# Genie-Kim/PintheMemory

Measured on AMD Instinct MI355X. Metric: train imgs/sec 768x768 bs=8 R50-DeepLabV3+ +mem, higher is better.
Workload: dtype f32

## Files before the change

include/pinmem_hip.h:

```cpp
#ifndef PINMEM_HIP_H
#define PINMEM_HIP_H
#include <stddef.h>
#include <stdint.h>

#ifdef __cplusplus
extern "C" {
#endif

typedef enum pm_status { PM_OK = 0, PM_EINVAL = -1, PM_EWORKSPACE = -2, PM_ELAUNCH = -3, PM_EUNSUPPORTED = -4 } pm_status;

typedef enum pm_dtype { PM_F32 = 0, PM_BF16 = 1 } pm_dtype;
#define PM_TF_ZERO_PAD64 1

typedef struct pm_tensor {
  void* ptr;
  int32_t n, h, w, c;
  int64_t pitch;
  int32_t dtype;
  int32_t flags;
} pm_tensor;

#define PM_ABI_VERSION 400

typedef struct pm_conv_params {
  int32_t struct_size;
  int32_t kh, kw, stride, pad, dil;
  int32_t prec;
  void* wino_v;
  int64_t wino_v_bytes;
  void* wxf;
  int64_t wxf_bytes;
  int32_t wxf_valid;
} pm_conv_params;

typedef struct pm_conv_epilogue {
  int64_t struct_size;
  const float* bias;
  const float* scale;
  const float* shift;
  const float* residual;
  int64_t residual_pitch;
  int32_t relu;
  float* bn_partials;
  int64_t bn_partials_bytes;
} pm_conv_epilogue;

const char* pm_last_error(void);
int pm_version(void);

size_t pm_conv_workspace(const pm_tensor* x, const pm_tensor* y, const pm_conv_params* p, int which );
size_t pm_conv_winograd_v_bytes(const pm_tensor* x, const pm_tensor* y, const pm_conv_params* p);
size_t pm_conv_wxf_bytes(const pm_tensor* x, const pm_tensor* y, const pm_conv_params* p);
size_t pm_conv_wxf_bytes_dgrad(const pm_tensor* dy, const pm_tensor* dx, const pm_conv_params* p);
typedef struct pm_wxf_job {
  const float* w;
  void* wxf;
  int64_t wxf_bytes;
  int32_t cout, kh, kw, cin;
  int32_t dgrad;
  int32_t reserved;
} pm_wxf_job;
int pm_conv_wxf_refresh_bf16(const pm_wxf_job* jobs, int n, void* stream);
int pm_conv_wxf_refresh_f32(const pm_wxf_job* jobs, int n, void* stream);
size_t pm_conv_bn_partials_bytes(const pm_tensor* x, const pm_tensor* y, const pm_conv_params* p);
int pm_conv_fwd(const pm_tensor* x, const float* w_krsc, const pm_tensor* y, const pm_conv_params* p,
                const pm_conv_epilogue* ep, void* ws, size_t ws_bytes, void* stream);
int pm_conv_bwd_data(const pm_tensor* dy, const float* w_krsc, const pm_tensor* dx, const pm_conv_params* p,
                     const pm_tensor* add, void* ws, size_t ws_bytes, void* stream);
int pm_conv_bwd_weight(const pm_tensor* x, const pm_tensor* dy, float* dw_krsc, float* dbias, const pm_conv_params* p,
                       void* ws, size_t ws_bytes, void* stream);

typedef struct pm_routing {
  int32_t struct_size;
  int32_t winograd;
  int32_t winograd_fused;
  int32_t conv16;
  int32_t conv16_wide;
  int32_t conv16_persistent;
  int32_t wgrad16;
  int32_t bf16_wgrad;
  int32_t split;
} pm_routing;
int pm_routing_get(pm_routing* out);
int pm_routing_set(const pm_routing* r);


int pm_set_winograd(int mode);
int pm_set_winograd_fused(int on);
int pm_set_conv16(int on);
int pm_set_bf16_wgrad(int on);
int pm_set_wgrad16(int on);
int pm_set_split(int on);

int pm_profile_enable(int on);
int pm_profile_dump(const char* csv_path);
int pm_profile_read(int mode, int bm, int bn, int km, int nst, double* total_ms, double* total_flops, int64_t* launches, int clear);
int pm_profile_read_prec(int mode, int bm, int bn, int km, int nst, int prec, double* total_ms, double* total_flops, int64_t* launches, int clear);
int pm_profile_read_bytes(int mode, int bm, int bn, int km, int nst, int prec, double* total_bytes);

size_t pm_bn_workspace(const pm_tensor* x);
int pm_bn_stats(const pm_tensor* x, float* moments, void* ws, size_t ws_bytes, void* stream);
int pm_bn_stats_finalize(const pm_tensor* x, float eps, float* mean, float* invstd, float* running_mean , float* running_var ,
                         float momentum, void* ws, size_t ws_bytes, void* stream);
int pm_bn_merge(const float* parts, int world, int c, float* moments, void* stream);
int pm_bn_merge_finalize(const float* parts, int world, int c, float eps, float* mean, float* invstd, float* running_mean ,
                         float* running_var , float momentum, void* stream);
int pm_bn_finalize(const float* moments, int c, float eps, float* mean, float* invstd,
                   float* running_mean, float* running_var, float momentum, void* stream);
int pm_bn_apply(const pm_tensor* x, const float* mean, const float* invstd, const float* gamma, const float* beta,
                const pm_tensor* residual , int relu, const pm_tensor* y, void* stream);
int pm_bn_apply_mask(const pm_tensor* x, const float* mean, const float* invstd, const float* gamma, const float* beta,
                     const pm_tensor* residual , int relu, const pm_tensor* y, uint8_t* mask , void* stream);
int pm_bn_bwd_reduce_mask(const pm_tensor* dy, const uint8_t* mask, const pm_tensor* x, const float* mean, const float* invstd,
                          const pm_tensor* gmask , float* sums, void* ws, size_t ws_bytes, void* stream);
int pm_bn_bwd_reduce(const pm_tensor* dy, const pm_tensor* y , const pm_tensor* x, const float* mean, const float* invstd,
                     const float* gamma , const float* beta , int relu, const pm_tensor* gmask ,
                     float* sums, void* ws, size_t ws_bytes, void* stream);
int pm_bn_bwd_apply(const pm_tensor* dy, const pm_tensor* y , const pm_tensor* x, const float* mean, const float* invstd,
                    const float* gamma, const float* beta , const float* sums, float count, int relu, const pm_tensor* dx,
                    const pm_tensor* dres , void* stream);
int pm_bn_partials_finalize(const float* partials, int64_t pixels, int c, float eps, float* mean, float* invstd, float* running_mean ,
                            float* running_var , float momentum, float* moments , void* stream);
int pm_bn_fold(const float* gamma, const float* beta, const float* running_mean, const float* running_var, const float* conv_bias,
               int c, float eps, float* scale, float* shift, void* stream);
int pm_bn_fold_multi(const void* table, const int* cs, const int* offs, int n, int max_c, int total, float eps, float* arena, void* stream);
int pm_relu_bwd(const pm_tensor* dy, const pm_tensor* y, const pm_tensor* dx, void* stream);
int pm_add(const pm_tensor* a, const pm_tensor* b, const pm_tensor* y, void* stream);
int pm_add_n(const pm_tensor* const* xs, int n, const pm_tensor* y, void* stream);
int pm_copy(const pm_tensor* src, const pm_tensor* dst, void* stream);
int pm_scale_shift_act(const pm_tensor* x, const float* scale, const float* shift, const pm_tensor* residual, int relu,
                       const pm_tensor* y, void* stream);

int pm_cast(const pm_tensor* x, const pm_tensor* y, void* stream);

int pm_maxpool3x3s2_fwd(const pm_tensor* x, const pm_tensor* y, uint8_t* argmax, void* stream);
int pm_maxpool3x3s2_bwd(const pm_tensor* dy, const uint8_t* argmax, const pm_tensor* dx, void* stream);
int pm_global_avgpool_fwd(const pm_tensor* x, const pm_tensor* y , void* stream);
int pm_global_avgpool_bwd(const pm_tensor* dy, const pm_tensor* dx, int accumulate, void* stream);

int pm_resize_bilinear_fwd(const pm_tensor* x, const pm_tensor* y, void* stream);
int pm_resize_bilinear_bwd(const pm_tensor* dy, const pm_tensor* dx, int accumulate, void* stream);
size_t pm_resize_bilinear_bwd_workspace(const pm_tensor* dy, const pm_tensor* dx);
int pm_resize_bilinear_bwd_separable(const pm_tensor* dy, const pm_tensor* dx, int accumulate, void* ws, size_t ws_bytes, void* stream);

int pm_resize_bilinear_hp_fwd(const pm_tensor* x, const pm_tensor* y, int flip_w, void* stream);
int pm_softmax_mean_update(const pm_tensor* logits, double* buffer, int counter, void* stream);
int pm_sliding_stitch(const pm_tensor* logits, const int32_t* tiles_xyxy, int ntiles, int H, int W, int flip_w, double* acc, int accumulate, void* stream);
int pm_argmax_f64(const double* buffer, int n, int h, int w, int c, int64_t* out_cls, double* out_prob , void* stream);

// ... 59 lines not shown
```

pinthememory_amd/csrc/bn.hip:

```cpp
#include "pm_common.h"

namespace {

constexpr int CB = 64;
constexpr int RL = 16;

__device__ __forceinline__ float bn_affine(float v, float mu, float is, float ga, float be) {
  const float s = is * ga;
  return fmaf(v, s, fmaf(-mu, s, be));
}

inline int chunk_rows(long P, int C) {
  const long colblocks = std::max<long>(1, (C + CB - 1) / CB);
  const long want = std::max<long>(512, 2048 / colblocks);
  long r = (P + want - 1) / want;
  r = std::max<long>(r, 64);
  return (int)((r + RL - 1) / RL * RL);
}

__global__ __launch_bounds__(256) void bn_stats_partial(const float* __restrict__ x, long pitch, long P, int C, int rows, float* __restrict__ part) {
  __shared__ float sm[RL][CB][2];
  const int g = threadIdx.x & 15, r = threadIdx.x >> 4;
  const int c = blockIdx.y * CB + g * 4;
  const long p0 = (long)blockIdx.x * rows, p1 = min(P, p0 + rows);
  float s1[4] = {0, 0, 0, 0}, s2[4] = {0, 0, 0, 0};
  if (c < C) {
    const float4 k = PM_LD4(x + c);
    for (long p = p0 + r; p < p1; p += RL) {
      const float4 v = PM_LD4(x + p * pitch + c);
      const float d0 = v.x - k.x, d1 = v.y - k.y, d2 = v.z - k.z, d3 = v.w - k.w;
      s1[0] += d0, s1[1] += d1, s1[2] += d2, s1[3] += d3;
      s2[0] += d0 * d0, s2[1] += d1 * d1, s2[2] += d2 * d2, s2[3] += d3 * d3;
    }
  }
#pragma unroll
  for (int j = 0; j < 4; ++j) sm[r][g * 4 + j][0] = s1[j], sm[r][g * 4 + j][1] = s2[j];
  __syncthreads();
  if (threadIdx.x < CB * 2) {
    const int cc = threadIdx.x >> 1, w = threadIdx.x & 1;
    float s = 0.f;
#pragma unroll
    for (int i = 0; i < RL; ++i) s += sm[i][cc][w];
    const int ch = blockIdx.y * CB + cc;
    if (ch < C) part[((long)blockIdx.x * C + ch) * 2 + w] = s;
  }
}

constexpr int FC = 4, FL = 64;
__device__ __forceinline__ void final_sums(const float* __restrict__ part, int nb, int C, int c, int lane, double& s1, double& s2) {
  __shared__ double red[FL][FC][2];
  double a = 0.0, b = 0.0;
  if (c < C)
#pragma unroll 8
    for (int i = lane; i < nb; i += FL) {
      const float2 v = *reinterpret_cast<const float2*>(part + ((long)i * C + c) * 2);
      a += (double)v.x, b += (double)v.y;
    }
  red[lane][threadIdx.x & (FC - 1)][0] = a, red[lane][threadIdx.x & (FC - 1)][1] = b;
  __syncthreads();
  s1 = s2 = 0.0;
  if (lane == 0) {
#pragma unroll
    for (int i = 0; i < FL; ++i) s1 += red[i][threadIdx.x & (FC - 1)][0], s2 += red[i][threadIdx.x & (FC - 1)][1];
  }
}

template <bool FIN>
__global__ __launch_bounds__(256) void bn_stats_final(const float* __restrict__ part, int nb, const float* __restrict__ x, long P, int C, float* __restrict__ moments,
                                                      float eps, float* __restrict__ mean, float* __restrict__ invstd, float* running_mean, float* running_var,
                                                      float momentum) {
  const int c = blockIdx.x * FC + (threadIdx.x & (FC - 1)), lane = threadIdx.x / FC;
  double s1, s2;
  final_sums(part, nb, C, c, lane, s1, s2);
  if (lane != 0 || c >= C) return;
  const double n = (double)P;
  const float m = (float)((double)x[c] + s1 / n), m2 = (float)fmax(s2 - s1 * s1 / n, 0.0), nf = (float)n;
  if constexpr (!FIN) {
    moments[c] = m;
    moments[C + c] = m2;
    moments[2 * C + c] = nf;
  } else {
    const float var = m2 / nf;
    mean[c] = m;
    invstd[c] = 1.f / sqrtf(var + eps);
    if (running_mean) running_mean[c] = (1.f - momentum) * running_mean[c] + momentum * m;
    if (running_var && nf > 1.f) running_var[c] = (1.f - momentum) * running_var[c] + momentum * (m2 / (nf - 1.f));
  }
}

__global__ void bn_finalize_kernel(const float* __restrict__ moments, int C, float eps, float* __restrict__ mean, float* __restrict__ invstd,
                                   float* running_mean, float* running_var, float momentum) {
  const int c = blockIdx.x * blockDim.x + threadIdx.x;
  if (c >= C) return;
// ... 291 lines not shown
  PM_REQUIRE(!gmask || (relu != 0 && pm_vec4(gmask) && pm_same_shape(gmask, x)), PM_EINVAL, "bn_bwd_reduce: gmask needs a ReLU mode and the shape of x");
  PM_REQUIRE(ws && ws_bytes >= pm_bn_workspace(x), PM_EWORKSPACE, "bn_bwd_reduce: workspace too small");
  const long P = pm_pixels(x);
  const int rows = chunk_rows(P, x->c), nb = pm_cdiv(P, rows);
  hipStream_t st = (hipStream_t)stream;
  dim3 grid(nb, pm_cdiv(x->c, CB));
  const float *pdy = (const float*)dy->ptr, *py = relu == 1 ? (const float*)y->ptr : nullptr, *px = (const float*)x->ptr;
  const long yp = relu == 1 ? y->pitch : 0;
  float* pg = gmask ? (float*)gmask->ptr : nullptr;
  const long gp = gmask ? gmask->pitch : 0;
#define PM_BN_BWD_PARTIAL(R, G)                                                                                                                         \
  hipLaunchKernelGGL((bn_bwd_partial<R, G>), grid, dim3(256), 0, st, pdy, (long)dy->pitch, py, yp, px, (long)x->pitch, mean, invstd, gamma, beta, pg, gp, P, \
                     x->c, rows, (float*)ws)
  if (relu == 0) PM_BN_BWD_PARTIAL(0, false);
  else if (relu == 1 && gmask) PM_BN_BWD_PARTIAL(1, true);
  else if (relu == 1) PM_BN_BWD_PARTIAL(1, false);
  else if (gmask) PM_BN_BWD_PARTIAL(2, true);
  else PM_BN_BWD_PARTIAL(2, false);
#undef PM_BN_BWD_PARTIAL
  hipLaunchKernelGGL(bn_bwd_final, dim3(pm_cdiv(x->c, FC)), dim3(256), 0, st, (const float*)ws, nb, x->c, sums);
  return pm_check_launch("bn_bwd_reduce");
}

extern "C" int pm_bn_bwd_reduce_mask(const pm_tensor* dy, const uint8_t* mask, const pm_tensor* x, const float* mean, const float* invstd,
                                     const pm_tensor* gmask, float* sums, void* ws, size_t ws_bytes, void* stream) {
  PM_REQUIRE(dy && x && mask, PM_EINVAL, "bn_bwd_reduce_mask: null");
  if (pm_is_bf16(x)) return pm16_bn_bwd_reduce(dy, nullptr, mask, x, mean, invstd, nullptr, nullptr, 3, gmask, sums, ws, ws_bytes, (hipStream_t)stream);
  if (int e = check_bn(dy, "bn_bwd_reduce_mask")) return e;
  if (int e = check_bn(x, "bn_bwd_reduce_mask")) return e;
  PM_REQUIRE(pm_same_shape(dy, x) && mean && invstd && sums && mask, PM_EINVAL, "bn_bwd_reduce_mask: bad args");
  PM_REQUIRE(!gmask || (pm_vec4(gmask) && pm_same_shape(gmask, x)), PM_EINVAL, "bn_bwd_reduce_mask: gmask must have the shape of x");
  PM_REQUIRE(ws && ws_bytes >= pm_bn_workspace(x), PM_EWORKSPACE, "bn_bwd_reduce_mask: workspace too small");
  const long P = pm_pixels(x);
  const int rows = chunk_rows(P, x->c), nb = pm_cdiv(P, rows);
  hipStream_t st = (hipStream_t)stream;
  dim3 grid(nb, pm_cdiv(x->c, CB));
  float* pg = gmask ? (float*)gmask->ptr : nullptr;
  const long gp = gmask ? gmask->pitch : 0;
  if (gmask)
    hipLaunchKernelGGL((bn_bwd_partial<3, true>), grid, dim3(256), 0, st, (const float*)dy->ptr, (long)dy->pitch, reinterpret_cast<const float*>(mask), 0l,
                       (const float*)x->ptr, (long)x->pitch, mean, invstd, (const float*)nullptr, (const float*)nullptr, pg, gp, P, x->c, rows, (float*)ws);
  else
    hipLaunchKernelGGL((bn_bwd_partial<3, false>), grid, dim3(256), 0, st, (const float*)dy->ptr, (long)dy->pitch, reinterpret_cast<const float*>(mask), 0l,
                       (const float*)x->ptr, (long)x->pitch, mean, invstd, (const float*)nullptr, (const float*)nullptr, pg, gp, P, x->c, rows, (float*)ws);
  hipLaunchKernelGGL(bn_bwd_final, dim3(pm_cdiv(x->c, FC)), dim3(256), 0, st, (const float*)ws, nb, x->c, sums);
  return pm_check_launch("bn_bwd_reduce_mask");
}

extern "C" int pm_bn_bwd_apply(const pm_tensor* dy, const pm_tensor* y, const pm_tensor* x, const float* mean, const float* invstd, const float* gamma,
                               const float* beta, const float* sums, float count, int relu, const pm_tensor* dx, const pm_tensor* dres, void* stream) {
  PM_REQUIRE(dy && x && dx, PM_EINVAL, "bn_bwd_apply: null");
  if (pm_is_bf16(x)) return pm16_bn_bwd_apply(dy, y, x, mean, invstd, gamma, beta, sums, count, relu, dx, dres, (hipStream_t)stream);
  if (int e = check_bn(dy, "bn_bwd_apply")) return e;
  if (int e = check_bn(x, "bn_bwd_apply")) return e;
  if (int e = check_bn(dx, "bn_bwd_apply")) return e;
  PM_REQUIRE(pm_same_shape(dy, x) && pm_same_shape(dx, x) && mean && invstd && gamma && sums, PM_EINVAL, "bn_bwd_apply: bad args");
  PM_REQUIRE(relu >= 0 && relu <= 2, PM_EINVAL, "bn_bwd_apply: relu mode %d (0 none, 1 mask from y, 2 mask rebuilt from x)", relu);
  PM_REQUIRE(relu != 1 || (y && pm_vec4(y) && pm_same_shape(y, x)), PM_EINVAL, "bn_bwd_apply: relu mode 1 needs the forward output");
  PM_REQUIRE(relu != 2 || beta, PM_EINVAL, "bn_bwd_apply: relu mode 2 needs beta");
  PM_REQUIRE(!dres || (pm_vec4(dres) && pm_same_shape(dres, x)), PM_EINVAL, "bn_bwd_apply: dres shape mismatch");
  const float *pd = (const float*)dy->ptr, *po = relu == 1 ? (const float*)y->ptr : nullptr, *px = (const float*)x->ptr;
  float *pdx = (float*)dx->ptr, *pdr = dres ? (float*)dres->ptr : nullptr;
  const long a = dy->pitch, b = relu == 1 ? y->pitch : 0, c = x->pitch, d = dx->pitch, e2 = dres ? dres->pitch : 0;
  const bool from_x = relu == 2;
  const int C = x->c;
  const bool dev_count = !(count > 0.f);
  const float host_inv_n = dev_count ? 0.f : 1.f / count;
  return pm_ew_launch(true, pm_pixels(x), C, (hipStream_t)stream, "bn_bwd_apply", [=] __device__(long p, int ch) {
    const float inv_n = dev_count ? 1.f / sums[2 * C] : host_inv_n;
    float4 g = PM_LD4(pd + p * a + ch);
    if (po) {
      const float4 o = PM_LD4(po + p * b + ch);
      g.x = o.x > 0.f ? g.x : 0.f, g.y = o.y > 0.f ? g.y : 0.f, g.z = o.z > 0.f ? g.z : 0.f, g.w = o.w > 0.f ? g.w : 0.f;
    }
    const float4 v = PM_LD4(px + p * c + ch), mu = PM_LD4(mean + ch), is = PM_LD4(invstd + ch), ga = PM_LD4(gamma + ch);
    if (from_x) {
      const float4 be = PM_LD4(beta + ch);
      g.x = bn_affine(v.x, mu.x, is.x, ga.x, be.x) > 0.f ? g.x : 0.f, g.y = bn_affine(v.y, mu.y, is.y, ga.y, be.y) > 0.f ? g.y : 0.f;
      g.z = bn_affine(v.z, mu.z, is.z, ga.z, be.z) > 0.f ? g.z : 0.f, g.w = bn_affine(v.w, mu.w, is.w, ga.w, be.w) > 0.f ? g.w : 0.f;
    }
    if (pdr) PM_ST4(pdr + p * e2 + ch, g);
    const float4 s1 = PM_LD4(sums + ch), s2 = PM_LD4(sums + C + ch);
    float4 r;
    r.x = (g.x - s1.x * inv_n - (v.x - mu.x) * is.x * (s2.x * inv_n)) * (is.x * ga.x);
    r.y = (g.y - s1.y * inv_n - (v.y - mu.y) * is.y * (s2.y * inv_n)) * (is.y * ga.y);
    r.z = (g.z - s1.z * inv_n - (v.z - mu.z) * is.z * (s2.z * inv_n)) * (is.z * ga.z);
    r.w = (g.w - s1.w * inv_n - (v.w - mu.w) * is.w * (s2.w * inv_n)) * (is.w * ga.w);
    PM_ST4(pdx + p * d + ch, r);
  });
}
```

pinthememory_amd/csrc/conv_igemm.hip:

```cpp
#include <stdlib.h>
#include <algorithm>
#include <type_traits>
#include <vector>

#include "pm_common.h"

#include "conv_igemm_kernel.h"

namespace {

template <int ZL, bool O16 = false>
__global__ __launch_bounds__(256) void splitk_reduce_vec_kernel(const float* __restrict__ ws, int ksplit, long slab, int M, int Nn,
                                                                float* __restrict__ C, long c_pitch, const float* bias,
                                                                const float* scale, const float* shift, const float* residual,
                                                                long res_pitch, int relu) {
  constexpr int GP = 256 / ZL;
  __shared__ float4 red[ZL > 1 ? ZL : 1][GP];
  const int gl = threadIdx.x % GP, zl = threadIdx.x / GP;
  const long groups = (long)M * Nn / 4;
  for (long g0 = (long)blockIdx.x * GP; g0 < groups; g0 += (long)gridDim.x * GP) {
    const long grp = g0 + gl;
    float4 v = make_float4(0.f, 0.f, 0.f, 0.f);
    if (grp < groups)
#pragma unroll 8
// ... 375 lines not shown
    g_prof.push_back(rec);
  }
  return pm_check_launch("conv_igemm");
}

int check_common(const pm_tensor* x, const pm_tensor* y, const pm_conv_params* p) {
  PM_REQUIRE(x && y && p && x->ptr && y->ptr, PM_EINVAL, "conv: null tensor");
  PM_REQUIRE(p->struct_size == (int32_t)sizeof(pm_conv_params), PM_EINVAL, "conv: pm_conv_params.struct_size %d != %zu -- caller built against another pinmem_hip.h (library ABI %d)",
             p->struct_size, sizeof(pm_conv_params), PM_ABI_VERSION);
  PM_REQUIRE(p->kh >= 1 && p->kw >= 1 && p->dil >= 1 && p->pad >= 0, PM_EINVAL, "conv: bad geometry");
  PM_REQUIRE(p->stride == 1 || p->stride == 2, PM_EUNSUPPORTED, "conv: stride %d unsupported (1 or 2)", p->stride);
  const int ho = (x->h + 2 * p->pad - p->dil * (p->kh - 1) - 1) / p->stride + 1;
  const int wo = (x->w + 2 * p->pad - p->dil * (p->kw - 1) - 1) / p->stride + 1;
  PM_REQUIRE(ho == y->h && wo == y->w && x->n == y->n, PM_EINVAL, "conv: output %dx%d does not match geometry (%dx%d)", y->h, y->w, ho, wo);
  PM_REQUIRE((x->dtype == PM_F32 || x->dtype == PM_BF16) && (y->dtype == PM_F32 || y->dtype == PM_BF16), PM_EUNSUPPORTED, "conv: dtype %d / %d", x->dtype, y->dtype);
  for (const pm_tensor* t : {x, y}) {
    if (pm_is_bf16(t)) PM_REQUIRE(pm_vec8(t), PM_EINVAL, "conv: bf16 tensors must be 16B aligned with pitch %% 8 == 0 and channels %% 8 == 0");
    else PM_REQUIRE(pm_vec_ok(t), PM_EINVAL, "conv: tensors must be 16B aligned with pitch %% 4 == 0");
  }
  PM_REQUIRE(x->c % 4 == 0, PM_EUNSUPPORTED, "conv: Cin %% 4 != 0 unsupported (pad the input channels)");
  PM_REQUIRE((y->c % 4 == 0) || (p->kh * p->kw == 1), PM_EUNSUPPORTED, "conv: Cout %% 4 != 0 only for 1x1");
  PM_REQUIRE(x->pitch >= x->c && y->pitch >= y->c, PM_EINVAL, "conv: pitch < channels");
  PM_REQUIRE(pm_pixels(x) * x->pitch < (1ll << 29) && pm_pixels(y) * y->pitch < (1ll << 29) && (int64_t)y->c * x->c * p->kh * p->kw < (1ll << 29),
             PM_EUNSUPPORTED, "conv: tensor too large for 32-bit byte offsets (2 GiB per tensor)");
  return PM_OK;
}

void fill_geom(ConvK& k, const pm_tensor* x, const pm_tensor* y, const pm_conv_params* p) {
  k.N = x->n, k.H = x->h, k.W = x->w, k.Cin = x->c, k.x_pitch = x->pitch;
  k.Ho = y->h, k.Wo = y->w, k.Cout = y->c, k.y_pitch = y->pitch;
  k.kh = p->kh, k.kw = p->kw, k.stride = p->stride, k.pad = p->pad, k.dil = p->dil;
  k.sshift = p->stride == 2 ? 1 : 0;
  k.prec = p->prec != 0 ? 1 : 0;
  k.T_eff = p->kh * p->kw, k.tk_w = p->kw, k.ky0 = k.kx0 = 0, k.ksy = k.ksx = 1;
  k.sub = k.sub_cy = k.sub_cx = 0, k.Hc = x->h, k.Wc = x->w;
  k.bias = k.scale = k.shift = k.residual = nullptr;
  k.res_pitch = 0, k.relu = 0, k.stats = nullptr, k.io16 = 0;
  k.stage_ep = 1;
  k.spl_prio = 1;
  k.n_group = 8;
  k.batch_xcd = 0;
  k.a_bs = k.b_bs = k.c_bs = 0;
}

struct WinoPlan {
  bool use;
  pm_wino_geom g;
  int Kp, P;
  size_t v_bytes, m_bytes, u_bytes;
  Plan pl;
};
WinoPlan wino_plan(const pm_tensor* xin, int cout, const pm_conv_params* p, bool wgrad = false) {
  WinoPlan wp{};
  if (wgrad && (long)xin->c * cout < 256 * 256) return wp;
  if (pm_route.winograd == 0 || p->kh != 3 || p->kw != 3 || p->stride != 1 || p->pad != p->dil || p->prec != 0) return wp;
  const int cin = xin->c;
  if (cin < 128 || cout < 128 || (cout & 3) || (cin & 3)) return wp;
  int m = 0;
  double best_ratio = 0.6;
  for (int cand = pm_route.winograd; cand >= 2; cand -= 2) {
    const pm_wino_geom g = pm_wino_make_geom(xin->n, xin->h, xin->w, p->dil, cand);
    const double cover = (double)(cand * g.TY * p->dil) * (double)(cand * g.TX * p->dil) / ((double)xin->h * xin->w);
    const double ratio = cover * (cand + 2) * (cand + 2) / (9.0 * cand * cand);
    if (ratio <= best_ratio) best_ratio = ratio, m = cand, wp.g = g;
  }
  if (!m) return wp;
  wp.P = (m + 2) * (m + 2);
  wp.Kp = (cin + BK - 1) / BK * BK;
  if (wp.g.tiles * (long)std::max(wp.Kp, cout) * 4 >= (1ll << 31)) return wp;
  wp.v_bytes = pm_align_up((size_t)wp.P * wp.g.tiles * wp.Kp * sizeof(float), 256);
  wp.m_bytes = pm_align_up((size_t)wp.P * wp.g.tiles * cout * sizeof(float), 256);
  wp.u_bytes = pm_align_up((size_t)wp.P * cout * wp.Kp * sizeof(float), 256);
  wp.pl.bm = 128, wp.pl.bn = 128;
  if (pm_cdiv(cout, 128) * 128 > cout * 1.12 && pm_cdiv(cout, 64) * 64 < pm_cdiv(cout, 128) * 128) wp.pl.bn = 64;
  if (wp.g.tiles <= 4608 && !pm_route.split) wp.pl.bm = 64;
  wp.pl.tiles_m = pm_cdiv(wp.g.tiles, wp.pl.bm), wp.pl.tiles_n = pm_cdiv(cout, wp.pl.bn);
  wp.pl.ksplit = 1, wp.pl.kper = wp.Kp, wp.pl.ws_bytes = 0;
  wp.use = true;
  return wp;
}
inline size_t wino_ws(const WinoPlan& wp) { return wp.v_bytes + wp.m_bytes + wp.u_bytes; }

int wino_conv(const pm_tensor* xin, const float* w, int w_cout, int w_cin, bool dgrad, const pm_tensor* yout, const WinoPlan& wp,
              const pm_conv_epilogue& ep, void* ws, hipStream_t st, float* v_keep = nullptr, float* u_ext = nullptr, bool u_valid = false) {
  float* V = v_keep ? v_keep : (float*)ws;
  float* Mo = (float*)((char*)ws + wp.v_bytes);
  float* U = u_ext ? u_ext : (float*)((char*)ws + wp.v_bytes + wp.m_bytes);
  const int cout = yout->c;
  if (int e = pm_wino_input_xf((const float*)xin->ptr, xin->pitch, xin->c, wp.Kp, wp.g, V, st)) return e;
  if (!(u_ext && u_valid))
    if (int e = pm_wino_filter_xf(w, w_cout, w_cin, wp.Kp, dgrad, wp.g.m, U, st)) return e;
  const pm_tensor xv = {V, 1, 1, (int32_t)wp.g.tiles, wp.Kp, wp.Kp};
  const pm_tensor yv = {Mo, 1, 1, (int32_t)wp.g.tiles, cout, cout};
  const pm_conv_params p1 = {(int32_t)sizeof(pm_conv_params), 1, 1, 1, 0, 1, 0};
  ConvK k;
  fill_geom(k, &xv, &yv, &p1);
  k.A = V, k.B = U, k.C = Mo;
  k.M = (int)wp.g.tiles, k.Nn = cout, k.K = wp.Kp;
  k.a_bytes = (unsigned)(wp.g.tiles * wp.Kp * 4), k.b_bytes = (unsigned)((long)cout * wp.Kp * 4), k.kmode = K_FAST;
  k.c_pitch = cout, k.c_split = 0;
  k.a_bs = wp.g.tiles * wp.Kp, k.b_bs = (long)cout * wp.Kp, k.c_bs = wp.g.tiles * cout;
  if (pm_route.winograd_fused && wp.g.m == 4 && wp.Kp % 16 == 0) {
    ProfRec rec{};
    if (g_prof_on) {
      (void)hipEventCreate(&rec.a), (void)hipEventCreate(&rec.b);
      rec.mode = 3, rec.bm = 32, rec.bn = 32, rec.km = 0, rec.prec = 0, rec.nst = 1, rec.M = (int)wp.g.tiles, rec.Nn = cout, rec.K = wp.Kp, rec.batch = wp.P, rec.ksplit = 1;
      rec.flops = 2.0 * wp.P * (double)wp.g.tiles * cout * xin->c;
      (void)hipEventRecord(rec.a, st);
    }
    const int e = pm_wino_fused_f4(V, U, cout, wp.Kp, wp.g, (float*)yout->ptr, yout->pitch, ep.bias, ep.scale, ep.shift, ep.residual, ep.residual_pitch, ep.relu, st);
    if (g_prof_on) {
      (void)hipEventRecord(rec.b, st);
      g_prof.push_back(rec);
    }
    return e;
  }
  if (int e = launch<MODE_FWD>(k, wp.pl, st, wp.P, 2.0 * wp.P * (double)wp.g.tiles * cout * xin->c)) return e;
  return pm_wino_output_xf(Mo, cout, wp.g, (float*)yout->ptr, yout->pitch, ep.bias, ep.scale, ep.shift, ep.residual, ep.residual_pitch, ep.relu, st);
}

struct WinoWgradPlan {
  Plan pl;
  size_t slab_bytes;
};
WinoWgradPlan wino_wgrad_plan(const WinoPlan& wp, int cout) {
  WinoWgradPlan q{};
  q.pl.bm = 128, q.pl.bn = 128;
  if (pm_cdiv(wp.Kp, 128) * 128 > wp.Kp * 1.12 && pm_cdiv(wp.Kp, 64) * 64 < pm_cdiv(wp.Kp, 128) * 128) q.pl.bn = 64;
  q.pl.tiles_m = pm_cdiv(cout, 128), q.pl.tiles_n = pm_cdiv(wp.Kp, q.pl.bn);
  const long ksteps = (wp.g.tiles + BK - 1) / BK;
  const long per_split = (long)q.pl.tiles_m * q.pl.tiles_n * wp.P;
  long ks = std::max<long>(1, std::min<long>((768 + per_split / 2) / per_split, ksteps / 8));
  const long steps_per = (ksteps + ks - 1) / ks;
  ks = (ksteps + steps_per - 1) / steps_per;
  q.pl.ksplit = (int)ks, q.pl.kper = (int)(steps_per * BK), q.pl.ws_bytes = 0;
  q.slab_bytes = pm_align_up((size_t)ks * wp.P * cout * wp.Kp * sizeof(float), 256);
  return q;
}
inline size_t wino_wgrad_ws(const WinoPlan& wp, const WinoWgradPlan& q) { return wp.v_bytes + wp.m_bytes + q.slab_bytes; }

int wino_wgrad(const pm_tensor* x, const pm_tensor* dy, float* dw, const WinoPlan& wp, const WinoWgradPlan& q, void* ws, hipStream_t st,
               float* v_kept = nullptr) {
  float* V = v_kept ? v_kept : (float*)ws;
  float* Z = (float*)((char*)ws + wp.v_bytes);
  float* slab = (float*)((char*)ws + wp.v_bytes + wp.m_bytes);
  const int cout = dy->c;
  if (!v_kept)
    if (int e = pm_wino_input_xf((const float*)x->ptr, x->pitch, x->c, wp.Kp, wp.g, V, st)) return e;
  if (int e = pm_wino_dy_xf((const float*)dy->ptr, dy->pitch, cout, wp.g, Z, st)) return e;
  const pm_tensor xv = {V, 1, 1, (int32_t)wp.g.tiles, wp.Kp, wp.Kp};
  const pm_tensor zv = {Z, 1, 1, (int32_t)wp.g.tiles, cout, cout};
  const pm_conv_params p1 = {(int32_t)sizeof(pm_conv_params), 1, 1, 1, 0, 1, 0};
  ConvK k;
  fill_geom(k, &xv, &zv, &p1);
  k.A = Z, k.B = V, k.C = slab;
  k.M = cout, k.Nn = wp.Kp, k.K = (int)wp.g.tiles;
  k.a_bytes = (unsigned)(wp.g.tiles * cout * 4), k.b_bytes = (unsigned)(wp.g.tiles * wp.Kp * 4), k.kmode = K_MID;
  k.c_pitch = wp.Kp, k.c_split = (long)wp.P * cout * wp.Kp;
  k.a_bs = wp.g.tiles * cout, k.b_bs = wp.g.tiles * wp.Kp, k.c_bs = (long)cout * wp.Kp;
  if (int e = launch<MODE_WGRAD>(k, q.pl, st, wp.P, 2.0 * wp.P * (double)wp.g.tiles * cout * x->c)) return e;
  return pm_wino_dw_xf(slab, q.pl.ksplit, cout, x->c, wp.Kp, wp.g.m, dw, st);
}

struct Bf16Plan {
  bool use;
  bool c16;
  pm_conv16 k16;
  bool inplace;
  int Cp;
  long M, Nn, Kf;
  size_t xb_bytes, wb_bytes;
  Plan pl;
};
Bf16Plan bf16_plan(const pm_tensor* xin, const pm_tensor* yout, const pm_conv_params* p) {
  Bf16Plan b{};
  if ((p->prec != 2 && !pm_is_bf16(xin) && !pm_is_bf16(yout)) || xin->c < 32) return b;
  b.Cp = (xin->c + 63) / 64 * 64;
  const long T = (long)p->kh * p->kw;
  b.M = pm_pixels(yout), b.Nn = yout->c, b.Kf = T * b.Cp / 2;
  b.inplace = pm_is_bf16(xin) && (xin->c % 64 == 0 || ((xin->flags & PM_TF_ZERO_PAD64) && xin->pitch >= b.Cp));
  const size_t xb = b.inplace ? (size_t)pm_pixels(xin) * xin->pitch * 2 : (size_t)pm_pixels(xin) * b.Cp * 2, wb = (size_t)yout->c * T * b.Cp * 2;
  if (xb >= (1ull << 31) || wb >= (1ull << 31)) return b;
  b.xb_bytes = b.inplace ? 0 : pm_align_up(xb, 256), b.wb_bytes = pm_align_up(wb, 256);
  b.pl = make_plan(MODE_FWD, b.M, b.Nn, b.Kf, true);
  if (b.pl.bn < 64) return b;
  b.use = true;
  constexpr long C16_MIN_M = 256;
  b.c16 = false;
  if (pm_route.conv16 && b.M >= C16_MIN_M && p->stride >= 1) {
    pm_conv16& k = b.k16;
    k = pm_conv16{};
    k.N = xin->n, k.H = xin->h, k.W = xin->w, k.Ho = yout->h, k.Wo = yout->w;
    k.a_pitch = b.inplace ? xin->pitch : b.Cp, k.Cp = b.Cp;
    k.kh = p->kh, k.kw = p->kw, k.stride = p->stride, k.pad = p->pad, k.dil = p->dil;
    k.M = (int)b.M, k.Nn = (int)b.Nn, k.K = (int)(T * b.Cp), k.ksteps = k.K / 64;
    k.c_pitch = yout->pitch, k.c_f32 = pm_is_bf16(yout) ? 0 : 1;
    pm_conv16_plan(&k);
    b.c16 = pm_route.conv16 == 2 || k.wide || k.bm == 64 || k.ksteps_per == 1 || (b.pl.bm == 64 && k.ksteps >= 16);
  }
  return b;
}
inline size_t bf16_ws(const Bf16Plan& b) {
  return b.xb_bytes + b.wb_bytes + std::max(pm_align_up(b.pl.ws_bytes, 256), b.c16 ? pm_conv16_slab_bytes(&b.k16) : (size_t)0);
}

int conv_bf16(const pm_tensor* xin, const float* w, int w_cout, int w_cin, bool rotate, const pm_tensor* yout, const pm_conv_params* pe, const Bf16Plan& b,
              const pm_conv_epilogue& e0, void* ws, hipStream_t st, char* wb_ext = nullptr, bool wb_valid = false) {
  char* xb = b.inplace ? (char*)xin->ptr : (char*)ws;
  char* wb = wb_ext ? wb_ext : (char*)ws + b.xb_bytes;
  float* slab = (float*)((char*)ws + b.xb_bytes + b.wb_bytes);
  const int T = pe->kh * pe->kw;
  if (!b.inplace) {
    if (pm_is_bf16(xin)) {
      if (int e = pm16_pad_rows((const pm_bf16*)xin->ptr, xin->pitch, xin->c, b.Cp, pm_pixels(xin), (pm_bf16*)xb, st)) return e;
    } else if (int e = pm_bf16_cast_rows((const float*)xin->ptr, xin->pitch, xin->c, b.Cp, pm_pixels(xin), xb, st)) return e;
  }
  if (!(wb_ext && wb_valid))
    if (int e = pm_bf16_cast_weights(w, w_cout, T, w_cin, b.Cp, rotate, wb, st)) return e;
  const long xpitch16 = b.inplace ? xin->pitch : b.Cp;
  if (b.c16) {
    const bool o16 = pm_is_bf16(yout);
    const bool ep_any = e0.bias || e0.scale || e0.residual || e0.relu;
    const bool ok = (!e0.bn_partials || o16) &&
                    (o16 ? ((yout->c | yout->pitch | (e0.residual ? e0.residual_pitch : 0)) & 7) == 0 && pm_aligned16(yout->ptr) && pm_aligned16(e0.residual)
                         : !(e0.scale || e0.residual || e0.relu));
    if (ok) {
      pm_conv16 k = b.k16;
      k.A = (const pm_bf16*)xb, k.B = (const pm_bf16*)wb;
      const double fl = 2.0 * (double)b.M * (double)b.Nn * (double)T * (double)xin->c * (g_prof_on ? pm_conv16_executed_fraction(&k) : 1.0);
      ProfRec rec{};
      if (g_prof_on) {
        (void)hipEventCreate(&rec.a), (void)hipEventCreate(&rec.b);
// ... 237 lines not shown
  pm_route.conv16_wide = (on == 3 || on == 8) ? 2 : (on == 7 ? 3 : ((on == 2 || on == 4) ? 0 : pm_route_defaults.conv16_wide));
  pm_route.conv16_persistent = on == 8 ? 0 : (on == 3 ? 1 : pm_route_defaults.conv16_persistent);
  return PM_OK;
}
extern "C" int pm_set_winograd_fused(int on) {
  pm_route.winograd_fused = on != 0;
  return PM_OK;
}
extern "C" int pm_set_wgrad16(int on) {
  pm_route.wgrad16 = on != 0;
  return PM_OK;
}
extern "C" int pm_set_split(int on) {
  pm_route.split = on ? 1 : 0;
  return PM_OK;
}
extern "C" int pm_set_bf16_wgrad(int on) {
  pm_route.bf16_wgrad = on != 0;
  return PM_OK;
}
extern "C" int pm_profile_enable(int on) {
  g_prof_on = on != 0;
  return PM_OK;
}
extern "C" int pm_profile_read_prec(int mode, int bm, int bn, int km, int nst, int prec, double* total_ms, double* total_flops, int64_t* launches, int clear);
extern "C" int pm_profile_read(int mode, int bm, int bn, int km, int nst, double* total_ms, double* total_flops, int64_t* launches, int clear) {
  return pm_profile_read_prec(mode, bm, bn, km, nst, -1, total_ms, total_flops, launches, clear);
}
extern "C" int pm_profile_read_prec(int mode, int bm, int bn, int km, int nst, int prec, double* total_ms, double* total_flops, int64_t* launches, int clear) {
  double ms = 0.0, fl = 0.0;
  int64_t n = 0;
  for (const ProfRec& r : g_prof) {
    if ((mode >= 0 && r.mode != mode) || (bm >= 0 && r.bm != bm) || (bn >= 0 && r.bn != bn) || (km >= 0 && r.km != km) || (nst >= 0 && r.nst != nst) ||
        (prec >= 0 && r.prec != prec))
      continue;
    float t = 0.f;
    if (hipEventSynchronize(r.b) != hipSuccess || hipEventElapsedTime(&t, r.a, r.b) != hipSuccess) continue;
    ms += t, fl += r.flops, ++n;
  }
  if (clear) {
    for (const ProfRec& r : g_prof) (void)hipEventDestroy(r.a), (void)hipEventDestroy(r.b);
    g_prof.clear();
  }
  if (total_ms) *total_ms = ms;
  if (total_flops) *total_flops = fl;
  if (launches) *launches = n;
  return PM_OK;
}

extern "C" int pm_profile_read_bytes(int mode, int bm, int bn, int km, int nst, int prec, double* total_bytes) {
  double b = 0.0;
  for (const ProfRec& r : g_prof) {
    if ((mode >= 0 && r.mode != mode) || (bm >= 0 && r.bm != bm) || (bn >= 0 && r.bn != bn) || (km >= 0 && r.km != km) || (nst >= 0 && r.nst != nst) ||
        (prec >= 0 && r.prec != prec))
      continue;
    b += r.bytes;
  }
  if (total_bytes) *total_bytes = b;
  return PM_OK;
}

extern "C" int pm_profile_dump(const char* path) {
  PM_REQUIRE(path, PM_EINVAL, "pm_profile_dump: null path");
  FILE* f = fopen(path, "w");
  PM_REQUIRE(f, PM_EINVAL, "pm_profile_dump: cannot open %s", path);
  fprintf(f, "mode,bm,bn,km,nst,prec,M,N,K,batch,ksplit,ms,gflop\n");
  for (const ProfRec& r : g_prof) {
    float t = 0.f;
    if (hipEventSynchronize(r.b) != hipSuccess || hipEventElapsedTime(&t, r.a, r.b) != hipSuccess) continue;
    fprintf(f, "%d,%d,%d,%d,%d,%d,%d,%d,%d,%d,%d,%.5f,%.4f\n", r.mode, r.bm, r.bn, r.km, r.nst, r.prec, r.M, r.Nn, r.K, r.batch, r.ksplit, t, r.flops * 1e-9);
  }
  fclose(f);
  return PM_OK;
}

extern "C" size_t pm_conv_winograd_v_bytes(const pm_tensor* x, const pm_tensor* y, const pm_conv_params* p0) {
  if (!x || !y || !p0) return 0;
  const pm_conv_params tp = tier_params(p0, x, y);
  const pm_conv_params* p = &tp;
  const WinoPlan f = wino_plan(x, y->c, p), g = wino_plan(x, y->c, p, true);
  return (f.use && g.use && f.g.m == g.g.m) ? f.v_bytes : 0;
}

extern "C" size_t pm_conv_wxf_bytes(const pm_tensor* x, const pm_tensor* y, const pm_conv_params* p0) {
  if (!x || !y || !p0) return 0;
  const pm_conv_params tp = tier_params(p0, x, y);
  const pm_conv_params* p = &tp;
  const WinoPlan f = wino_plan(x, y->c, p);
  if (f.use) return f.u_bytes;
  if (p->prec == 2) {
    const Bf16Plan b = bf16_plan(x, y, p);
    if (b.use) return b.wb_bytes;
  }
  return 0;
}

extern "C" int pm_conv_wxf_refresh_f32(const pm_wxf_job* jobs, int n, void* stream) {
  PM_REQUIRE(n >= 0 && (jobs || n == 0), PM_EINVAL, "conv_wxf_refresh_f32: bad job table");
  std::vector<const float*> w(n);
  std::vector<float*> U(n);
  std::vector<int> cout(n), cin(n), kp(n), m(n);
  for (int i = 0; i < n; ++i) {
    const pm_wxf_job& q = jobs[i];
    PM_REQUIRE(q.w && q.wxf && q.cout > 0 && q.cin > 0 && q.kh == 3 && q.kw == 3 && q.dgrad == 0, PM_EINVAL,
               "conv_wxf_refresh_f32: job %d: forward transforms of 3x3 filters only", i);
    PM_REQUIRE(pm_aligned16(q.wxf), PM_EINVAL, "conv_wxf_refresh_f32: job %d: buffer must be 16-byte aligned", i);
    const int Kp = (q.cin + BK - 1) / BK * BK;
    const size_t u4 = pm_align_up((size_t)36 * q.cout * Kp * sizeof(float), 256), u2 = pm_align_up((size_t)16 * q.cout * Kp * sizeof(float), 256);
    PM_REQUIRE((size_t)q.wxf_bytes == u4 || (size_t)q.wxf_bytes == u2, PM_EINVAL, "conv_wxf_refresh_f32: job %d: %ld bytes is neither the F(4x4) nor the F(2x2) transform of %d x %d",
               i, (long)q.wxf_bytes, q.cout, q.cin);
    w[i] = q.w, U[i] = (float*)q.wxf, cout[i] = q.cout, cin[i] = q.cin, kp[i] = Kp, m[i] = (size_t)q.wxf_bytes == u4 ? 4 : 2;
  }
  return pm_wino_filter_xf_multi(w.data(), U.data(), cout.data(), cin.data(), kp.data(), m.data(), n, (hipStream_t)stream);
}

extern "C" size_t pm_conv_wxf_bytes_dgrad(const pm_tensor* dy, const pm_tensor* dx, const pm_conv_params* p0) {
  if (!dy || !dx || !p0) return 0;
  const pm_conv_params tp = tier_params(p0, dy, dx);
  if (!dgrad_bf16_ok(&tp)) return 0;
  const pm_conv_params q = dgrad_as_fwd(&tp);
  const Bf16Plan b = bf16_plan(dy, dx, &q);
  return b.use ? b.wb_bytes : 0;
}

static bool bn_partials_route(const pm_tensor* x, const pm_tensor* y, const pm_conv_params* p) {
  if (!x || !y || !p || check_common(x, y, p) != PM_OK) return false;
  if (pm_is_bf16(y)) {
    if (!pm_vec8(y)) return false;
    const Bf16Plan b = bf16_plan(x, y, p);
    return b.use && (b.c16 ? (b.k16.ksplit == 1 && !b.k16.wide) : b.pl.ksplit == 1);
  }
  if (pm_is_bf16(x)) return false;
  if ((y->c & 3) || (y->pitch & 3) || !pm_aligned16(y->ptr)) return false;
  if (p->prec == 2) {
    const Bf16Plan b = bf16_plan(x, y, p);
    if (b.use) return b.pl.ksplit == 1;
  }
  if (wino_plan(x, y->c, p).use) return false;
  if (p->prec != 0) return false;
  long M, Nn, K;
  gemm_dims(MODE_FWD, x, y, p, M, Nn, K);
  const Plan pl = make_plan(MODE_FWD, M, Nn, K, false);
  return pl.ksplit == 1 && pl.bn >= 64;
}
extern "C" size_t pm_conv_bn_partials_bytes(const pm_tensor* x, const pm_tensor* y, const pm_conv_params* p) {
  if (!bn_partials_route(x, y, p)) return 0;
  return pm_align_up((size_t)pm_cdiv(pm_pixels(y), 32) * y->c * 2 * sizeof(float), 256);
}

extern "C" size_t pm_conv_workspace(const pm_tensor* x, const pm_tensor* y, const pm_conv_params* p0, int which) {
  const pm_conv_params tp = tier_params(p0, x, y);
  const pm_conv_params* p = &tp;
  if (which == MODE_DGRAD && p->stride == 2) {
    {
      const S2Native s = s2_native_plan(y, x, p);
      if (s.ok) return s.total;
    }
    size_t slab = 0, tmp = 0;
    for (int cls = 0; cls < 4; ++cls) {
      const S2Class c = s2_class(cls, x, p);
      tmp = std::max(tmp, (size_t)c.M * x->c * sizeof(float));
      if (c.M > 0 && c.nky * c.nkx > 0) slab = std::max(slab, make_plan(MODE_DGRAD, c.M, x->c, (long)c.nky * c.nkx * y->c, p->prec != 0).ws_bytes);
    }
    return pm_align_up(4 * pm_align_up(tmp, 256) + slab + 256, 256) + upcast_bytes(y);
  }
  if (which == MODE_FWD && p->prec == 2) {
    const Bf16Plan b = bf16_plan(x, y, p);
    if (b.use) return bf16_ws(b);
  }
  if (which == MODE_DGRAD && dgrad_bf16_ok(p)) {
    const pm_conv_params q = dgrad_as_fwd(p);
    const Bf16Plan b = bf16_plan(y, x, &q);
    if (b.use) return bf16_ws(b);
  }
  if (which == MODE_FWD || which == MODE_DGRAD) {
    const WinoPlan wp = which == MODE_FWD ? wino_plan(x, y->c, p) : wino_plan(y, x->c, p);
    if (wp.use) return wino_ws(wp);
  }
  const size_t bias_part = pm_align_up((size_t)pm_cdiv(pm_pixels(y), colsum_rows(pm_pixels(y), y->c)) * y->c * sizeof(float), 256);
  if (which == MODE_WGRAD && (pm_is_bf16(x) || pm_is_bf16(y))) {
    long M, Nn, K;
    gemm_dims(which, x, y, p, M, Nn, K);
    return pm_align_up(make_plan(which, M, Nn, K, true).ws_bytes, 256) + bias_part + upcast_bytes(x) + upcast_bytes(y);
  }
  if (which == MODE_WGRAD && p->prec == 2) {
    const Bf16WgradPlan b = bf16_wgrad_plan(x, y, p);
    if (b.use) return pm_align_up(bf16_wgrad_ws(b), 256) + bias_part;
  }
  if (which == MODE_WGRAD) {
    const WinoPlan wp = wino_plan(x, y->c, p, true);
    if (wp.use) return pm_align_up(wino_wgrad_ws(wp, wino_wgrad_plan(wp, y->c)), 256) + bias_part;
  }
  long M, Nn, K;
  gemm_dims(which, x, y, p, M, Nn, K);
  size_t b = make_plan(which, M, Nn, K, p->prec != 0).ws_bytes;
  if (which == MODE_WGRAD) b += bias_part;
  return pm_align_up(b, 256);
}

extern "C" int pm_conv_fwd(const pm_tensor* x, const float* w, const pm_tensor* y, const pm_conv_params* p0,
                           const pm_conv_epilogue* ep, void* ws, size_t ws_bytes, void* stream) {
  if (int e = check_common(x, y, p0)) return e;
  const pm_conv_params tp = tier_params(p0, x, y);
  const pm_conv_params* p = &tp;
  PM_REQUIRE(!ep || ep->struct_size == (int64_t)sizeof(pm_conv_epilogue), PM_EINVAL,
             "conv_fwd: pm_conv_epilogue.struct_size %ld != %zu -- caller built against another pinmem_hip.h (library ABI %d)", ep ? (long)ep->struct_size : 0l,
             sizeof(pm_conv_epilogue), PM_ABI_VERSION);
  if (ep && ep->bn_partials) {
    PM_REQUIRE(!ep->relu && !ep->residual, PM_EINVAL, "conv_fwd: bn_partials are the statistics of the convolution output (no residual / ReLU)");
    const size_t need = pm_conv_bn_partials_bytes(x, y, p);
    PM_REQUIRE(need != 0 && (size_t)ep->bn_partials_bytes >= need, PM_EINVAL, "conv_fwd: this call cannot emit bn_partials (ask pm_conv_bn_partials_bytes): %zu needed", need);
  }
  PM_REQUIRE(w && pm_aligned16(w), PM_EINVAL, "conv_fwd: weight null or unaligned");
  {
    pm_conv_epilogue e1 = {(int64_t)sizeof(pm_conv_epilogue), nullptr, nullptr, nullptr, nullptr, 0, 0};
    if (ep) e1 = *ep;
    PM_REQUIRE((e1.scale == nullptr) == (e1.shift == nullptr), PM_EINVAL, "conv_fwd: scale and shift go together");
    const WinoPlan wp = wino_plan(x, y->c, p);
    if (wp.use) {
      PM_REQUIRE(ws && ws_bytes >= wino_ws(wp), PM_EWORKSPACE, "conv_fwd(winograd): workspace %zu < %zu", ws_bytes, wino_ws(wp));
      float* keep = (p->wino_v && (size_t)p->wino_v_bytes >= wp.v_bytes) ? (float*)p->wino_v : nullptr;
      float* uext = (p->wxf && (size_t)p->wxf_bytes >= wp.u_bytes) ? (float*)p->wxf : nullptr;
      return wino_conv(x, w, y->c, x->c, false, y, wp, e1, ws, (hipStream_t)stream, keep, uext, p->wxf_valid != 0);
    }
  }
  if (p->prec == 2) {
    const Bf16Plan b = bf16_plan(x, y, p);
    if (b.use) {
      pm_conv_epilogue e2 = {(int64_t)sizeof(pm_conv_epilogue), nullptr, nullptr, nullptr, nullptr, 0, 0};
      if (ep) e2 = *ep;
      PM_REQUIRE((e2.scale == nullptr) == (e2.shift == nullptr), PM_EINVAL, "conv_fwd: scale and shift go together");
      PM_REQUIRE(ws && ws_bytes >= bf16_ws(b), PM_EWORKSPACE, "conv_fwd(bf16): workspace %zu < %zu", ws_bytes, bf16_ws(b));
      char* wext = (p->wxf && (size_t)p->wxf_bytes >= b.wb_bytes) ? (char*)p->wxf : nullptr;
      return conv_bf16(x, w, y->c, x->c, false, y, p, b, e2, ws, (hipStream_t)stream, wext, p->wxf_valid != 0);
    }
  }
  PM_REQUIRE(pm_is_f32(x), PM_EUNSUPPORTED, "conv_fwd: a bf16 input needs at least 32 channels (got %d)", x->c);
  long M, Nn, K;
  gemm_dims(MODE_FWD, x, y, p, M, Nn, K);
  Plan pl = make_plan(MODE_FWD, M, Nn, K, p->prec != 0);
  PM_REQUIRE(pl.ws_bytes <= ws_bytes && (pl.ws_bytes == 0 || ws), PM_EWORKSPACE, "conv_fwd: workspace %zu < %zu", ws_bytes, pl.ws_bytes);
  ConvK k;
  fill_geom(k, x, y, p);
  k.io16 = pm_is_bf16(y) ? 1 : 0;
  k.A = (const float*)x->ptr, k.B = w;
  k.M = (int)M, k.Nn = (int)Nn, k.K = (int)K;
  k.a_bytes = (unsigned)(pm_pixels(x) * x->pitch * 4), k.b_bytes = (unsigned)((long)y->c * K * 4), k.kmode = x->c % BK == 0 ? 0 : (x->c >= BK ? 1 : 2);
  pm_conv_epilogue e0 = {(int64_t)sizeof(pm_conv_epilogue), nullptr, nullptr, nullptr, nullptr, 0, 0};
  if (ep) e0 = *ep;
  PM_REQUIRE((e0.scale == nullptr) == (e0.shift == nullptr), PM_EINVAL, "conv_fwd: scale and shift go together");
  hipStream_t st = (hipStream_t)stream;
  if (pl.ksplit > 1) {
    k.C = (float*)ws, k.c_pitch = Nn, k.c_split = M * Nn;
    if (int e = launch<MODE_FWD>(k, pl, st)) return e;
    return splitk_reduce((const float*)ws, pl.ksplit, M, Nn, (float*)y->ptr, (long)y->pitch, e0.bias, e0.scale, e0.shift, e0.residual,
                         (long)e0.residual_pitch, e0.relu, st, k.io16 != 0);
  }
  k.C = (float*)y->ptr, k.c_pitch = y->pitch, k.c_split = 0;
  k.bias = e0.bias, k.scale = e0.scale, k.shift = e0.shift, k.residual = e0.residual, k.res_pitch = e0.residual_pitch, k.relu = e0.relu;
  k.stats = e0.bn_partials;
  return launch<MODE_FWD>(k, pl, st);
}

extern "C" int pm_conv_bwd_data(const pm_tensor* dy0, const float* w, const pm_tensor* dx, const pm_conv_params* p0, const pm_tensor* add,
                                void* ws, size_t ws_bytes, void* stream) {
  if (int e = check_common(dx, dy0, p0)) return e;
  const pm_conv_params tp = tier_params(p0, dy0, dx);
  const pm_conv_params* p = &tp;
  const pm_tensor* dy = dy0;
  pm_tensor dy32;
  PM_REQUIRE(!add || (add->ptr && pm_same_shape(add, dx) && add->dtype == dx->dtype), PM_EINVAL, "conv_bwd_data: `add` must match dx (shape and dtype)");
  PM_REQUIRE(!add || !pm_is_bf16(add) || pm_vec8(add), PM_EINVAL, "conv_bwd_data: bf16 `add` must be 16B aligned with pitch %% 8 == 0");
  const float* addp = add ? (const float*)add->ptr : nullptr;
  const long add_pitch = add ? add->pitch : 0;
  PM_REQUIRE(w && pm_aligned16(w), PM_EINVAL, "conv_bwd_data: weight null or unaligned");
  hipStream_t st0 = (hipStream_t)stream;
  if (p->stride == 2) {
    const size_t need = pm_conv_workspace(dx, dy, p, MODE_DGRAD);
    PM_REQUIRE(ws && ws_bytes >= need, PM_EWORKSPACE, "conv_bwd_data(stride 2): workspace %zu < %zu", ws_bytes, need);
    PM_REQUIRE(dx->c % 4 == 0, PM_EUNSUPPORTED, "conv_bwd_data(stride 2): Cin %% 4 != 0");
    {
      S2Native s = s2_native_plan(dy, dx, p);
      if (s.ok) return dgrad_s2_bf16(dy, w, dx, p, add, s, ws, st0);
    }
    if (pm_is_bf16(dy)) {
      if (int e = upcast(dy0, (char*)ws + need - upcast_bytes(dy0), &dy32, st0)) return e;
      dy = &dy32;
    }
    size_t tmp_bytes = 0;
    for (int cls = 0; cls < 4; ++cls) tmp_bytes = std::max(tmp_bytes, (size_t)s2_class(cls, dx, p).M * dx->c * sizeof(float));
    tmp_bytes = pm_align_up(tmp_bytes, 256);
    float* tmp = (float*)ws;
    float* slab = (float*)((char*)ws + 4 * tmp_bytes);
    unsigned char valid[4];
    for (int cls = 0; cls < 4; ++cls) {
      const S2Class c = s2_class(cls, dx, p);
      valid[cls] = c.M > 0 && c.nky * c.nkx > 0;
      if (!valid[cls]) continue;
      const long Kc = (long)c.nky * c.nkx * dy->c;
      const Plan pl = make_plan(MODE_DGRAD, c.M, dx->c, Kc, p->prec != 0);
      ConvK k;
      fill_geom(k, dx, dy, p);
      k.A = (const float*)dy->ptr, k.B = w;
      k.M = (int)c.M, k.Nn = dx->c, k.K = (int)Kc;
      k.a_bytes = (unsigned)(pm_pixels(dy) * dy->pitch * 4), k.b_bytes = (unsigned)((long)dy->c * p->kh * p->kw * dx->c * 4);
      k.kmode = dy->c >= BK ? K_MID : K_SMALL;
      k.T_eff = c.nky * c.nkx, k.tk_w = c.nkx, k.ky0 = c.ky0, k.kx0 = c.kx0, k.ksy = c.ksy, k.ksx = c.ksx;
      k.sub = 1, k.sub_cy = c.cy, k.sub_cx = c.cx, k.Hc = c.Hc, k.Wc = c.Wc;
      float* out = (float*)((char*)tmp + cls * tmp_bytes);
      if (pl.ksplit > 1) {
        k.C = slab, k.c_pitch = dx->c, k.c_split = c.M * dx->c;
        if (int e = launch<MODE_DGRAD>(k, pl, st0)) return e;
        if (int e = splitk_reduce(slab, pl.ksplit, c.M, dx->c, out, (long)dx->c, nullptr, nullptr, nullptr, nullptr, 0l, 0, st0)) return e;
      } else {
        k.C = out, k.c_pitch = dx->c, k.c_split = 0;
        if (int e = launch<MODE_DGRAD>(k, pl, st0)) return e;
      }
    }
    const int valid_mask = valid[0] | (valid[1] << 1) | (valid[2] << 2) | (valid[3] << 3);
    const long total = pm_pixels(dx) * (dx->c / 4);
    if (pm_is_bf16(dx))
      hipLaunchKernelGGL(dgrad_s2_interleave_kernel<true>, dim3((int)std::min<long>((total + 255) / 256, 8192)), dim3(256), 0, st0, (const float*)tmp,
                         (long)(tmp_bytes / sizeof(float)), valid_mask, (float*)dx->ptr, (long)dx->pitch, dx->n, dx->h, dx->w, dx->c, addp, add_pitch);
    else
      hipLaunchKernelGGL(dgrad_s2_interleave_kernel<false>, dim3((int)std::min<long>((total + 255) / 256, 8192)), dim3(256), 0, st0, (const float*)tmp,
                         (long)(tmp_bytes / sizeof(float)), valid_mask, (float*)dx->ptr, (long)dx->pitch, dx->n, dx->h, dx->w, dx->c, addp, add_pitch);
    return pm_check_launch("dgrad_s2_interleave");
  }
  if (dgrad_bf16_ok(p)) {
    const pm_conv_params q = dgrad_as_fwd(p);
    const Bf16Plan b = bf16_plan(dy, dx, &q);
    if (b.use) {
      PM_REQUIRE(ws && ws_bytes >= bf16_ws(b), PM_EWORKSPACE, "conv_bwd_data(bf16): workspace %zu < %zu", ws_bytes, bf16_ws(b));
      const pm_conv_epilogue e1 = {(int64_t)sizeof(pm_conv_epilogue), nullptr, nullptr, nullptr, addp, add_pitch, 0};
      char* wext = (p->wxf && (size_t)p->wxf_bytes >= b.wb_bytes) ? (char*)p->wxf : nullptr;
      return conv_bf16(dy, w, dy->c, dx->c, true, dx, &q, b, e1, ws, st0, wext, p->wxf_valid != 0);
    }
  }
  {
    const WinoPlan wp = wino_plan(dy, dx->c, p);
    if (wp.use) {
      PM_REQUIRE(ws && ws_bytes >= wino_ws(wp), PM_EWORKSPACE, "conv_bwd_data(winograd): workspace %zu < %zu", ws_bytes, wino_ws(wp));
      const pm_conv_epilogue e1 = {(int64_t)sizeof(pm_conv_epilogue), nullptr, nullptr, nullptr, addp, add_pitch, 0};
      return wino_conv(dy, w, dy->c, dx->c, true, dx, wp, e1, ws, st0);
    }
  }
  PM_REQUIRE(pm_is_f32(dy), PM_EUNSUPPORTED, "conv_bwd_data: a bf16 dy needs at least 32 channels and a stride-1 geometry the forward form covers");
  long M, Nn, K;
  gemm_dims(MODE_DGRAD, dx, dy, p, M, Nn, K);
  Plan pl = make_plan(MODE_DGRAD, M, Nn, K, p->prec != 0);
  PM_REQUIRE(pl.ws_bytes <= ws_bytes && (pl.ws_bytes == 0 || ws), PM_EWORKSPACE, "conv_bwd_data: workspace %zu < %zu", ws_bytes, pl.ws_bytes);
  ConvK k;
  fill_geom(k, dx, dy, p);
  k.io16 = pm_is_bf16(dx) ? 1 : 0;
  k.A = (const float*)dy->ptr, k.B = w;
  k.M = (int)M, k.Nn = (int)Nn, k.K = (int)K;
  k.a_bytes = (unsigned)(pm_pixels(dy) * dy->pitch * 4), k.b_bytes = (unsigned)((long)dy->c * p->kh * p->kw * dx->c * 4), k.kmode = (dy->c % BK == 0 && p->stride == 1) ? 0 : (dy->c >= BK ? 1 : 2);
  hipStream_t st = (hipStream_t)stream;
  if (pl.ksplit > 1) {
    k.C = (float*)ws, k.c_pitch = Nn, k.c_split = M * Nn;
    if (int e = launch<MODE_DGRAD>(k, pl, st)) return e;
    return splitk_reduce((const float*)ws, pl.ksplit, M, Nn, (float*)dx->ptr, (long)dx->pitch, nullptr, nullptr, nullptr, addp, add_pitch, 0, st, k.io16 != 0);
  }
  k.C = (float*)dx->ptr, k.c_pitch = dx->pitch, k.c_split = 0;
  k.residual = addp, k.res_pitch = add_pitch;
  return launch<MODE_DGRAD>(k, pl, st);
}

extern "C" int pm_conv_bwd_weight(const pm_tensor* x0, const pm_tensor* dy0, float* dw, float* dbias, const pm_conv_params* p0, void* ws,
                                  size_t ws_bytes, void* stream) {
  if (int e = check_common(x0, dy0, p0)) return e;
  const pm_conv_params tp = tier_params(p0, x0, dy0);
  const pm_conv_params* p = &tp;
  PM_REQUIRE(dw && pm_aligned16(dw), PM_EINVAL, "conv_bwd_weight: dw null or unaligned");
  hipStream_t st = (hipStream_t)stream;
  const size_t need = pm_conv_workspace(x0, dy0, p, MODE_WGRAD);
  PM_REQUIRE(need <= ws_bytes && ws, PM_EWORKSPACE, "conv_bwd_weight: workspace %zu < %zu", ws_bytes, need);
  const pm_tensor *x = x0, *dy = dy0;
  pm_tensor x32, dy32;
  const bool tier = pm_is_bf16(x0) || pm_is_bf16(dy0);
  const bool native16 = pm_is_bf16(x0) && pm_is_bf16(dy0) && dy0->c >= 32;
  if (tier) {
    char* tail = (char*)ws + need;
    if (!native16 && pm_is_bf16(x0)) {
      tail -= upcast_bytes(x0);
      if (int e = upcast(x0, tail, &x32, st)) return e;
      x = &x32;
    }
    if (pm_is_bf16(dy0) && (!native16 || dbias)) {
      tail -= upcast_bytes(dy0);
      if (int e = upcast(dy0, tail, &dy32, st)) return e;
      if (!native16) dy = &dy32;
    }
  }
  long M, Nn, K;
  gemm_dims(MODE_WGRAD, x, dy, p, M, Nn, K);
  Plan pl = make_plan(MODE_WGRAD, M, Nn, K, p->prec != 0);
  const Bf16WgradPlan bw = tier ? Bf16WgradPlan{} : bf16_wgrad_plan(x, dy, p);
  if (bw.use) {
    if (int e = conv_wgrad_bf16(x, dy, dw, p, bw, ws, st)) return e;
    pl.ws_bytes = bf16_wgrad_ws(bw);
  }
  const WinoPlan wp = wino_plan(x, dy->c, p, true);
  if (wp.use) {
    const WinoWgradPlan q = wino_wgrad_plan(wp, dy->c);
    float* kept = (p->wino_v && (size_t)p->wino_v_bytes >= wp.v_bytes) ? (float*)p->wino_v : nullptr;
    if (int e = wino_wgrad(x, dy, dw, wp, q, ws, st, kept)) return e;
    pl.ws_bytes = wino_wgrad_ws(wp, q);
  }
  ConvK k;
  fill_geom(k, x, dy, p);
  if (p->prec == 2) k.prec = 3;
  if (native16) {
    PM_REQUIRE(x->c % 8 == 0 && dy->c % 8 == 0 && pl.bn >= 64, PM_EUNSUPPORTED, "conv_bwd_weight(bf16): channels %% 8 != 0 or a tile narrower than 64");
    k.prec = 4;
    pl.kper = (pl.kper + 63) / 64 * 64;
    pl.ksplit = (int)((K + pl.kper - 1) / pl.kper);
  }
  const int esz = native16 ? 2 : 4;
  k.A = (const float*)dy->ptr, k.B = (const float*)x->ptr;
  k.M = (int)M, k.Nn = (int)Nn, k.K = (int)K;
  k.a_bytes = (unsigned)(pm_pixels(dy) * dy->pitch * esz), k.b_bytes = (unsigned)(pm_pixels(x) * x->pitch * esz), k.kmode = dy->w >= (native16 ? 2 * BK : BK) ? 1 : 2;
  pm_wgrad16 w16{};
  bool use16 = false;
  if (native16 && !wp.use && !bw.use) {
    w16.X = (const pm_bf16*)x->ptr, w16.DY = (const pm_bf16*)dy->ptr;
    w16.N = x->n, w16.H = x->h, w16.W = x->w, w16.Ho = dy->h, w16.Wo = dy->w;
    w16.x_pitch = x->pitch, w16.dy_pitch = dy->pitch, w16.Cin = x->c, w16.Cout = dy->c;
    w16.kh = p->kh, w16.kw = p->kw, w16.stride = p->stride, w16.pad = p->pad, w16.dil = p->dil;
    w16.M = (int)M, w16.Nn = (int)Nn, w16.P = (int)K, w16.kper = 64, w16.c_split = M * Nn;
    w16.C = dw;
    use16 = K < (1l << 30) && pm_wgrad16_plan(&w16);
    if (use16) {
      const long tiles = (long)w16.tiles_m * w16.tiles_n, steps = (K + 63) / 64;
      int best_ks = 1;
      double best = 1e30;
      for (int ks = 1; ks <= pl.ksplit; ++ks) {
        const long per = (steps + ks - 1) / ks, kse = (steps + per - 1) / per;
        const long rounds = (tiles * kse + 255) / 256;
        const double cost = (double)rounds * (per + 6) + (kse > 1 ? (double)kse * M * Nn * 8.0 / 4e12 / 1.0e-6 : 0.0);
        if (cost < best) best = cost, best_ks = (int)kse;
      }
      const long per = (steps + best_ks - 1) / best_ks;
      w16.kper = (int)per * 64, w16.ksplit = (int)((steps + per - 1) / per);
    }
  }
  if (use16) {
    ProfRec rec{};
    if (g_prof_on) {
      (void)hipEventCreate(&rec.a), (void)hipEventCreate(&rec.b);
      rec.mode = MODE_WGRAD, rec.bm = w16.bm, rec.bn = w16.bn, rec.km = 2, rec.prec = 4, rec.nst = 3, rec.M = (int)M, rec.Nn = (int)Nn, rec.K = (int)K, rec.batch = 1, rec.ksplit = w16.ksplit,
      rec.flops = 2.0 * (double)M * (double)Nn * (double)K;
      (void)hipEventRecord(rec.a, st);
    }
    if (w16.ksplit > 1) w16.C = (float*)ws;
    const int e = pm_wgrad16_launch(&w16, st);
    if (g_prof_on) {
      (void)hipEventRecord(rec.b, st);
      g_prof.push_back(rec);
    }
    if (e) return e;
    if (w16.ksplit > 1)
      if (int e2 = splitk_reduce((const float*)ws, w16.ksplit, M, Nn, dw, (long)Nn, nullptr, nullptr, nullptr, nullptr, 0l, 0, st)) return e2;
  } else if (wp.use || bw.use) {
  } else if (pl.ksplit > 1) {
    k.C = (float*)ws, k.c_pitch = Nn, k.c_split = M * Nn;
    if (int e = launch<MODE_WGRAD>(k, pl, st)) return e;
    if (int e = splitk_reduce((const float*)ws, pl.ksplit, M, Nn, dw, (long)Nn, nullptr, nullptr, nullptr, nullptr, 0l, 0, st)) return e;
  } else {
    k.C = dw, k.c_pitch = Nn, k.c_split = 0;
    if (int e = launch<MODE_WGRAD>(k, pl, st)) return e;
  }
  if (dbias) {
    const pm_tensor* dyb = pm_is_bf16(dy0) ? &dy32 : dy0;
    const long P = pm_pixels(dyb);
    const int rpb = colsum_rows(P, dyb->c), nb = pm_cdiv(P, rpb);
    float* part = (float*)((char*)ws + pm_align_up(pl.ws_bytes, 256));
    if (dyb->pitch == ((dyb->c + 3) & ~3) && dyb->pitch <= 64 && pm_aligned16(dyb->ptr))
      hipLaunchKernelGGL(colsum_partial_narrow_kernel, dim3(nb), dim3(256), 0, st, (const float*)dyb->ptr, (int)(dyb->pitch / 4), P, dyb->c, rpb, part);
    else
      hipLaunchKernelGGL(colsum_partial_kernel, dim3(nb, pm_cdiv(dyb->c, 64)), dim3(256), 0, st, (const float*)dyb->ptr, (long)dyb->pitch, P, dyb->c, rpb, part);
    hipLaunchKernelGGL(colsum_final_kernel, dim3(pm_cdiv(dyb->c, 64)), dim3(1024), 0, st, (const float*)part, nb, dyb->c, dbias);
    return pm_check_launch("conv_bias_grad");
  }
  return PM_OK;
}
```

pinthememory_amd/csrc/pm_common.h:

```cpp
#pragma once
#include <hip/hip_runtime.h>
#include <algorithm>
#include <atomic>
#include <stdarg.h>
#include <stdint.h>
#include <stdio.h>

#include "../../include/pinmem_hip.h"

void pm_set_error(const char* fmt, ...);

#define PM_REQUIRE(cond, code, ...)      \
  do {                                   \
    if (!(cond)) {                       \
      pm_set_error(__VA_ARGS__);         \
      return (code);                     \
    }                                    \
  } while (0)

static inline int pm_check_launch(const char* what) {
  hipError_t e = hipGetLastError();
  if (e != hipSuccess) {
    pm_set_error("%s: launch failed: %s", what, hipGetErrorString(e));
    return PM_ELAUNCH;
  }
  return PM_OK;
}

static inline bool pm_aligned16(const void* p) { return (reinterpret_cast<uintptr_t>(p) & 15u) == 0; }
static inline int64_t pm_pixels(const pm_tensor* t) { return (int64_t)t->n * t->h * t->w; }
static inline int pm_cdiv(int64_t a, int64_t b) { return (int)((a + b - 1) / b); }
static inline size_t pm_align_up(size_t v, size_t a) { return (v + a - 1) / a * a; }

static inline bool pm_vec_ok(const pm_tensor* t) { return pm_aligned16(t->ptr) && (t->pitch % 4) == 0; }
static inline bool pm_is_f32(const pm_tensor* t) { return t->dtype == PM_F32; }
static inline bool pm_is_bf16(const pm_tensor* t) { return t->dtype == PM_BF16; }
#define PM_REQUIRE_F32(t, who) PM_REQUIRE(!(t) || pm_is_f32(t), PM_EUNSUPPORTED, "%s: fp32 tensors only (got dtype %d)", who, (t)->dtype)
static inline bool pm_vec8(const pm_tensor* t) { return pm_is_bf16(t) && pm_aligned16(t->ptr) && (t->pitch % 8) == 0 && (t->c % 8) == 0; }

struct pm_wino_geom {
  int N, H, W, d, m, TY, TX;
  long tiles;
};
pm_wino_geom pm_wino_make_geom(int n, int h, int w, int d, int m);
int pm_wino_input_xf(const float* x, long pitch, int C, int Kp, const pm_wino_geom& g, float* V, hipStream_t st);
int pm_wino_filter_xf(const float* w, int Cout, int Cin, int Kp, bool dgrad, int m, float* U, hipStream_t st);
int pm_wino_filter_xf_multi(const float* const* w, float* const* U, const int* cout, const int* cin, const int* kp, const int* m, int n, hipStream_t st);
int pm_wino_output_xf(const float* M, int Cout, const pm_wino_geom& g, float* y, long ypitch, const float* bias, const float* scale, const float* shift,
                      const float* residual, long res_pitch, int relu, hipStream_t st);
int pm_wino_fused_f4(const float* V, const float* U, int Cout, int Kp, const pm_wino_geom& g, float* y, long ypitch, const float* bias, const float* scale,
                     const float* shift, const float* residual, long res_pitch, int relu, hipStream_t st);
int pm_wino_dy_xf(const float* dy, long pitch, int Cout, const pm_wino_geom& g, float* Z, hipStream_t st);
int pm_wino_dw_xf(const float* slab, int ks, int Cout, int Cin, int Kp, int m, float* dw, hipStream_t st);

int pm_bf16_cast_rows(const float* x, long pitch, int C, int Cp, long P, void* out, hipStream_t st);
int pm_bf16_cast_weights(const float* w, int Cout, int T, int Cin, int Cp, bool rotate, void* out, hipStream_t st);
struct PmS2Classes {
  int ky0[4], nky[4], kx0[4], nkx[4];
  void* out[4];
};
int pm_bf16_cast_weights_s2(const float* w, int Cout, int kh, int kw, int Cin, int Cp, const PmS2Classes* cl, hipStream_t st);
int pm_bf16_transpose_taps(const float* x, long pitch, int C, int N, int H, int W, int Ho, int Wo, int kh, int kw, int stride, int pad, int dil, void* out,
                           hipStream_t st);

typedef unsigned short pm_bf16;
int pm16_bn_stats(const pm_tensor* x, float* moments, float eps, float* mean, float* invstd, float* running_mean, float* running_var, float momentum, void* ws,
                  size_t ws_bytes, hipStream_t st);
size_t pm16_bn_workspace(const pm_tensor* x);
int pm16_bn_apply_mask(const pm_tensor* x, const float* mean, const float* invstd, const float* gamma, const float* beta, const pm_tensor* res, int relu,
                       const pm_tensor* y, uint8_t* mask, hipStream_t st);
int pm16_bn_bwd_reduce(const pm_tensor* dy, const pm_tensor* y, const uint8_t* mask, const pm_tensor* x, const float* mean, const float* invstd, const float* gamma,
                       const float* beta, int relu, const pm_tensor* gmask, float* sums, void* ws, size_t ws_bytes, hipStream_t st);
int pm16_bn_bwd_apply(const pm_tensor* dy, const pm_tensor* y, const pm_tensor* x, const float* mean, const float* invstd, const float* gamma, const float* beta,
                      const float* sums, float count, int relu, const pm_tensor* dx, const pm_tensor* dres, hipStream_t st);
int pm16_add_n(const pm_tensor* const* xs, int n, const pm_tensor* y, hipStream_t st);
int pm16_copy(const pm_tensor* x, const pm_tensor* y, hipStream_t st);
int pm16_maxpool_fwd(const pm_tensor* x, const pm_tensor* y, uint8_t* argmax, hipStream_t st);
int pm16_maxpool_bwd(const pm_tensor* dy, const uint8_t* argmax, const pm_tensor* dx, hipStream_t st);
int pm16_gap_fwd(const pm_tensor* x, const pm_tensor* y, hipStream_t st);
int pm16_gap_bwd(const pm_tensor* dy, const pm_tensor* dx, int accumulate, hipStream_t st);
int pm16_resize_fwd(const pm_tensor* x, const pm_tensor* y, hipStream_t st);
int pm16_resize_bwd(const pm_tensor* dy, const pm_tensor* dx, int accumulate, hipStream_t st);
size_t pm16_resize_bwd_workspace(const pm_tensor* dy, const pm_tensor* dx);
int pm16_resize_bwd_separable(const pm_tensor* dy, const pm_tensor* dx, int accumulate, void* ws, size_t ws_bytes, hipStream_t st);
int pm16_to_f32(const pm_bf16* x, long pitch, int C, long P, float* out, long out_pitch, hipStream_t st);
int pm16_pad_rows(const pm_bf16* x, long pitch, int C, int Cp, long P, pm_bf16* out, hipStream_t st);

struct pm_conv16 {
  const pm_bf16* A;
  const pm_bf16* B;
  void* C;
  int N, H, W, Ho, Wo;
  long a_pitch;
  int Cp;
  int kh, kw, stride, pad, dil;
  int M, Nn, K, ksteps;
  long c_pitch;
  int c_f32;
  const float *bias, *scale, *shift;
  const void* residual;
  long res_pitch;
  int relu;
  float* stats;
  int bm, bn, tiles_m, tiles_n, ksplit, ksteps_per;
  long c_split;
  int wide;
};
void pm_conv16_plan(pm_conv16* k);
int pm_conv16w_launch(const pm_conv16* k, hipStream_t st);
int pm_conv16w_persistent(const pm_conv16* k);
size_t pm_conv16_slab_bytes(const pm_conv16* k);
double pm_conv16_executed_fraction(const pm_conv16* k);
int pm_conv16_launch(const pm_conv16* k, hipStream_t st);

struct pm_wgrad16 {
  const pm_bf16* X;
  const pm_bf16* DY;
  float* C;
  int N, H, W, Ho, Wo;
  long x_pitch, dy_pitch;
  int Cin, Cout, kh, kw, stride, pad, dil;
  int M, Nn, P;
  int kper, ksplit;
  long c_split;
  int bm, bn, tiles_m, tiles_n;
};
bool pm_wgrad16_plan(pm_wgrad16* k);
int pm_wgrad16_launch(const pm_wgrad16* k, hipStream_t st);
// ... 165 lines not shown
```

pinthememory_amd/csrc/winograd.hip:

```cpp
#include "pm_common.h"

namespace {

enum { W_BT = 0, W_AT = 1, W_G = 2, W_A = 3, W_GT = 4 };

template <int MT>
__host__ __device__ constexpr float wino_bt(int i, int j) {
  if (MT == 2) {
    constexpr float t[4][4] = {{1, 0, -1, 0}, {0, 1, 1, 0}, {0, -1, 1, 0}, {0, 1, 0, -1}};
    return t[i & 3][j & 3];
  }
  constexpr float t[6][6] = {{4, 0, -5, 0, 1, 0}, {0, -4, -4, 1, 1, 0}, {0, 4, -4, -1, 1, 0}, {0, -2, -1, 2, 1, 0}, {0, 2, -1, -2, 1, 0}, {0, 4, 0, -5, 0, 1}};
  return t[i][j];
}
template <int MT>
__host__ __device__ constexpr float wino_at(int i, int j) {
  if (MT == 2) {
    constexpr float t[2][4] = {{1, 1, 1, 0}, {0, 1, -1, -1}};
    return t[i & 1][j & 3];
  }
  constexpr float t[4][6] = {{1, 1, 1, 1, 1, 0}, {0, 1, -1, 2, -2, 0}, {0, 1, 1, 4, 4, 0}, {0, 1, -1, 8, -8, 1}};
  return t[i][j];
}
template <int MT>
__host__ __device__ constexpr float wino_g(int i, int j) {
  if (MT == 2) {
    constexpr float t[4][3] = {{1, 0, 0}, {0.5f, 0.5f, 0.5f}, {0.5f, -0.5f, 0.5f}, {0, 0, 1}};
    return t[i & 3][j];
  }
  constexpr float t[6][3] = {{1.f / 4, 0, 0},          {-1.f / 6, -1.f / 6, -1.f / 6}, {-1.f / 6, 1.f / 6, -1.f / 6},
                             {1.f / 24, 1.f / 12, 1.f / 6}, {1.f / 24, -1.f / 12, 1.f / 6},  {0, 0, 1}};
  return t[i][j];
}
template <int MT, int WHICH>
__host__ __device__ constexpr float wino_coef(int r, int c) {
  return WHICH == W_BT ? wino_bt<MT>(r, c) : WHICH == W_AT ? wino_at<MT>(r, c) : WHICH == W_G ? wino_g<MT>(r, c) : WHICH == W_A ? wino_at<MT>(c, r) : wino_g<MT>(c, r);
}

template <int W>
struct Vec {
  float v[W];
};
template <int W>
__device__ __forceinline__ Vec<W> vzero() {
  Vec<W> r;
#pragma unroll
  for (int i = 0; i < W; ++i) r.v[i] = 0.f;
  return r;
}
template <int W>
__device__ __forceinline__ Vec<W> vload(const float* p) {
  Vec<W> r;
  if constexpr (W == 4) {
    const float4 q = PM_LD4(p);
    r.v[0] = q.x, r.v[1] = q.y, r.v[2] = q.z, r.v[3] = q.w;
  } else if constexpr (W == 2) {
    const float2 q = *reinterpret_cast<const float2*>(p);
    r.v[0] = q.x, r.v[1] = q.y;
  } else {
    r.v[0] = *p;
  }
  return r;
}
template <int W>
__device__ __forceinline__ void vstore(float* p, const Vec<W>& r) {
  if constexpr (W == 4) PM_ST4(p, make_float4(r.v[0], r.v[1], r.v[2], r.v[3]));
  else if constexpr (W == 2) *reinterpret_cast<float2*>(p) = make_float2(r.v[0], r.v[1]);
  else *p = r.v[0];
}

template <int MT, int WHICH, int R, int C, int W>
__device__ __forceinline__ void mat_apply(const Vec<W> (&in)[C], Vec<W> (&out)[R]) {
#pragma unroll
  for (int r = 0; r < R; ++r) {
    Vec<W> acc = vzero<W>();
    bool first = true;
#pragma unroll
    for (int c = 0; c < C; ++c) {
      const float k = wino_coef<MT, WHICH>(r, c);
      if (k == 0.f) continue;
#pragma unroll
      for (int i = 0; i < W; ++i) {
        if (first) acc.v[i] = k == 1.f ? in[c].v[i] : (k == -1.f ? -in[c].v[i] : k * in[c].v[i]);
        else if (k == 1.f) acc.v[i] += in[c].v[i];
        else if (k == -1.f) acc.v[i] -= in[c].v[i];
        else acc.v[i] = fmaf(k, in[c].v[i], acc.v[i]);
      }
      first = false;
    }
    out[r] = acc;
  }
}

struct TileId {
  int n, ry, rx, ty, tx;
};
__device__ __forceinline__ TileId decode_tile(unsigned tile, const pm_wino_geom& g) {
  TileId t;
  t.tx = (int)(tile % (unsigned)g.TX);
  unsigned q = tile / (unsigned)g.TX;
  t.ty = (int)(q % (unsigned)g.TY);
  q /= (unsigned)g.TY;
  t.rx = (int)(q % (unsigned)g.d);
  q /= (unsigned)g.d;
  t.ry = (int)(q % (unsigned)g.d);
  t.n = (int)(q / (unsigned)g.d);
  return t;
}

template <int MT, int W>
__global__ __launch_bounds__(256) void wino_input_kernel(const float* __restrict__ x, long xp, int C, int Kp, const pm_wino_geom g, float* __restrict__ V) {
  constexpr int A = MT + 2;
  const unsigned kg = Kp / W;
  const unsigned total = (unsigned)g.tiles * kg;
  const long plane = g.tiles * (long)Kp;
  for (unsigned i = blockIdx.x * 256u + threadIdx.x; i < total; i += gridDim.x * 256u) {
    const unsigned tile = i / kg;
    const int c = (int)(i - tile * kg) * W;
    const TileId t = decode_tile(tile, g);
    const bool cok = c < C;
    Vec<W> tt[A][A];
#pragma unroll
    for (int b = 0; b < A; ++b) {
      const int xx = t.rx + g.d * (MT * t.tx + b - 1);
      const bool xok = cok && (unsigned)xx < (unsigned)g.W;
      Vec<W> col[A], o[A];
#pragma unroll
      for (int a = 0; a < A; ++a) {
        const int yy = t.ry + g.d * (MT * t.ty + a - 1);
        col[a] = (xok && (unsigned)yy < (unsigned)g.H) ? vload<W>(x + ((long)(t.n * g.H + yy) * g.W + xx) * xp + c) : vzero<W>();
      }
      mat_apply<MT, W_BT>(col, o);
#pragma unroll
      for (int a = 0; a < A; ++a) tt[a][b] = o[a];
    }
    float* out = V + (long)tile * Kp + c;
#pragma unroll
    for (int a = 0; a < A; ++a) {
      Vec<W> o[A];
      mat_apply<MT, W_BT>(tt[a], o);
#pragma unroll
      for (int b = 0; b < A; ++b) vstore<W>(out + (a * A + b) * plane, o[b]);
    }
  }
}

template <int MT, int W>
__global__ __launch_bounds__(256) void wino_output_kernel(const float* __restrict__ M, int Cout, const pm_wino_geom g, float* __restrict__ y, long yp,
                                                          const float* __restrict__ bias, const float* __restrict__ scale,
                                                          const float* __restrict__ shift, const float* __restrict__ residual, long rp, int relu) {
  constexpr int A = MT + 2;
  const unsigned cg = Cout / W;
  const unsigned total = (unsigned)g.tiles * cg;
  const long plane = g.tiles * (long)Cout;
  for (unsigned i = blockIdx.x * 256u + threadIdx.x; i < total; i += gridDim.x * 256u) {
    const unsigned tile = i / cg;
    const int c = (int)(i - tile * cg) * W;
    const TileId t = decode_tile(tile, g);
    const float* in = M + (long)tile * Cout + c;
    Vec<W> s[MT][A];
#pragma unroll
    for (int b = 0; b < A; ++b) {
      Vec<W> col[A], o[MT];
#pragma unroll
      for (int a = 0; a < A; ++a) col[a] = vload<W>(in + (a * A + b) * plane);
      mat_apply<MT, W_AT>(col, o);
#pragma unroll
      for (int a = 0; a < MT; ++a) s[a][b] = o[a];
    }
    Vec<W> bi = vzero<W>(), sc = vzero<W>(), sh = vzero<W>();
    if (bias) bi = vload<W>(bias + c);
    if (scale) sc = vload<W>(scale + c), sh = vload<W>(shift + c);
#pragma unroll
    for (int a = 0; a < MT; ++a) {
      const int yy = t.ry + g.d * (MT * t.ty + a);
      Vec<W> o[MT];
      mat_apply<MT, W_AT>(s[a], o);
#pragma unroll
      for (int b = 0; b < MT; ++b) {
        const int xx = t.rx + g.d * (MT * t.tx + b);
        if (yy >= g.H || xx >= g.W) continue;
        const long pix = (long)(t.n * g.H + yy) * g.W + xx;
        Vec<W> v = o[b];
        if (bias) {
#pragma unroll
          for (int q = 0; q < W; ++q) v.v[q] += bi.v[q];
        }
        if (scale) {
#pragma unroll
          for (int q = 0; q < W; ++q) v.v[q] = v.v[q] * sc.v[q] + sh.v[q];
        }
        if (residual) {
          const Vec<W> rr = vload<W>(residual + pix * rp + c);
#pragma unroll
          for (int q = 0; q < W; ++q) v.v[q] += rr.v[q];
        }
        if (relu) {
#pragma unroll
          for (int q = 0; q < W; ++q) v.v[q] = fmaxf(v.v[q], 0.f);
        }
        vstore<W>(y + pix * yp + c, v);
      }
    }
  }
}

template <int MT, bool DGRAD>
__device__ __forceinline__ void wino_filter_block(const float* __restrict__ w, int Cout, int Cin, int Kp, float* __restrict__ U, int bx, int by,
                                                  float (*sg)[32][33]) {
  constexpr int A = MT + 2;
  const int tx = threadIdx.x & 31, ty = threadIdx.x >> 5;
  const int R = DGRAD ? Cin : Cout;
  const int Kr = DGRAD ? Cout : Cin;
// ... 16 lines not shown
    Vec<4> col[3], o[A];
#pragma unroll
    for (int ky = 0; ky < 3; ++ky)
#pragma unroll
      for (int e = 0; e < 4; ++e) col[ky].v[e] = DGRAD ? sg[(2 - ky) * 3 + (2 - kx)][4 * q + e][j] : sg[ky * 3 + kx][j][4 * q + e];
    mat_apply<MT, W_G>(col, o);
#pragma unroll
    for (int a = 0; a < A; ++a) gg[a][kx] = o[a];
  }
  float* out = U + (long)row * Kp + k;
#pragma unroll
  for (int a = 0; a < A; ++a) {
    Vec<4> o[A];
    mat_apply<MT, W_G>(gg[a], o);
#pragma unroll
    for (int b = 0; b < A; ++b) {
#pragma unroll
      for (int e = 0; e < 4; ++e)
        if (k + e >= Kr) o[b].v[e] = 0.f;
      vstore<4>(out + (a * A + b) * plane, o[b]);
    }
  }
}
template <int MT, bool DGRAD>
__global__ __launch_bounds__(256) void wino_filter_kernel(const float* __restrict__ w, int Cout, int Cin, int Kp, float* __restrict__ U) {
  __shared__ float sg[9][32][33];
  wino_filter_block<MT, DGRAD>(w, Cout, Cin, Kp, U, blockIdx.x, blockIdx.y, sg);
}

constexpr int WR_BATCH = 48;
struct WinoRefreshJobs {
  const float* w[WR_BATCH];
  float* U[WR_BATCH];
  int cout[WR_BATCH], cin[WR_BATCH], kp[WR_BATCH], m[WR_BATCH];
  int start[WR_BATCH + 1];
  int n;
};
__global__ __launch_bounds__(256) void wino_filter_multi_kernel(const WinoRefreshJobs t) {
  __shared__ float sg[9][32][33];
  int j = 0;
  while (j + 1 < t.n && (int)blockIdx.x >= t.start[j + 1]) ++j;
  const int local = (int)blockIdx.x - t.start[j];
  const int nbx = t.kp[j] / 32;
  const int bx = local % nbx, by = local / nbx;
  if (t.m[j] == 4) wino_filter_block<4, false>(t.w[j], t.cout[j], t.cin[j], t.kp[j], t.U[j], bx, by, sg);
  else wino_filter_block<2, false>(t.w[j], t.cout[j], t.cin[j], t.kp[j], t.U[j], bx, by, sg);
}

template <int MT, int W>
__global__ __launch_bounds__(256) void wino_dy_kernel(const float* __restrict__ dy, long yp, int Cout, const pm_wino_geom g, float* __restrict__ Z) {
  constexpr int A = MT + 2;
  const unsigned cg = Cout / W;
  const unsigned total = (unsigned)g.tiles * cg;
  const long plane = g.tiles * (long)Cout;
  for (unsigned i = blockIdx.x * 256u + threadIdx.x; i < total; i += gridDim.x * 256u) {
    const unsigned tile = i / cg;
    const int c = (int)(i - tile * cg) * W;
    const TileId t = decode_tile(tile, g);
    Vec<W> r[A][MT];
#pragma unroll
    for (int b = 0; b < MT; ++b) {
      const int xx = t.rx + g.d * (MT * t.tx + b);
      Vec<W> col[MT], o[A];
#pragma unroll
      for (int a = 0; a < MT; ++a) {
        const int yy = t.ry + g.d * (MT * t.ty + a);
        col[a] = (yy < g.H && xx < g.W) ? vload<W>(dy + ((long)(t.n * g.H + yy) * g.W + xx) * yp + c) : vzero<W>();
      }
      mat_apply<MT, W_A>(col, o);
#pragma unroll
      for (int a = 0; a < A; ++a) r[a][b] = o[a];
    }
    float* out = Z + (long)tile * Cout + c;
#pragma unroll
    for (int a = 0; a < A; ++a) {
      Vec<W> o[A];
      mat_apply<MT, W_A>(r[a], o);
#pragma unroll
      for (int b = 0; b < A; ++b) vstore<W>(out + (a * A + b) * plane, o[b]);
    }
  }
}

template <int MT>
__global__ __launch_bounds__(256) void wino_dw_kernel(const float* __restrict__ slab, int ks, int Cout, int Cin, int Kp, float* __restrict__ dw) {
  constexpr int A = MT + 2, P = A * A;
  const long total = (long)Cout * Cin, plane = (long)Cout * Kp;
  for (long i = (long)blockIdx.x * 256 + threadIdx.x; i < total; i += (long)gridDim.x * 256) {
    const int co = (int)(i / Cin), ci = (int)(i - (long)co * Cin);
    const float* in = slab + (long)co * Kp + ci;
    float du[P];
#pragma unroll
    for (int q = 0; q < P; ++q) du[q] = 0.f;
    for (int z = 0; z < ks; ++z) {
      float ld[P];
#pragma unroll
      for (int q = 0; q < P; ++q) ld[q] = in[((long)z * P + q) * plane];
#pragma unroll
      for (int q = 0; q < P; ++q) du[q] += ld[q];
    }
    Vec<1> h[3][A];
#pragma unroll
    for (int b = 0; b < A; ++b) {
      Vec<1> col[A], o[3];
#pragma unroll
      for (int a = 0; a < A; ++a) col[a].v[0] = du[a * A + b];
      mat_apply<MT, W_GT>(col, o);
#pragma unroll
      for (int k = 0; k < 3; ++k) h[k][b] = o[k];
    }
    float* out = dw + (long)co * 9 * Cin + ci;
#pragma unroll
    for (int k = 0; k < 3; ++k) {
      Vec<1> o[3];
      mat_apply<MT, W_GT>(h[k], o);
#pragma unroll
      for (int l = 0; l < 3; ++l) out[(k * 3 + l) * (long)Cin] = o[l].v[0];
    }
  }
}

typedef float f32x16 __attribute__((ext_vector_type(16)));

struct WinoFusedArgs {
  const float* V;
  const float* U;
  float* y;
  long yp;
  int Cout, Kp;
  pm_wino_geom g;
  const float* bias;
  const float* scale;
  const float* shift;
  const float* residual;
  long rp;
  int relu;
  int ncb;
};

constexpr int WF_THREADS = 768, WF_TB = 32, WF_CB = 32, WF_BK = 16, WF_P = 36;
constexpr size_t WF_LDS = (size_t)WF_P * WF_TB * (WF_CB + 1) * sizeof(float);

__device__ __forceinline__ int wf_xcd_remap(int bid, int nwg) {
  const int q = nwg >> 3, r = nwg & 7, xcd = bid & 7, idx = bid >> 3;
  const int base = xcd < r ? xcd * (q + 1) : r * (q + 1) + (xcd - r) * q;
  return base + idx;
}

__global__ __launch_bounds__(WF_THREADS) void wino_fused_f4_kernel(const WinoFusedArgs a) {
  extern __shared__ __align__(16) float4 lds4[];
  const int tid = threadIdx.x, lane = tid & 63, wave = tid >> 6;
  const int lid = wf_xcd_remap(blockIdx.x, gridDim.x);
  const int tb = lid / a.ncb, cb = lid - tb * a.ncb;
  const long tile0 = (long)tb * WF_TB;
  const int co0 = cb * WF_CB;

  const int rem = tid & 255, row = rem >> 2, chunk = rem & 3, pgrp = tid >> 8;
  const bool is_a = row < WF_TB;
  bool valid;
  const float* gp;
  long plane;
  if (is_a) {
    const long tile = tile0 + row;
    valid = tile < a.g.tiles;
    gp = a.V + (valid ? tile : 0) * a.Kp + chunk * 4;
    plane = a.g.tiles * (long)a.Kp;
// ... 34 lines not shown
      acc[j] = __builtin_amdgcn_mfma_f32_32x32x2f32(a0.y, b0.y, acc[j], 0, 0, 0);
      acc[j] = __builtin_amdgcn_mfma_f32_32x32x2f32(a0.z, b0.z, acc[j], 0, 0, 0);
      acc[j] = __builtin_amdgcn_mfma_f32_32x32x2f32(a0.w, b0.w, acc[j], 0, 0, 0);
      acc[j] = __builtin_amdgcn_mfma_f32_32x32x2f32(a1.x, b1.x, acc[j], 0, 0, 0);
      acc[j] = __builtin_amdgcn_mfma_f32_32x32x2f32(a1.y, b1.y, acc[j], 0, 0, 0);
      acc[j] = __builtin_amdgcn_mfma_f32_32x32x2f32(a1.z, b1.z, acc[j], 0, 0, 0);
      acc[j] = __builtin_amdgcn_mfma_f32_32x32x2f32(a1.w, b1.w, acc[j], 0, 0, 0);
    }
  };

  const int nk = a.Kp / WF_BK;
  gload(0);
  lstore();
  __syncthreads();
  for (int kt = 0; kt < nk; ++kt) {
    if (kt + 1 < nk) gload((kt + 1) * WF_BK);
    compute();
    __syncthreads();
    if (kt + 1 < nk) {
      lstore();
      __syncthreads();
    }
  }

  float* Ms = reinterpret_cast<float*>(lds4);
#pragma unroll
  for (int j = 0; j < 3; ++j) {
    const int pnt = wave * 3 + j;
#pragma unroll
    for (int q = 0; q < 16; ++q) Ms[(pnt * WF_TB + (q & 3) + 8 * (q >> 2) + 4 * half) * (WF_CB + 1) + l31] = acc[j][q];
  }
  __syncthreads();
  constexpr int MT = 4, A = 6;
  for (int idx = tid; idx < WF_TB * WF_CB; idx += WF_THREADS) {
    const int t = idx >> 5, c = idx & 31;
    const long tile = tile0 + t;
    const int co = co0 + c;
    if (tile >= a.g.tiles || co >= a.Cout) continue;
    const TileId ti = decode_tile((unsigned)tile, a.g);
    Vec<1> sv[MT][A];
#pragma unroll
    for (int b = 0; b < A; ++b) {
      Vec<1> col[A], o[MT];
#pragma unroll
      for (int aa = 0; aa < A; ++aa) col[aa].v[0] = Ms[((aa * A + b) * WF_TB + t) * (WF_CB + 1) + c];
      mat_apply<MT, W_AT>(col, o);
#pragma unroll
      for (int aa = 0; aa < MT; ++aa) sv[aa][b] = o[aa];
    }
    const float bi = a.bias ? a.bias[co] : 0.f, sc = a.scale ? a.scale[co] : 0.f, sh = a.scale ? a.shift[co] : 0.f;
#pragma unroll
    for (int aa = 0; aa < MT; ++aa) {
      const int yy = ti.ry + a.g.d * (MT * ti.ty + aa);
      Vec<1> o[MT];
      mat_apply<MT, W_AT>(sv[aa], o);
#pragma unroll
      for (int b = 0; b < MT; ++b) {
        const int xx = ti.rx + a.g.d * (MT * ti.tx + b);
        if (yy >= a.g.H || xx >= a.g.W) continue;
        const long pix = (long)(ti.n * a.g.H + yy) * a.g.W + xx;
        float v = o[b].v[0];
        if (a.bias) v += bi;
        if (a.scale) v = v * sc + sh;
        if (a.residual) v += a.residual[pix * a.rp + co];
        if (a.relu) v = fmaxf(v, 0.f);
        a.y[pix * a.yp + co] = v;
      }
    }
  }
}

inline unsigned nblocks(long total) { return (unsigned)std::min<long>((total + 255) / 256, 1 << 20); }

}

pm_wino_geom pm_wino_make_geom(int n, int h, int w, int d, int m) {
  pm_wino_geom g;
  g.N = n, g.H = h, g.W = w, g.d = d, g.m = m;
  g.TY = (pm_cdiv(h, d) + m - 1) / m, g.TX = (pm_cdiv(w, d) + m - 1) / m;
  g.tiles = (long)n * d * d * g.TY * g.TX;
  return g;
}

int pm_wino_input_xf(const float* x, long pitch, int C, int Kp, const pm_wino_geom& g, float* V, hipStream_t st) {
  if (g.m == 4) hipLaunchKernelGGL((wino_input_kernel<4, 2>), dim3(nblocks(g.tiles * (Kp / 2))), dim3(256), 0, st, x, pitch, C, Kp, g, V);
  else hipLaunchKernelGGL((wino_input_kernel<2, 4>), dim3(nblocks(g.tiles * (Kp / 4))), dim3(256), 0, st, x, pitch, C, Kp, g, V);
  return pm_check_launch("wino_input");
}

int pm_wino_filter_xf(const float* w, int Cout, int Cin, int Kp, bool dgrad, int m, float* U, hipStream_t st) {
  const int R = dgrad ? Cin : Cout;
  dim3 grid(Kp / 32, pm_cdiv(R, 32));
  if (m == 4) {
    if (dgrad) hipLaunchKernelGGL((wino_filter_kernel<4, true>), grid, dim3(256), 0, st, w, Cout, Cin, Kp, U);
    else hipLaunchKernelGGL((wino_filter_kernel<4, false>), grid, dim3(256), 0, st, w, Cout, Cin, Kp, U);
  } else {
    if (dgrad) hipLaunchKernelGGL((wino_filter_kernel<2, true>), grid, dim3(256), 0, st, w, Cout, Cin, Kp, U);
    else hipLaunchKernelGGL((wino_filter_kernel<2, false>), grid, dim3(256), 0, st, w, Cout, Cin, Kp, U);
  }
  return pm_check_launch("wino_filter");
}

int pm_wino_filter_xf_multi(const float* const* w, float* const* U, const int* cout, const int* cin, const int* kp, const int* m, int n, hipStream_t st) {
  for (int i0 = 0; i0 < n; i0 += WR_BATCH) {
    WinoRefreshJobs t;
    t.n = std::min(WR_BATCH, n - i0);
    long blocks = 0;
    for (int i = 0; i < t.n; ++i) {
      t.w[i] = w[i0 + i], t.U[i] = U[i0 + i], t.cout[i] = cout[i0 + i], t.cin[i] = cin[i0 + i], t.kp[i] = kp[i0 + i], t.m[i] = m[i0 + i];
      t.start[i] = (int)blocks;
      blocks += (long)(kp[i0 + i] / 32) * pm_cdiv(cout[i0 + i], 32);
    }
    t.start[t.n] = (int)blocks;
    if (blocks == 0) continue;
    hipLaunchKernelGGL(wino_filter_multi_kernel, dim3((unsigned)blocks), dim3(256), 0, st, t);
    if (int e = pm_check_launch("wino_filter_multi")) return e;
  }
  return PM_OK;
}

int pm_wino_output_xf(const float* M, int Cout, const pm_wino_geom& g, float* y, long ypitch, const float* bias, const float* scale, const float* shift,
                      const float* residual, long res_pitch, int relu, hipStream_t st) {
  if (g.m == 4)
    hipLaunchKernelGGL((wino_output_kernel<4, 2>), dim3(nblocks(g.tiles * (Cout / 2))), dim3(256), 0, st, M, Cout, g, y, ypitch, bias, scale, shift, residual,
                       res_pitch, relu);
  else
    hipLaunchKernelGGL((wino_output_kernel<2, 4>), dim3(nblocks(g.tiles * (Cout / 4))), dim3(256), 0, st, M, Cout, g, y, ypitch, bias, scale, shift, residual,
                       res_pitch, relu);
  return pm_check_launch("wino_output");
}

int pm_wino_dy_xf(const float* dy, long pitch, int Cout, const pm_wino_geom& g, float* Z, hipStream_t st) {
  if (g.m == 4) hipLaunchKernelGGL((wino_dy_kernel<4, 2>), dim3(nblocks(g.tiles * (Cout / 2))), dim3(256), 0, st, dy, pitch, Cout, g, Z);
  else hipLaunchKernelGGL((wino_dy_kernel<2, 4>), dim3(nblocks(g.tiles * (Cout / 4))), dim3(256), 0, st, dy, pitch, Cout, g, Z);
  return pm_check_launch("wino_dy");
}

int pm_wino_dw_xf(const float* slab, int ks, int Cout, int Cin, int Kp, int m, float* dw, hipStream_t st) {
  const unsigned nb = (unsigned)std::min<long>(((long)Cout * Cin + 255) / 256, 1 << 16);
  if (m == 4) hipLaunchKernelGGL(wino_dw_kernel<4>, dim3(nb), dim3(256), 0, st, slab, ks, Cout, Cin, Kp, dw);
  else hipLaunchKernelGGL(wino_dw_kernel<2>, dim3(nb), dim3(256), 0, st, slab, ks, Cout, Cin, Kp, dw);
  return pm_check_launch("wino_dw");
}

int pm_wino_fused_f4(const float* V, const float* U, int Cout, int Kp, const pm_wino_geom& g, float* y, long ypitch, const float* bias, const float* scale,
                     const float* shift, const float* residual, long res_pitch, int relu, hipStream_t st) {
  static pm_lds_optin optin;
  (void)optin(reinterpret_cast<const void*>(&wino_fused_f4_kernel), (int)WF_LDS);
  WinoFusedArgs a;
  a.V = V, a.U = U, a.y = y, a.yp = ypitch, a.Cout = Cout, a.Kp = Kp, a.g = g;
  a.bias = bias, a.scale = scale, a.shift = shift, a.residual = residual, a.rp = res_pitch, a.relu = relu;
  a.ncb = (Cout + WF_CB - 1) / WF_CB;
  const long ntb = (g.tiles + WF_TB - 1) / WF_TB;
  hipLaunchKernelGGL(wino_fused_f4_kernel, dim3((unsigned)(ntb * a.ncb)), dim3(WF_THREADS), WF_LDS, st, a);
  return pm_check_launch("wino_fused_f4");
}
```

pinthememory_amd/hip/kernels.py:

```python
import ctypes
from ctypes import byref

import os

import torch

from . import lib as L
from .lib import PmConvEpilogue, PmConvParams, check, ptr, stream, tdesc, workspace


def _lib():
    return L.load()


CONV_PREC = 0
ACT_DTYPE = torch.float32


def set_conv_precision(name):
    global CONV_PREC, ACT_DTYPE
    CONV_PREC = {'f32': 0, 'fp32': 0, 'bf16': 2, 'bf16_operands': 2, 'bf16_staged': 1}[name]
    ACT_DTYPE = torch.bfloat16 if name == 'bf16' else torch.float32


# ... 100 lines not shown
    if ent is None:
        for k in [k for k, e in _U_CACHE.items() if isinstance(e[0], weakref.ref) and e[0]() is None]:
            _evict(_U_CACHE.pop(k))
        while _U_CACHE and (len(_U_CACHE) >= _U_CACHE_MAX or sum(e[2].numel() * 4 for e in _U_CACHE.values()) + nbu > _U_CACHE_BYTES):
            _evict(_U_CACHE.pop(next(iter(_U_CACHE))))
        ent = [weakref.ref(owner) if owner is not None else w_krsc, -1, torch.empty(nbu // 4, dtype=torch.float32, device=w_krsc.device), None, None, True]
    ent[5] = True
    version = (owner if owner is not None else w_krsc)._version
    valid = ent[1] == version
    if not valid:
        ent[1] = -1
    _U_CACHE[key] = ent
    p.wxf, p.wxf_bytes, p.wxf_valid = ent[2].data_ptr(), nbu, 1 if valid else 0
    raw = stream()
    if raw not in _U_STREAMS:
        _U_STREAMS[raw] = L.stream_obj()
    if valid and ent[3] is not None and ent[4] != raw:
        _U_STREAMS[raw].wait_event(ent[3])
    return None if valid else (ent, version)


def forget_filter_events():
    for ent in _U_CACHE.values():
        ent[3] = ent[4] = None


WXF_REFRESH = os.environ.get('PM_WXF_REFRESH', '1') != '0'


def refresh_bf16_filters():
    if CONV_PREC != 2 or KEEP_WINOGRAD_U is False or not _U_CACHE or not WXF_REFRESH:
        return 0
    import weakref
    dev = torch.cuda.current_device()
    todo = []
    for key, ent in _U_CACHE.items():
        if key[4] != 2 or key[3] != dev or not ent[5]:
            continue
        ent[5] = False
        owner = ent[0]() if isinstance(ent[0], weakref.ref) else ent[0]
        if owner is None or owner.data_ptr() != key[0] or ent[1] == owner._version or not ent[2].is_cuda:
            continue
        todo.append((key, ent, owner))
    if not todo:
        return 0
    jobs = (L.PmWxfJob * len(todo))()
    for j, (key, ent, owner) in zip(jobs, todo):
        cout, kh, kw, cin = key[1]
        j.w, j.wxf, j.wxf_bytes, j.cout, j.kh, j.kw, j.cin, j.dgrad = key[0], ent[2].data_ptr(), key[2], cout, kh, kw, cin, 1 if key[5] else 0
        ent[1] = -1
    check(_lib().pm_conv_wxf_refresh_bf16(jobs, len(todo), stream()), 'pm_conv_wxf_refresh_bf16')
    cur = L.stream_obj()
    raw = cur.cuda_stream
    if raw not in _U_STREAMS:
        _U_STREAMS[raw] = cur
    ev = cur.record_event()
    for key, ent, owner in todo:
        ent[1], ent[3], ent[4] = owner._version, ev, raw
    return len(todo)


_SIZES = {}
_GEN = [0]


def _sizes(key, fn):
    v = _SIZES.get(key)
    if v is None:
        if len(_SIZES) > 8192:
            _SIZES.clear()
        v = _SIZES[key] = fn()
    return v


_XFORM_COUNT = [0, False]


def filter_transform_count(enable=None):
    if enable is not None:
        _XFORM_COUNT[1] = bool(enable)
    return _XFORM_COUNT[0]


def conv_fwd(x, w_krsc, stride, pad, dil, bias=None, scale=None, shift=None, residual=None, relu=False, out=None, keep_v=None, bn_partials=None, out_dtype=None):
    cout, kh, kw, cin = w_krsc.shape
    n, h, w_, c = x.shape
    assert c == cin, 'conv: Cin mismatch %d vs %d' % (c, cin)
    ho, wo = conv_out_hw(h, w_, kh, stride, pad, dil)
    y = out if out is not None else new((n, ho, wo, cout), x, pitch_pad=True, dtype=out_dtype if out_dtype is not None else ACT_DTYPE)
    assert residual is None or residual.dtype == y.dtype, 'conv_fwd: the fused residual has the dtype of the output'
    xd, yd = tdesc(x), tdesc(y)
    p = L.conv_params(kh, kw, stride, pad, dil, CONV_PREC)
    lib = _lib()
    nbv, nbu, nb, npb = _sizes(('f', x.shape, x.stride(), x.dtype, xd.flags, w_krsc.shape, y.stride(), y.dtype, stride, pad, dil, CONV_PREC, _GEN[0]),
                               lambda: (lib.pm_conv_winograd_v_bytes(byref(xd), byref(yd), byref(p)), lib.pm_conv_wxf_bytes(byref(xd), byref(yd), byref(p)),
                                        lib.pm_conv_workspace(byref(xd), byref(yd), byref(p), 0), lib.pm_conv_bn_partials_bytes(byref(xd), byref(yd), byref(p))))
    if keep_v is not None:
        nbv = nbv if KEEP_WINOGRAD_V else 0
        v = torch.empty(nbv // 4, dtype=torch.float32, device=x.device) if nbv else None
        keep_v.append(v)
        if v is not None:
            p.wino_v, p.wino_v_bytes = v.data_ptr(), nbv
    u_ent = None
    if (kh == 3 and CONV_PREC == 0) or CONV_PREC == 2:
        u_ent = _wino_u(p, w_krsc, nbu)
    if _XFORM_COUNT[1] and p.wxf_valid == 0 and nbu:
        _XFORM_COUNT[0] += 1
    ws = workspace(nb, x.device) if nb else None
    part = None
    if bn_partials is not None:
        ep16 = BN_EPILOGUE16 or (BN_EP16_MIN_BYTES > 0 and y.numel() * 2 >= BN_EP16_MIN_BYTES)
        ep32 = BN_EPILOGUE or (BN_EP_MIN_BYTES > 0 and y.numel() * 4 >= BN_EP_MIN_BYTES)
        npb = npb if ((ep16 if y.dtype == torch.bfloat16 else ep32) and residual is None and not relu and scale is None) else 0
        part = torch.empty(npb // 4, dtype=torch.float32, device=x.device) if npb else None
        bn_partials.append(part)
    ep = None
    if bias is not None or scale is not None or residual is not None or relu or part is not None:
        rd = tdesc(residual) if residual is not None else None
        ep = L.conv_epilogue(ptr(bias), ptr(scale), ptr(shift), rd.ptr if rd else None, rd.pitch if rd else 0, 1 if relu else 0, ptr(part),
                            part.numel() * 4 if part is not None else 0)
    check(lib.pm_conv_fwd(byref(xd), w_krsc.data_ptr(), byref(yd), byref(p), byref(ep) if ep else None, ptr(ws), nb, stream()), 'pm_conv_fwd')
    if u_ent is not None:
        ent, version = u_ent
        cur = L.stream_obj()
        ent[3], ent[4] = cur.record_event(), cur.cuda_stream
        ent[1] = version
    return y


def conv_bwd_data(dy, w_krsc, x_shape, stride, pad, dil, add=None, dtype=None):
    cout, kh, kw, cin = w_krsc.shape
    dx = new(x_shape, dy, dtype=dtype)
    dyd, dxd = tdesc(dy), tdesc(dx)
    p = L.conv_params(kh, kw, stride, pad, dil, CONV_PREC)
    lib = _lib()
    nb, nbu = _sizes(('d', dy.shape, dy.stride(), dy.dtype, dyd.flags, w_krsc.shape, dx.shape, dx.stride(), dx.dtype, stride, pad, dil, CONV_PREC, _GEN[0]),
                     lambda: (lib.pm_conv_workspace(byref(dxd), byref(dyd), byref(p), 1), lib.pm_conv_wxf_bytes_dgrad(byref(dyd), byref(dxd), byref(p))))
    ws = workspace(nb, dy.device) if nb else None
    ad = tdesc(add) if add is not None else None
    u_ent = _wino_u(p, w_krsc, nbu, dgrad=True) if CONV_PREC == 2 else None
    check(lib.pm_conv_bwd_data(byref(dyd), w_krsc.data_ptr(), byref(dxd), byref(p), byref(ad) if ad else None, ptr(ws), nb, stream()), 'pm_conv_bwd_data')
    if u_ent is not None:
        ent, version = u_ent
        cur = L.stream_obj()
        ent[3], ent[4] = cur.record_event(), cur.cuda_stream
        ent[1] = version
    return dx


def conv_bwd_weight(x, dy, w_shape_krsc, stride, pad, dil, want_bias=False, wino_v=None, on_stream=None):
    cout, kh, kw, cin = w_shape_krsc
    dw = torch.empty(w_shape_krsc, dtype=torch.float32, device=x.device)
    db = torch.empty(cout, dtype=torch.float32, device=x.device) if want_bias else None
    xd, dyd = tdesc(x), tdesc(dy)
    p = L.conv_params(kh, kw, stride, pad, dil, CONV_PREC)
    if wino_v is not None:
        p.wino_v, p.wino_v_bytes = wino_v.data_ptr(), wino_v.numel() * 4
    lib = _lib()
    nb = _sizes(('w', x.shape, x.stride(), x.dtype, dy.shape, dy.stride(), dy.dtype, w_shape_krsc, stride, pad, dil, CONV_PREC, wino_v is not None, _GEN[0]),
                lambda: lib.pm_conv_workspace(byref(xd), byref(dyd), byref(p), 2))
    raw = stream() if on_stream is None else on_stream.cuda_stream
    ws = workspace(nb, x.device, on_stream)
    check(lib.pm_conv_bwd_weight(byref(xd), byref(dyd), dw.data_ptr(), ptr(db), byref(p), ptr(ws), nb, raw), 'pm_conv_bwd_weight')
    return dw, db


def bn_stats(x):
    c = x.shape[3]
    mom = torch.empty(3 * c, dtype=torch.float32, device=x.device)
    xd = tdesc(x)
    lib = _lib()
    nb = _sizes(('bn', x.shape, x.dtype), lambda: lib.pm_bn_workspace(byref(xd)))
    ws = workspace(nb, x.device)
    check(lib.pm_bn_stats(byref(xd), mom.data_ptr(), ptr(ws), nb, stream()), 'pm_bn_stats')
    return mom


def bn_stats_finalize(x, eps, running_mean=None, running_var=None, momentum=0.1):
    c = x.shape[3]
    mean = torch.empty(c, dtype=torch.float32, device=x.device)
    invstd = torch.empty_like(mean)
    xd = tdesc(x)
    lib = _lib()
    nb = _sizes(('bn', x.shape, x.dtype), lambda: lib.pm_bn_workspace(byref(xd)))
    ws = workspace(nb, x.device)
    check(lib.pm_bn_stats_finalize(byref(xd), eps, mean.data_ptr(), invstd.data_ptr(), ptr(running_mean), ptr(running_var), momentum, ptr(ws), nb, stream()),
          'pm_bn_stats_finalize')
    return mean, invstd


def bn_partials_finalize(part, pixels, c, eps, running_mean=None, running_var=None, momentum=0.1):
    mean = torch.empty(c, dtype=torch.float32, device=part.device)
    invstd = torch.empty_like(mean)
    check(_lib().pm_bn_partials_finalize(part.data_ptr(), pixels, c, eps, mean.data_ptr(), invstd.data_ptr(), ptr(running_mean), ptr(running_var), momentum, None,
                                         stream()), 'pm_bn_partials_finalize')
    return mean, invstd


def bn_partials_moments(part, pixels, c):
    mom = torch.empty(3 * c, dtype=torch.float32, device=part.device)
    check(_lib().pm_bn_partials_finalize(part.data_ptr(), pixels, c, 0.0, None, None, None, None, 0.0, mom.data_ptr(), stream()), 'pm_bn_partials_finalize')
    return mom


def bn_merge(parts, world, c):
    out = torch.empty(3 * c, dtype=torch.float32, device=parts.device)
    check(_lib().pm_bn_merge(parts.data_ptr(), world, c, out.data_ptr(), stream()), 'pm_bn_merge')
    return out


def bn_merge_finalize(parts, world, c, eps, running_mean=None, running_var=None, momentum=0.1):
    mean = torch.empty(c, dtype=torch.float32, device=parts.device)
    invstd = torch.empty_like(mean)
    check(_lib().pm_bn_merge_finalize(parts.data_ptr(), world, c, eps, mean.data_ptr(), invstd.data_ptr(), ptr(running_mean), ptr(running_var), momentum,
                                      stream()), 'pm_bn_merge_finalize')
    return mean, invstd


def bn_finalize(moments, c, eps, running_mean=None, running_var=None, momentum=0.1):
    mean = torch.empty(c, dtype=torch.float32, device=moments.device)
    invstd = torch.empty_like(mean)
    check(_lib().pm_bn_finalize(moments.data_ptr(), c, eps, mean.data_ptr(), invstd.data_ptr(), ptr(running_mean), ptr(running_var), momentum, stream()),
          'pm_bn_finalize')
    return mean, invstd


def bn_fold_multi(table, cs, offs, n, max_c, total, eps):
    arena = torch.empty(2 * total, dtype=torch.float32, device=table.device)
    check(_lib().pm_bn_fold_multi(table.data_ptr(), cs.data_ptr(), offs.data_ptr(), n, max_c, total, eps, arena.data_ptr(), stream()), 'pm_bn_fold_multi')
    return arena


def bn_fold(gamma, beta, running_mean, running_var, eps, conv_bias=None):
    c = gamma.numel()
    scale = torch.empty(c, dtype=torch.float32, device=gamma.device)
    shift = torch.empty_like(scale)
    check(_lib().pm_bn_fold(gamma.data_ptr(), beta.data_ptr(), running_mean.data_ptr(), running_var.data_ptr(), ptr(conv_bias), c, eps, scale.data_ptr(),
                            shift.data_ptr(), stream()), 'pm_bn_fold')
    return scale, shift


def bn_apply(x, mean, invstd, gamma, beta, residual=None, relu=False, out=None, want_mask=False):
    y = out if out is not None else torch.empty_like(x, memory_format=torch.contiguous_format)
    rd = tdesc(residual) if residual is not None else None
    grp = 8 if x.dtype == torch.bfloat16 else 4
    mask = torch.empty((x.shape[0] * x.shape[1] * x.shape[2], x.shape[3] // grp), dtype=torch.uint8, device=x.device) if want_mask else None
    check(_lib().pm_bn_apply_mask(byref(tdesc(x)), mean.data_ptr(), invstd.data_ptr(), gamma.data_ptr(), beta.data_ptr(), byref(rd) if rd else None,
                                  1 if relu else 0, byref(tdesc(y)), ptr(mask), stream()), 'pm_bn_apply_mask')
    return (y, mask) if want_mask else y


def bn_bwd_reduce_mask(dy, mask, x, mean, invstd, want_gmask=True, with_count=False):
    c = x.shape[3]
    sums = torch.empty(2 * c + (1 if with_count else 0), dtype=torch.float32, device=x.device)
    if with_count:
        sums[2 * c:].fill_(float(x.shape[0] * x.shape[1] * x.shape[2]))
    xd = tdesc(x)
    lib = _lib()
    nb = _sizes(('bn', x.shape, x.dtype), lambda: lib.pm_bn_workspace(byref(xd)))
    ws = workspace(nb, x.device)
    gm = torch.empty(x.shape, dtype=x.dtype, device=x.device) if want_gmask else None
    gd = tdesc(gm) if want_gmask else None
    check(lib.pm_bn_bwd_reduce_mask(byref(tdesc(dy)), mask.data_ptr(), byref(xd), mean.data_ptr(), invstd.data_ptr(), byref(gd) if gd else None,
                                    sums.data_ptr(), ptr(ws), nb, stream()), 'pm_bn_bwd_reduce_mask')
    return sums, gm


def scale_shift_act(x, scale, shift, residual=None, relu=False):
    y = torch.empty(x.shape, dtype=torch.float32, device=x.device)
    rd = tdesc(residual) if residual is not None else None
    check(_lib().pm_scale_shift_act(byref(tdesc(x)), scale.data_ptr(), shift.data_ptr(), byref(rd) if rd else None, 1 if relu else 0, byref(tdesc(y)), stream()),
          'pm_scale_shift_act')
    return y


def bn_bwd_reduce(dy, y, x, mean, invstd, relu, gamma=None, beta=None, want_gmask=False, with_count=False):
    relu = int(relu)
    c = x.shape[3]
    sums = torch.empty(2 * c + (1 if with_count else 0), dtype=torch.float32, device=x.device)
    if with_count:
        sums[2 * c:].fill_(float(x.shape[0] * x.shape[1] * x.shape[2]))
    xd = tdesc(x)
    lib = _lib()
    nb = _sizes(('bn', x.shape, x.dtype), lambda: lib.pm_bn_workspace(byref(xd)))
    ws = workspace(nb, x.device)
    yd = tdesc(y) if relu == 1 else None
    gm = torch.empty(x.shape, dtype=x.dtype, device=x.device) if want_gmask else None
    gd = tdesc(gm) if want_gmask else None
    check(lib.pm_bn_bwd_reduce(byref(tdesc(dy)), byref(yd) if yd else None, byref(xd), mean.data_ptr(), invstd.data_ptr(), ptr(gamma), ptr(beta), relu,
                               byref(gd) if gd else None, sums.data_ptr(), ptr(ws), nb, stream()), 'pm_bn_bwd_reduce')
    return sums, gm


def bn_bwd_apply(dy, y, x, mean, invstd, gamma, sums, count, relu, want_dres, beta=None):
    relu = int(relu)
    dx = torch.empty(x.shape, dtype=x.dtype, device=x.device)
    dres = torch.empty(x.shape, dtype=x.dtype, device=x.device) if want_dres else None
    yd = tdesc(y) if relu == 1 else None
    dr = tdesc(dres) if want_dres else None
    check(_lib().pm_bn_bwd_apply(byref(tdesc(dy)), byref(yd) if yd else None, byref(tdesc(x)), mean.data_ptr(), invstd.data_ptr(), gamma.data_ptr(),
                                 ptr(beta), sums.data_ptr(), float(count), relu, byref(tdesc(dx)), byref(dr) if dr else None, stream()), 'pm_bn_bwd_apply')
    return dx, dres


def relu_bwd(dy, y):
    dx = torch.empty(y.shape, dtype=torch.float32, device=y.device)
    check(_lib().pm_relu_bwd(byref(tdesc(dy)), byref(tdesc(y)), byref(tdesc(dx)), stream()), 'pm_relu_bwd')
    return dx


def add_n(xs):
    from .lib import PmTensor
    from ctypes import POINTER, pointer
    descs = [tdesc(x) for x in xs]
    arr = (POINTER(PmTensor) * len(xs))(*[pointer(d) for d in descs])
    y = torch.empty(xs[0].shape, dtype=xs[0].dtype, device=xs[0].device)
    check(_lib().pm_add_n(arr, len(xs), byref(tdesc(y)), stream()), 'pm_add_n')
    return y


def add(a, b, out=None):
    y = out if out is not None else torch.empty(a.shape, dtype=a.dtype, device=a.device)
    check(_lib().pm_add(byref(tdesc(a)), byref(tdesc(b)), byref(tdesc(y)), stream()), 'pm_add')
    return y


def copy(src, dst):
    check(_lib().pm_copy(byref(tdesc(src)), byref(tdesc(dst)), stream()), 'pm_copy')
    return dst


def maxpool_fwd(x):
    n, h, w, c = x.shape
    y = torch.empty((n, (h - 1) // 2 + 1, (w - 1) // 2 + 1, c), dtype=x.dtype, device=x.device)
    arg = torch.empty(y.shape, dtype=torch.uint8, device=x.device)
    check(_lib().pm_maxpool3x3s2_fwd(byref(tdesc(x)), byref(tdesc(y)), arg.data_ptr(), stream()), 'pm_maxpool3x3s2_fwd')
    return y, arg


def maxpool_bwd(dy, arg, x_shape):
    dx = torch.empty(x_shape, dtype=dy.dtype, device=dy.device)
    check(_lib().pm_maxpool3x3s2_bwd(byref(tdesc(dy)), arg.data_ptr(), byref(tdesc(dx)), stream()), 'pm_maxpool3x3s2_bwd')
    return dx


def global_avgpool_fwd(x):
    n, h, w, c = x.shape
    y = torch.empty((n, 1, 1, c), dtype=x.dtype, device=x.device)
    check(_lib().pm_global_avgpool_fwd(byref(tdesc(x)), byref(tdesc(y)), stream()), 'pm_global_avgpool_fwd')
    return y


def global_avgpool_bwd(dy, x_shape):
    dx = torch.empty(x_shape, dtype=dy.dtype, device=dy.device)
    check(_lib().pm_global_avgpool_bwd(byref(tdesc(dy)), byref(tdesc(dx)), 0, stream()), 'pm_global_avgpool_bwd')
    return dx


def resize_fwd(x, size, out=None):
    n, h, w, c = x.shape
    own_pad = c % 4 != 0 and x.stride(2) == (c + 3) // 4 * 4
    y = out if out is not None else new((n, size[0], size[1], c), x, pitch_pad=True, zero_pad=not own_pad)
    check(_lib().pm_resize_bilinear_fwd(byref(tdesc(x)), byref(tdesc(y)), stream()), 'pm_resize_bilinear_fwd')
    return y


RESIZE_SEPARABLE = os.environ.get('PM_RESIZE_SEP', '1') == '1'


def resize_bwd(dy, x_shape, separable=None):
    separable = RESIZE_SEPARABLE if separable is None else separable
    dx = new(x_shape, dy, pitch_pad=True)
    lib, dyd, dxd = _lib(), tdesc(dy), tdesc(dx)
    nb = lib.pm_resize_bilinear_bwd_workspace(byref(dyd), byref(dxd)) if separable else 0
    if nb:
        ws = workspace(nb, dy.device)
        check(lib.pm_resize_bilinear_bwd_separable(byref(dyd), byref(dxd), 0, ptr(ws), nb, stream()), 'pm_resize_bilinear_bwd_separable')
    else:
        check(lib.pm_resize_bilinear_bwd(byref(dyd), byref(dxd), 0, stream()), 'pm_resize_bilinear_bwd')
    return dx


def resize_hp_fwd(x, size, flip_w=False):
    n, h, w, c = x.shape
    y = torch.empty((n, size[0], size[1], c), dtype=torch.float32, device=x.device)
# ... 310 lines not shown
```

pinthememory_amd/hip/lib.py:

```python
import ctypes
import os
from ctypes import POINTER, byref, c_char_p, c_float, c_int, c_int32, c_int64, c_size_t, c_void_p

import torch

_HERE = os.path.dirname(os.path.dirname(os.path.abspath(__file__)))
LIB_PATH = os.environ.get('PM_LIB') or os.path.join(_HERE, 'libpinmem_hip.so')


class PmTensor(ctypes.Structure):
    _fields_ = [('ptr', c_void_p), ('n', c_int32), ('h', c_int32), ('w', c_int32), ('c', c_int32), ('pitch', c_int64), ('dtype', c_int32), ('flags', c_int32)]


PM_F32, PM_BF16 = 0, 1
PM_TF_ZERO_PAD64 = 1


class PmSgdEntry(ctypes.Structure):
    _fields_ = [('param', c_void_p), ('grad', c_void_p), ('momentum_buffer', c_void_p), ('numel', c_int64)]


class PmWxfJob(ctypes.Structure):
    _fields_ = [('w', c_void_p), ('wxf', c_void_p), ('wxf_bytes', c_int64), ('cout', c_int32), ('kh', c_int32), ('kw', c_int32), ('cin', c_int32),
                ('dgrad', c_int32), ('reserved', c_int32)]


class PmConvParams(ctypes.Structure):
    _fields_ = [('struct_size', c_int32), ('kh', c_int32), ('kw', c_int32), ('stride', c_int32), ('pad', c_int32), ('dil', c_int32), ('prec', c_int32),
                ('wino_v', c_void_p), ('wino_v_bytes', c_int64),
                ('wxf', c_void_p), ('wxf_bytes', c_int64), ('wxf_valid', c_int32)]


class PmRouting(ctypes.Structure):
    _fields_ = [('struct_size', c_int32), ('winograd', c_int32), ('winograd_fused', c_int32), ('conv16', c_int32), ('conv16_wide', c_int32),
                ('conv16_persistent', c_int32), ('wgrad16', c_int32), ('bf16_wgrad', c_int32), ('split', c_int32)]


class PmConvEpilogue(ctypes.Structure):
    _fields_ = [('struct_size', c_int64), ('bias', c_void_p), ('scale', c_void_p), ('shift', c_void_p), ('residual', c_void_p),
                ('residual_pitch', c_int64), ('relu', c_int32), ('bn_partials', c_void_p), ('bn_partials_bytes', c_int64)]


def conv_params(kh, kw, stride, pad, dil, prec=0):
    return PmConvParams(ctypes.sizeof(PmConvParams), kh, kw, stride, pad, dil, prec)


def conv_epilogue(*fields):
    return PmConvEpilogue(ctypes.sizeof(PmConvEpilogue), *fields)


ABI_VERSION = 400


class PinmemError(RuntimeError):
    pass


_T, _P, _E = POINTER(PmTensor), POINTER(PmConvParams), POINTER(PmConvEpilogue)
_vp, _sz, _i, _f, _i64 = c_void_p, c_size_t, c_int, c_float, c_int64

SIGNATURES = {
    'pm_last_error': (c_char_p, []),
    'pm_version': (c_int, []),
    'pm_conv_winograd_v_bytes': (_sz, [_T, _T, _P]),
    'pm_conv_wxf_bytes': (_sz, [_T, _T, _P]),
    'pm_conv_wxf_bytes_dgrad': (_sz, [_T, _T, _P]),
    'pm_conv_wxf_refresh_bf16': (_i, [_vp, _i, _vp]),
    'pm_conv_wxf_refresh_f32': (_i, [_vp, _i, _vp]),
    'pm_conv_workspace': (_sz, [_T, _T, _P, _i]),
    'pm_conv_fwd': (_i, [_T, _vp, _T, _P, _E, _vp, _sz, _vp]),
    'pm_conv_bwd_data': (_i, [_T, _vp, _T, _P, _T, _vp, _sz, _vp]),
    'pm_conv_bwd_weight': (_i, [_T, _T, _vp, _vp, _P, _vp, _sz, _vp]),
    'pm_set_winograd': (_i, [_i]),
    'pm_set_winograd_fused': (_i, [_i]),
    'pm_set_conv16': (_i, [_i]),
    'pm_profile_enable': (_i, [_i]),
    'pm_profile_dump': (_i, [ctypes.c_char_p]),
    'pm_profile_read': (_i, [_i, _i, _i, _i, _i, POINTER(ctypes.c_double), POINTER(ctypes.c_double), POINTER(c_int64), _i]),
    'pm_profile_read_prec': (_i, [_i, _i, _i, _i, _i, _i, POINTER(ctypes.c_double), POINTER(ctypes.c_double), POINTER(c_int64), _i]),
    'pm_profile_read_bytes': (_i, [_i, _i, _i, _i, _i, _i, POINTER(ctypes.c_double)]),
    'pm_bn_workspace': (_sz, [_T]),
    'pm_bn_stats': (_i, [_T, _vp, _vp, _sz, _vp]),
    'pm_bn_merge': (_i, [_vp, _i, _i, _vp, _vp]),
    'pm_bn_merge_finalize': (_i, [_vp, _i, _i, _f, _vp, _vp, _vp, _vp, _f, _vp]),
    'pm_bn_finalize': (_i, [_vp, _i, _f, _vp, _vp, _vp, _vp, _f, _vp]),
    'pm_bn_stats_finalize': (_i, [_T, _f, _vp, _vp, _vp, _vp, _f, _vp, _sz, _vp]),
    'pm_bn_fold': (_i, [_vp, _vp, _vp, _vp, _vp, _i, _f, _vp, _vp, _vp]),
    'pm_bn_fold_multi': (_i, [_vp, _vp, _vp, _i, _i, _i, _f, _vp, _vp]),
    'pm_bn_apply': (_i, [_T, _vp, _vp, _vp, _vp, _T, _i, _T, _vp]),
    'pm_bn_apply_mask': (_i, [_T, _vp, _vp, _vp, _vp, _T, _i, _T, _vp, _vp]),
    'pm_bn_bwd_reduce_mask': (_i, [_T, _vp, _T, _vp, _vp, _T, _vp, _vp, _sz, _vp]),
    'pm_bn_bwd_reduce': (_i, [_T, _T, _T, _vp, _vp, _vp, _vp, _i, _T, _vp, _vp, _sz, _vp]),
    'pm_bn_bwd_apply': (_i, [_T, _T, _T, _vp, _vp, _vp, _vp, _vp, _f, _i, _T, _T, _vp]),
    'pm_relu_bwd': (_i, [_T, _T, _T, _vp]),
    'pm_add': (_i, [_T, _T, _T, _vp]),
    'pm_add_n': (_i, [POINTER(_T), _i, _T, _vp]),
    'pm_copy': (_i, [_T, _T, _vp]),
    'pm_scale_shift_act': (_i, [_T, _vp, _vp, _T, _i, _T, _vp]),
    'pm_maxpool3x3s2_fwd': (_i, [_T, _T, _vp, _vp]),
    'pm_maxpool3x3s2_bwd': (_i, [_T, _vp, _T, _vp]),
    'pm_global_avgpool_fwd': (_i, [_T, _T, _vp]),
    'pm_global_avgpool_bwd': (_i, [_T, _T, _i, _vp]),
    'pm_resize_bilinear_fwd': (_i, [_T, _T, _vp]),
    'pm_resize_bilinear_bwd': (_i, [_T, _T, _i, _vp]),
    'pm_resize_bilinear_bwd_workspace': (_sz, [_T, _T]),
    'pm_resize_bilinear_bwd_separable': (_i, [_T, _T, _i, _vp, _sz, _vp]),
    'pm_resize_bilinear_hp_fwd': (_i, [_T, _T, _i, _vp]),
    'pm_softmax_mean_update': (_i, [_T, _vp, _i, _vp]),
    'pm_sliding_stitch': (_i, [_T, _vp, _i, _i, _i, _i, _vp, _i, _vp]),
    'pm_argmax_f64': (_i, [_vp, _i, _i, _i, _i, _vp, _vp, _vp]),
    'pm_image_u8_to_nhwc4': (_i, [_vp, _i64, POINTER(c_float), POINTER(c_float), _vp, _vp]),
    'pm_labels_u8_to_i64': (_i, [_vp, _i64, _vp, _vp]),
    'pm_nchw_to_nhwc': (_i, [_vp, _i, _T, _vp]),
    'pm_nhwc_to_nchw': (_i, [_T, _vp, _vp]),
    'pm_label_nearest': (_i, [_vp, _i, _i, _i, _vp, _i, _i, _vp]),
    'pm_upsample_ce_workspace': (_sz, [_i, _i, _i]),
    'pm_upsample_ce_fwd': (_i, [_T, _f, _vp, _i, _i, _vp, _vp, _sz, _vp]),
    'pm_upsample_ce_bwd_workspace': (_sz, [_T, _i, _i]),
    'pm_upsample_ce_bwd': (_i, [_T, _f, _vp, _i, _i, _vp, _vp, _T, _vp, _sz, _vp]),
    'pm_upsample_ce_field_bytes': (_sz, [_T, _i, _i]),
    'pm_upsample_ce_fwd_field': (_i, [_T, _f, _vp, _i, _i, _vp, _vp, _vp, _sz, _vp]),
    'pm_upsample_ce_bwd_field': (_i, [_T, _f, _i, _i, _vp, _vp, _vp, _T, _vp]),
    'pm_mem_read_fwd': (_i, [_T, _vp, _i, _vp, _T, _vp, _vp, _vp]),
    'pm_mem_read_fwd_pq_workspace': (_sz, [_i64, _i]),
    'pm_mem_read_fwd_pq': (_i, [_T, _vp, _i, _vp, _vp, _T, _vp, _vp, _vp, _vp, _sz, _vp]),
    'pm_mem_colsoftmax_workspace': (_sz, [_i64, _i]),
    'pm_mem_colsoftmax': (_i, [_vp, _vp, _i64, _i, _vp, _vp, _sz, _vp]),
    'pm_mem_read_bwd_workspace': (_sz, [_i64, _i, _i]),
    'pm_mem_read_bwd': (_i, [_T, _vp, _i, _vp, _T, _vp, _T, _vp, _vp, _sz, _vp]),
    'pm_mem_write_accum_workspace': (_sz, [_T, _i]),
    'pm_mem_write_accum': (_i, [_T, _vp, _i, _i, _i, _i, _vp, _vp, _sz, _vp]),
    'pm_mem_write_accum_bwd': (_i, [_T, _vp, _i, _i, _i, _i, _vp, _T, _vp]),
    'pm_mem_write_update': (_i, [_vp, _vp, _i, _i, _f, _vp, _vp, _vp]),
    'pm_mem_write_update_bwd': (_i, [_vp, _vp, _i, _i, _f, _vp, _vp, _vp, _vp]),
    'pm_sgd_momentum': (_i, [_vp, _vp, _vp, _i64, _f, _f, _f, _i, _vp]),
    'pm_set_bf16_wgrad': (_i, [_i]),
    'pm_set_wgrad16': (_i, [_i]),
    'pm_set_split': (_i, [_i]),
    'pm_routing_get': (_i, [POINTER(PmRouting)]),
    'pm_routing_set': (_i, [POINTER(PmRouting)]),
    'pm_conv_bn_partials_bytes': (_sz, [_T, _T, POINTER(PmConvParams)]),
    'pm_bn_partials_finalize': (_i, [_vp, _i64, _i, _f, _vp, _vp, _vp, _vp, _f, _vp, _vp]),
    'pm_sgd_momentum_multi': (_i, [_vp, _i, _f, _f, _f, _vp]),
    'pm_sgd_momentum_multi_dev': (_i, [_vp, _i, _f, _vp, _f, _f, _vp]),
    'pm_cast': (_i, [_T, _T, _vp]),
}

_lib = None


def load():
    global _lib
    if _lib is not None:
        return _lib
    if not os.environ.get('PM_LIB'):
        from .. import build as _build
        _build.build()
    lib = ctypes.CDLL(LIB_PATH)
    for name, (res, args) in SIGNATURES.items():
        fn = getattr(lib, name)
        fn.restype, fn.argtypes = res, args
    if lib.pm_version() != ABI_VERSION:
        raise PinmemError('%s reports ABI %d, this binding is written against %d (include/pinmem_hip.h)' % (LIB_PATH, lib.pm_version(), ABI_VERSION))
    _lib = lib
    return lib


def check(code, what=''):
    if code != 0:
        raise PinmemError('%s failed (%d): %s' % (what, code, load().pm_last_error().decode()))


_raw_stream = torch._C._cuda_getCurrentRawStream
_cur_device = torch._C._cuda_getDevice


# ... 70 lines not shown
```

pinthememory_amd/hip/ops.py:

```python
import os as _os

import torch

from . import kernels as K
from . import lib as L
from .. import dist as D


def nhwc(t):
    v = t.permute(0, 2, 3, 1)
    n, h, w, c = v.shape
    sn, sh, sw, sc = v.stride()
    pitch = sw if w > 1 else (sh if h > 1 else (sn if n > 1 else c))
    ok = (sc == 1 or c == 1) and pitch >= c and (h == 1 or w == 1 or sh == w * pitch) and (n == 1 or h * w == 1 or sn == h * w * pitch)
    if ok and v.dtype == torch.float32:
        return v
    if v.dtype == torch.bfloat16:
        if ok and pitch % 8 == 0 and c % 8 == 0 and v.data_ptr() % 16 == 0:
            return v
        return v.contiguous()
    if h * w == 1:
        return v.contiguous().float()
    return K.nchw_to_nhwc(t.float())

# ... 24 lines not shown


_nbt_pending = []


def flush_bn_counters():
    if _nbt_pending:
        torch._foreach_add_(_nbt_pending, 1)
        _nbt_pending.clear()


_OVERLAP_ENV = _os.environ.get('PM_OVERLAP_WGRAD')
OVERLAP_WGRAD = True if _OVERLAP_ENV is None else _OVERLAP_ENV == '1'


def overlap_wgrad():
    if not OVERLAP_WGRAD:
        return False
    return not (_OVERLAP_ENV is None and K.CONV_PREC == 2 and K.ACT_DTYPE == torch.bfloat16)


_side = {}
_proxy = {}


def masked_stream(n_cus, device=None, first=0):
    import ctypes
    dev = torch.cuda.current_device() if device is None else device
    total = torch.cuda.get_device_properties(dev).multi_processor_count
    n_cus = max(1, min(int(n_cus), total))
    words = (total + 31) // 32
    mask = (ctypes.c_uint32 * words)()
    picked = {(first + (i * total) // n_cus) % total for i in range(n_cus)}
    for cu in picked:
        mask[cu // 32] |= 1 << (cu % 32)
    hip = ctypes.CDLL('libamdhip64.so')
    st = ctypes.c_void_p()
    with torch.cuda.device(dev):
        err = hip.hipExtStreamCreateWithCUMask(ctypes.byref(st), ctypes.c_uint32(words), mask)
    if err != 0 or not st.value:
        raise RuntimeError('hipExtStreamCreateWithCUMask(%d CUs) failed: %d' % (n_cus, err))
    return torch.cuda.ExternalStream(st.value, device=dev)


WGRAD_CUS = int(_os.environ.get('PM_WGRAD_CUS', '0'))


def _side_stream():
    dev = torch.cuda.current_device()
    if dev not in _side:
        _side[dev] = masked_stream(WGRAD_CUS, dev) if WGRAD_CUS > 0 else torch.cuda.Stream(device=dev)
    return _side[dev]


class _Defer(torch.autograd.Function):
    @staticmethod
    def forward(ctx, w):
        return w.view_as(w)

    @staticmethod
    def backward(ctx, g):
        L.stream_obj().wait_stream(_side_stream())
        return g


def begin_forward():
    flush_bn_counters()
    _proxy.clear()


def defer_weights(module):
    if not (overlap_wgrad() and torch.is_grad_enabled()):
        return
    for m in module.modules():
        if isinstance(m, torch.nn.Conv2d) and m.bias is None and m.weight.requires_grad and id(m.weight) not in _proxy:
            _proxy[id(m.weight)] = _Defer.apply(m.weight)


def _w(weight):
    p = _proxy.get(id(weight))
    return (p, True) if p is not None else (weight, False)


def _wgrad(x, dy, wshape, geom, want_bias=False, deferred=False, wino_v=None):
    if not deferred:
        return K.conv_bwd_weight(x, dy, wshape, *geom, want_bias=want_bias, wino_v=wino_v)
    side, main = _side_stream(), L.stream_obj()
    ev = torch.cuda.Event()
    ev.record(main)
    side.wait_event(ev)
    out = K.conv_bwd_weight(x, dy, wshape, *geom, want_bias=want_bias, wino_v=wino_v, on_stream=side)
    if wino_v is not None:
        wino_v.record_stream(side)
    x.record_stream(side)
    dy.record_stream(side)
    for t in out:
        if t is not None:
            t.record_stream(side)
    return out


commit_done = {}


def wait_commit():
    if not commit_done or not torch.cuda.is_available():
        return
    ev = commit_done.pop(torch.cuda.current_device(), None)
    if ev is not None:
        torch.cuda.current_stream().wait_event(ev)


BN_FUSED_FINALIZE = _os.environ.get('PM_BN_FUSED', '1') == '1'


RELU_MASK_BYTES = _os.environ.get('PM_BN_MASK', '1') == '1'


MERGE_SYNCBN = _os.environ.get('PM_MERGE_SYNCBN', '1') == '1'


def _bn_train_stats_multi(ys, bns, partials):
    c = ys[0].shape[3]
    moms = []
    for y, part in zip(ys, partials):
        pixels = y.shape[0] * y.shape[1] * y.shape[2]
        moms.append(K.bn_partials_moments(part, pixels, c) if part is not None else K.bn_stats(y))
    n = len(ys)
    flat, world = D.gather_moments(torch.cat(moms), bns[0].group)
    parts = flat.view(world, n, 3 * c)
    return [K.bn_merge_finalize(parts[:, i].contiguous().view(-1), world, c, bn.eps, bn.running_mean, bn.running_var, bn.momentum) for i, bn in enumerate(bns)]


def _mergeable(bns, ys):
    return (MERGE_SYNCBN and BN_FUSED_FINALIZE and D.is_dist() and len(bns) > 1 and all(b.group is not None and b.group is bns[0].group for b in bns)
            and len({y.shape[3] for y in ys}) == 1)


def _bn_train_fwd(y, gamma, beta, bn, residual, relu, out=None, partials=None, want_mask=False):
    c = y.shape[3]
    pixels = y.shape[0] * y.shape[1] * y.shape[2]
    if bn.group is None and BN_FUSED_FINALIZE:
        if partials is not None:
            mean, invstd = K.bn_partials_finalize(partials, pixels, c, bn.eps, bn.running_mean, bn.running_var, bn.momentum)
        else:
            mean, invstd = K.bn_stats_finalize(y, bn.eps, bn.running_mean, bn.running_var, bn.momentum)
    elif bn.group is not None and D.is_dist() and BN_FUSED_FINALIZE:
        mom = K.bn_partials_moments(partials, pixels, c) if partials is not None else K.bn_stats(y)
        flat, world = D.gather_moments(mom, bn.group)
        mean, invstd = K.bn_merge_finalize(flat, world, c, bn.eps, bn.running_mean, bn.running_var, bn.momentum)
    else:
        mom = K.bn_partials_moments(partials, pixels, c) if partials is not None else K.bn_stats(y)
        if bn.group is not None:
            mom = D.merge_moments(mom, c, bn.group)
        mean, invstd = K.bn_finalize(mom, c, bn.eps, bn.running_mean, bn.running_var, bn.momentum)
    if want_mask:
        o, mask = K.bn_apply(y, mean, invstd, gamma, beta, residual=residual, relu=relu, out=out, want_mask=True)
        return o, mean, invstd, mask
    return K.bn_apply(y, mean, invstd, gamma, beta, residual=residual, relu=relu, out=out), mean, invstd


def _bn_train_bwd(dv, o, y, mean, invstd, gamma, beta, relu, group, want_dres, has_res, mask=None):
    c = y.shape[3]
    mode = 0 if not relu else (1 if has_res else 2)
    hand_over = mode == 1 and want_dres
    if hand_over and mask is not None:
        sums, gm = K.bn_bwd_reduce_mask(dv, mask, y, mean, invstd, want_gmask=True, with_count=group is not None)
    else:
        sums, gm = K.bn_bwd_reduce(dv, o, y, mean, invstd, mode, gamma, beta, want_gmask=hand_over, with_count=group is not None)
    local = sums
    if group is not None:
        sums = D.all_reduce_sum_copy(local, group)
    count = float(y.shape[0] * y.shape[1] * y.shape[2]) if group is None else -1.0
    if hand_over:
        dy, _ = K.bn_bwd_apply(gm, None, y, mean, invstd, gamma, sums, count, 0, False)
        dres = gm
    else:
        dy, dres = K.bn_bwd_apply(dv, o, y, mean, invstd, gamma, sums, count, mode, want_dres, beta)
    return dy, dres, local[c:2 * c], local[:c]


class _Bottleneck(torch.autograd.Function):

    @staticmethod
    def forward(ctx, x, w1, g1, b1, w2, g2, b2, w3, g3, b3, wd, gd, bd, geoms, bns, deferred):
        xv = nhwc(x)
        k1, k2, k3 = K.krsc(w1), K.krsc(w2), K.krsc(w3)
        ps = []
        y1 = K.conv_fwd(xv, k1, *geoms[0], bn_partials=ps)
        o1, m1, i1 = _bn_train_fwd(y1, g1, b1, bns[0], None, True, partials=ps[0])
        kv = []
        y2 = K.conv_fwd(o1, k2, *geoms[1], keep_v=kv, bn_partials=ps)
        o2, m2, i2 = _bn_train_fwd(y2, g2, b2, bns[1], None, True, partials=ps[1])
        y3 = K.conv_fwd(o2, k3, *geoms[2], bn_partials=ps)
        merged = False
        if wd is not None:
            kd = K.krsc(wd)
            yd = K.conv_fwd(xv, kd, *geoms[3], bn_partials=ps)
            merged = _mergeable([bns[3], bns[2]], [yd, y3])
            if merged:
                (md, idd), (m3, i3) = _bn_train_stats_multi([yd, y3], [bns[3], bns[2]], [ps[3], ps[2]])
                res = K.bn_apply(yd, md, idd, gd, bd, residual=None, relu=False)
            else:
                res, md, idd = _bn_train_fwd(yd, gd, bd, bns[3], None, False, partials=ps[3])
        else:
            kd = yd = md = idd = None
            res = xv
        if merged:
            out, mask3 = K.bn_apply(y3, m3, i3, g3, b3, residual=res, relu=True, want_mask=True) if RELU_MASK_BYTES else (K.bn_apply(y3, m3, i3, g3, b3, residual=res, relu=True), None)
        elif RELU_MASK_BYTES:
            out, m3, i3, mask3 = _bn_train_fwd(y3, g3, b3, bns[2], res, True, partials=ps[2], want_mask=True)
        else:
            (out, m3, i3), mask3 = _bn_train_fwd(y3, g3, b3, bns[2], res, True, partials=ps[2]), None
        ctx.geoms, ctx.groups, ctx.has_ds, ctx.deferred = geoms, [b.group for b in bns], wd is not None, deferred
        ctx.save_for_backward(xv, k1, k2, k3, kd, y1, o1, y2, o2, y3, yd, out, m1, i1, m2, i2, m3, i3, md, idd, g1, g2, g3, gd, b1, b2, b3, kv[0], mask3)
        return nchw(out)

    @staticmethod
    def backward(ctx, dout):
        xv, k1, k2, k3, kd, y1, o1, y2, o2, y3, yd, out, m1, i1, m2, i2, m3, i3, md, idd, g1, g2, g3, gd, b1, b2, b3, v2, mask3 = ctx.saved_tensors
        ge, gr, df = ctx.geoms, ctx.groups, ctx.deferred
        dv = _grad_view(dout)
        pair = None
        if ctx.has_ds and MERGE_SYNCBN and D.is_dist() and gr[2] is not None and gr[3] is gr[2] and y3.shape[3] == yd.shape[3]:
            c3 = y3.shape[3]
            if mask3 is not None:
                s3, gm = K.bn_bwd_reduce_mask(dv, mask3, y3, m3, i3, want_gmask=True, with_count=True)
            else:
                s3, gm = K.bn_bwd_reduce(dv, out, y3, m3, i3, 1, g3, b3, want_gmask=True, with_count=True)
            sd, _ = K.bn_bwd_reduce(gm, None, yd, md, idd, 0, gd, None, want_gmask=False, with_count=True)
            both = D.all_reduce_sum_copy(torch.cat([s3, sd]), gr[2])
            g3sum, gdsum = both[:s3.numel()], both[s3.numel():]
            dy3, _ = K.bn_bwd_apply(gm, None, y3, m3, i3, g3, g3sum, -1.0, 0, False)
            dres, dg3, db3 = gm, s3[c3:2 * c3], s3[:c3]
            dyd, _ = K.bn_bwd_apply(gm, None, yd, md, idd, gd, gdsum, -1.0, 0, False, None)
            pair = (dyd, sd[c3:2 * c3], sd[:c3])
        else:
            dy3, dres, dg3, db3 = _bn_train_bwd(dv, out, y3, m3, i3, g3, b3, True, gr[2], True, True, mask=mask3)
        dw3, _ = _wgrad(o2, dy3, tuple(k3.shape), ge[2], deferred=df[2])
        do2 = K.conv_bwd_data(dy3, k3, tuple(o2.shape), *ge[2])
        dy2, _, dg2, db2 = _bn_train_bwd(do2, o2, y2, m2, i2, g2, b2, True, gr[1], False, False)
        dw2, _ = _wgrad(o1, dy2, tuple(k2.shape), ge[1], deferred=df[1], wino_v=v2)
        do1 = K.conv_bwd_data(dy2, k2, tuple(o1.shape), *ge[1])
        dy1, _, dg1, db1 = _bn_train_bwd(do1, o1, y1, m1, i1, g1, b1, True, gr[0], False, False)
        dw1, _ = _wgrad(xv, dy1, tuple(k1.shape), ge[0], deferred=df[0])
        dwd = dgd = dbd = None
        skip = dres
        if ctx.has_ds:
            if pair is not None:
                dyd, dgd, dbd = pair
            else:
                dyd, _, dgd, dbd = _bn_train_bwd(dres, None, yd, md, idd, gd, None, False, gr[3], False, False)
            dwdk, _ = _wgrad(xv, dyd, tuple(kd.shape), ge[3], deferred=df[3])
            dwd = dwdk.permute(0, 3, 1, 2)
            skip = K.conv_bwd_data(dyd, kd, tuple(xv.shape), *ge[3]) if ctx.needs_input_grad[0] else None
        dx = nchw(K.conv_bwd_data(dy1, k1, tuple(xv.shape), *ge[0], add=skip)) if ctx.needs_input_grad[0] else None
        p = lambda d: d.permute(0, 3, 1, 2)
        return dx, p(dw1), dg1, db1, p(dw2), dg2, db2, p(dw3), dg3, db3, dwd, dgd, dbd, None, None, None


FOLD_BATCH = _os.environ.get('PM_FOLD_BATCH', '1') == '1'
_fold_cache = None
fold_misses = 0
last_prefold_event = None


class prefold:
    def __init__(self, model):
        self.model, self.active = model, False

    def __enter__(self):
        global _fold_cache, last_prefold_event
        last_prefold_event = None
        m = self.model
        if not FOLD_BATCH or m.training or torch.is_grad_enabled() or _fold_cache is not None:
            return self
        bns = getattr(m, '_pm_bn_list', None)
        if bns is None:
            bns = [b for b in m.modules() if isinstance(b, torch.nn.modules.batchnorm._BatchNorm)]
            m.__dict__['_pm_bn_list'] = bns
        bns = [b for b in bns if b.running_mean is not None and b.weight is not None and b.running_mean.is_cuda and not b.training]
        if not bns or len({b.eps for b in bns}) != 1:
            return self
        ptrs = tuple(t.data_ptr() for b in bns for t in (b.weight, b.bias, b.running_mean, b.running_var))
        plan = m.__dict__.get('_pm_fold_plan')
        if plan is None or plan[0] != ptrs:
            dev = bns[0].running_mean.device
            cs = [b.num_features for b in bns]
            offs, tot = [], 0
            for c in cs:
                offs.append(tot)
                tot += (c + 3) // 4 * 4
            as_i64 = [p - (1 << 64) if p >= (1 << 63) else p for p in ptrs]
            plan = (ptrs, torch.tensor(as_i64, dtype=torch.int64, device=dev), torch.tensor(cs, dtype=torch.int32, device=dev),
                    torch.tensor(offs, dtype=torch.int32, device=dev), cs, offs, tot)
            m.__dict__['_pm_fold_plan'] = plan
        _, table, dcs, doffs, cs, offs, tot = plan
        arena = K.bn_fold_multi(table, dcs, doffs, len(cs), max(cs), tot, bns[0].eps)
        _fold_cache = {b.running_mean.data_ptr(): (arena[o:o + c], arena[tot + o:tot + o + c]) for b, c, o in zip(bns, cs, offs)}
        self.active = True
        last_prefold_event = torch.cuda.current_stream().record_event() if len(bns) == len(m.__dict__['_pm_bn_list']) else None
        return self

    def __exit__(self, *exc):
        global _fold_cache
        if self.active:
            _fold_cache = None
        return False


class _ConvBnAct(torch.autograd.Function):

    @staticmethod
    def forward(ctx, x, w, bias, gamma, beta, residual, geom, bn, relu, out, deferred=False):
        stride, pad, dil = geom
        xv, wk = nhwc(x), K.krsc(w)
        rv = nhwc(residual) if residual is not None else None
        ov = nhwc(out) if out is not None else None
        ctx.geom, ctx.relu, ctx.train, ctx.deferred = geom, relu, bn.training, deferred and bias is None
        needs_grad = bn.grad_enabled and any(ctx.needs_input_grad[:6])
        if not bn.training and not needs_grad:
            hit = _fold_cache.get(bn.running_mean.data_ptr()) if (_fold_cache is not None and bias is None) else None
            if hit is None:
                global fold_misses
                fold_misses += 1
            scale, shift = hit if hit is not None else K.bn_fold(gamma, beta, bn.running_mean, bn.running_var, bn.eps, bias)
            o = K.conv_fwd(xv, wk, stride, pad, dil, scale=scale, shift=shift, residual=rv, relu=relu, out=ov)
            return nchw(o)
        kv, ps = [], []
        y = K.conv_fwd(xv, wk, stride, pad, dil, bias=bias, keep_v=kv if ctx.needs_input_grad[1] else None, bn_partials=ps if bn.training else None)
        if bn.training:
            o, mean, invstd = _bn_train_fwd(y, gamma, beta, bn, rv, relu, ov, partials=ps[0])
        else:
            mean, invstd = bn.running_mean, torch.rsqrt(bn.running_var + bn.eps)
            o = K.bn_apply(y, mean, invstd, gamma, beta, residual=rv, relu=relu, out=ov)
        ctx.group, ctx.has_bias, ctx.has_res = bn.group, bias is not None, residual is not None
        ctx.save_for_backward(xv, wk, y, o, mean, invstd, gamma, beta, kv[0] if kv else None)
        return nchw(o)

    @staticmethod
    def backward(ctx, dout):
        xv, wk, y, o, mean, invstd, gamma, beta, vk = ctx.saved_tensors
        stride, pad, dil = ctx.geom
        dv = _grad_view(dout)
        want_dres = ctx.has_res and ctx.needs_input_grad[5]
        if ctx.train:
            dy, dres, dgamma, dbeta = _bn_train_bwd(dv, o, y, mean, invstd, gamma, beta, ctx.relu, ctx.group, want_dres, ctx.has_res)
        else:
            c = y.shape[3]
            mode = 0 if not ctx.relu else (1 if ctx.has_res else 2)
            sums, g = K.bn_bwd_reduce(dv, o, y, mean, invstd, mode, gamma, beta, want_gmask=mode != 0)
            g = dv if g is None else g
            dy = K.scale_shift_act(g, gamma * invstd, torch.zeros_like(gamma))
            dres, dgamma, dbeta = (g if want_dres else None), sums[c:], sums[:c]
        dx = nchw(K.conv_bwd_data(dy, wk, tuple(xv.shape), stride, pad, dil, dtype=xv.dtype)) if ctx.needs_input_grad[0] else None
        dw = db = None
        if ctx.needs_input_grad[1] or (ctx.has_bias and ctx.needs_input_grad[2]):
            dwk, db = _wgrad(xv, dy, tuple(wk.shape), (stride, pad, dil), want_bias=ctx.has_bias, deferred=ctx.deferred, wino_v=vk)
            dw = dwk.permute(0, 3, 1, 2)
        return dx, dw, db, dgamma, dbeta, (nchw(dres) if dres is not None else None), None, None, None, None, None


class _ConvBnActN(torch.autograd.Function):

    @staticmethod
    def forward(ctx, n, geoms, bns, outs, deferreds, *ts):
        xs, ws, gammas, betas = ts[0:n], ts[n:2 * n], ts[2 * n:3 * n], ts[3 * n:4 * n]
        xvs, wks = [nhwc(x) for x in xs], [K.krsc(w) for w in ws]
        ys, kvs, parts = [], [], []
        for i in range(n):
            kv, ps = [], []
            ys.append(K.conv_fwd(xvs[i], wks[i], *geoms[i], keep_v=kv if ctx.needs_input_grad[5 + n + i] else None, bn_partials=ps))
            kvs.append(kv[0] if kv else None)
            parts.append(ps[0])
        stats = _bn_train_stats_multi(ys, bns, parts)
        os_ = [K.bn_apply(ys[i], stats[i][0], stats[i][1], gammas[i], betas[i], residual=None, relu=True, out=nhwc(outs[i]) if outs[i] is not None else None) for i in range(n)]
        ctx.n, ctx.geoms, ctx.group, ctx.deferreds = n, geoms, bns[0].group, deferreds
        ctx.save_for_backward(*xvs, *wks, *ys, *os_, *[st[0] for st in stats], *[st[1] for st in stats], *gammas, *betas, *kvs)
        return tuple(nchw(o) for o in os_)

    @staticmethod
    def backward(ctx, *douts):
        n = ctx.n
        sv = ctx.saved_tensors
        xvs, wks, ys, os_, means, invs, gammas, betas, kvs = (sv[i * n:(i + 1) * n] for i in range(9))
        c = ys[0].shape[3]
        red = [K.bn_bwd_reduce(_grad_view(douts[i]), os_[i], ys[i], means[i], invs[i], 2, gammas[i], betas[i], want_gmask=False, with_count=True) for i in range(n)]
        tot = D.all_reduce_sum_copy(torch.cat([r[0] for r in red]), ctx.group)
        ln = red[0][0].numel()
        dxs, dws, dgs, dbs = [], [], [], []
        for i in range(n):
            dy, _ = K.bn_bwd_apply(_grad_view(douts[i]), os_[i], ys[i], means[i], invs[i], gammas[i], tot[i * ln:(i + 1) * ln], -1.0, 2, False, betas[i])
            dxs.append(nchw(K.conv_bwd_data(dy, wks[i], tuple(xvs[i].shape), *ctx.geoms[i], dtype=xvs[i].dtype)) if ctx.needs_input_grad[5 + i] else None)
            dwk, _ = _wgrad(xvs[i], dy, tuple(wks[i].shape), ctx.geoms[i], deferred=ctx.deferreds[i], wino_v=kvs[i])
            dws.append(dwk.permute(0, 3, 1, 2))
            dgs.append(red[i][0][c:2 * c]), dbs.append(red[i][0][:c])
        return (None, None, None, None, None, *dxs, *dws, *dgs, *dbs)


def conv_bn_act_n(xs, seqs, outs):
    convs, bns_m = [q[0] for q in seqs], [q[1] for q in seqs]
    ok = MERGE_SYNCBN and BN_FUSED_FINALIZE and D.is_dist() and torch.is_grad_enabled() and all(b.training for b in bns_m) and all(cv.bias is None for cv in convs)
    if ok:
        groups = [D.bn_group(b) for b in bns_m]
        ok = all(g is not None and g is groups[0] for g in groups) and len({cv.out_channels for cv in convs}) == 1
    if not ok:
        return [conv_bn_act(x, cv, bn, relu=True, out=o) for x, cv, bn, o in zip(xs, convs, bns_m, outs)]
    states = [BNState(b) for b in bns_m]
    wd = [_w(cv.weight) for cv in convs]
    n = len(xs)
    return list(_ConvBnActN.apply(n, [_geom(cv) for cv in convs], states, list(outs), [d for _, d in wd], *xs, *[w for w, _ in wd],
                                  *[b.weight for b in bns_m], *[b.bias for b in bns_m]))


class _Conv(torch.autograd.Function):

    @staticmethod
    def forward(ctx, x, w, bias, geom):
        stride, pad, dil = geom
        xv, wk = nhwc(x), K.krsc(w)
        y = K.conv_fwd(xv, wk, stride, pad, dil, bias=bias, out_dtype=torch.float32)
        ctx.geom, ctx.has_bias = geom, bias is not None
        ctx.save_for_backward(xv, wk)
        return nchw(y)

    @staticmethod
    def backward(ctx, dout):
        xv, wk = ctx.saved_tensors
# ... 282 lines not shown
```

Measured before the change: 155.6.

## Fold BatchNorm+ReLU into Winograd input transform for bottleneck 3x3 convs

In the bottleneck forward pass, the first BN+ReLU is applied inside the Winograd input-transform kernel of the 3x3 conv. This skips materialising the normalised activation o1 and removes one elementwise pass over memory. A backward path is also added that fuses BN backward with the Winograd dgrad and dy transforms, but it is disabled by default (FOLD_BN_WINO_BWD=False). The backward recomputes from y1 instead of storing o1, and the change adds ABI fields and extra routing conditions.

```diff
diff --git a/include/pinmem_hip.h b/include/pinmem_hip.h
--- a/include/pinmem_hip.h
+++ b/include/pinmem_hip.h
@@ -20,7 +20,7 @@
   int32_t flags;
 } pm_tensor;
 
-#define PM_ABI_VERSION 400
+#define PM_ABI_VERSION 401
 
 typedef struct pm_conv_params {
   int32_t struct_size;
@@ -31,6 +31,9 @@
   void* wxf;
   int64_t wxf_bytes;
   int32_t wxf_valid;
+  int32_t wino_v_valid;
+  void* wino_z;
+  int64_t wino_z_bytes;
 } pm_conv_params;
 
 typedef struct pm_conv_epilogue {
@@ -43,6 +46,10 @@
   int32_t relu;
   float* bn_partials;
   int64_t bn_partials_bytes;
+  const float* in_mean;
+  const float* in_invstd;
+  const float* in_gamma;
+  const float* in_beta;
 } pm_conv_epilogue;
 
 const char* pm_last_error(void);
@@ -65,6 +72,9 @@
 size_t pm_conv_bn_partials_bytes(const pm_tensor* x, const pm_tensor* y, const pm_conv_params* p);
 int pm_conv_fwd(const pm_tensor* x, const float* w_krsc, const pm_tensor* y, const pm_conv_params* p,
                 const pm_conv_epilogue* ep, void* ws, size_t ws_bytes, void* stream);
+int pm_bn_bwd_wino_bytes(const pm_tensor* y, int cin, const pm_conv_params* p, int64_t* v_bytes, int64_t* z_bytes);
+int pm_bn_bwd_wino(const pm_tensor* g, const pm_tensor* y, const float* mean, const float* invstd, const float* gamma, const float* beta, const float* sums,
+                   float count, int cin, const pm_conv_params* p, void* v, int64_t v_bytes, void* z, int64_t z_bytes, void* stream);
 int pm_conv_bwd_data(const pm_tensor* dy, const float* w_krsc, const pm_tensor* dx, const pm_conv_params* p,
                      const pm_tensor* add, void* ws, size_t ws_bytes, void* stream);
 int pm_conv_bwd_weight(const pm_tensor* x, const pm_tensor* dy, float* dw_krsc, float* dbias, const pm_conv_params* p,
diff --git a/pinthememory_amd/csrc/bn.hip b/pinthememory_amd/csrc/bn.hip
--- a/pinthememory_amd/csrc/bn.hip
+++ b/pinthememory_amd/csrc/bn.hip
@@ -1,14 +1,10 @@
 #include "pm_common.h"
+#include "bn_math.h"
 
 namespace {
 
 constexpr int CB = 64;
 constexpr int RL = 16;
-
-__device__ __forceinline__ float bn_affine(float v, float mu, float is, float ga, float be) {
-  const float s = is * ga;
-  return fmaf(v, s, fmaf(-mu, s, be));
-}
 
 inline int chunk_rows(long P, int C) {
   const long colblocks = std::max<long>(1, (C + CB - 1) / CB);
@@ -466,10 +462,10 @@
     if (pdr) PM_ST4(pdr + p * e2 + ch, g);
     const float4 s1 = PM_LD4(sums + ch), s2 = PM_LD4(sums + C + ch);
     float4 r;
-    r.x = (g.x - s1.x * inv_n - (v.x - mu.x) * is.x * (s2.x * inv_n)) * (is.x * ga.x);
-    r.y = (g.y - s1.y * inv_n - (v.y - mu.y) * is.y * (s2.y * inv_n)) * (is.y * ga.y);
-    r.z = (g.z - s1.z * inv_n - (v.z - mu.z) * is.z * (s2.z * inv_n)) * (is.z * ga.z);
-    r.w = (g.w - s1.w * inv_n - (v.w - mu.w) * is.w * (s2.w * inv_n)) * (is.w * ga.w);
+    r.x = bn_bwd_dx(g.x, v.x, mu.x, is.x, ga.x, s1.x, s2.x, inv_n);
+    r.y = bn_bwd_dx(g.y, v.y, mu.y, is.y, ga.y, s1.y, s2.y, inv_n);
+    r.z = bn_bwd_dx(g.z, v.z, mu.z, is.z, ga.z, s1.z, s2.z, inv_n);
+    r.w = bn_bwd_dx(g.w, v.w, mu.w, is.w, ga.w, s1.w, s2.w, inv_n);
     PM_ST4(pdx + p * d + ch, r);
   });
 }
diff --git a/pinthememory_amd/csrc/bn_math.h b/pinthememory_amd/csrc/bn_math.h
--- /dev/null
+++ b/pinthememory_amd/csrc/bn_math.h
@@ -0,0 +1,11 @@
+#pragma once
+#include <hip/hip_runtime.h>
+
+__device__ __forceinline__ float bn_affine(float v, float mu, float is, float ga, float be) {
+  const float s = is * ga;
+  return fmaf(v, s, fmaf(-mu, s, be));
+}
+
+__device__ __forceinline__ float bn_bwd_dx(float g, float v, float mu, float is, float ga, float s1, float s2, float inv_n) {
+  return fmaf(-((v - mu) * is), s2 * inv_n, fmaf(-s1, inv_n, g)) * (is * ga);
+}
diff --git a/pinthememory_amd/csrc/conv_igemm.hip b/pinthememory_amd/csrc/conv_igemm.hip
--- a/pinthememory_amd/csrc/conv_igemm.hip
+++ b/pinthememory_amd/csrc/conv_igemm.hip
@@ -481,12 +481,14 @@
 inline size_t wino_ws(const WinoPlan& wp) { return wp.v_bytes + wp.m_bytes + wp.u_bytes; }
 
 int wino_conv(const pm_tensor* xin, const float* w, int w_cout, int w_cin, bool dgrad, const pm_tensor* yout, const WinoPlan& wp,
-              const pm_conv_epilogue& ep, void* ws, hipStream_t st, float* v_keep = nullptr, float* u_ext = nullptr, bool u_valid = false) {
+              const pm_conv_epilogue& ep, void* ws, hipStream_t st, float* v_keep = nullptr, float* u_ext = nullptr, bool u_valid = false,
+              const pm_wino_bn* in_bn = nullptr, bool v_valid = false) {
   float* V = v_keep ? v_keep : (float*)ws;
   float* Mo = (float*)((char*)ws + wp.v_bytes);
   float* U = u_ext ? u_ext : (float*)((char*)ws + wp.v_bytes + wp.m_bytes);
   const int cout = yout->c;
-  if (int e = pm_wino_input_xf((const float*)xin->ptr, xin->pitch, xin->c, wp.Kp, wp.g, V, st)) return e;
+  if (!(v_keep && v_valid))
+    if (int e = pm_wino_input_xf((const float*)xin->ptr, xin->pitch, xin->c, wp.Kp, wp.g, V, st, in_bn)) return e;
   if (!(u_ext && u_valid))
     if (int e = pm_wino_filter_xf(w, w_cout, w_cin, wp.Kp, dgrad, wp.g.m, U, st)) return e;
   const pm_tensor xv = {V, 1, 1, (int32_t)wp.g.tiles, wp.Kp, wp.Kp};
@@ -539,14 +541,15 @@
 inline size_t wino_wgrad_ws(const WinoPlan& wp, const WinoWgradPlan& q) { return wp.v_bytes + wp.m_bytes + q.slab_bytes; }
 
 int wino_wgrad(const pm_tensor* x, const pm_tensor* dy, float* dw, const WinoPlan& wp, const WinoWgradPlan& q, void* ws, hipStream_t st,
-               float* v_kept = nullptr) {
+               float* v_kept = nullptr, float* z_kept = nullptr) {
   float* V = v_kept ? v_kept : (float*)ws;
-  float* Z = (float*)((char*)ws + wp.v_bytes);
+  float* Z = z_kept ? z_kept : (float*)((char*)ws + wp.v_bytes);
   float* slab = (float*)((char*)ws + wp.v_bytes + wp.m_bytes);
   const int cout = dy->c;
   if (!v_kept)
     if (int e = pm_wino_input_xf((const float*)x->ptr, x->pitch, x->c, wp.Kp, wp.g, V, st)) return e;
-  if (int e = pm_wino_dy_xf((const float*)dy->ptr, dy->pitch, cout, wp.g, Z, st)) return e;
+  if (!z_kept)
+    if (int e = pm_wino_dy_xf((const float*)dy->ptr, dy->pitch, cout, wp.g, Z, st)) return e;
   const pm_tensor xv = {V, 1, 1, (int32_t)wp.g.tiles, wp.Kp, wp.Kp};
   const pm_tensor zv = {Z, 1, 1, (int32_t)wp.g.tiles, cout, cout};
   const pm_conv_params p1 = {(int32_t)sizeof(pm_conv_params), 1, 1, 1, 0, 1, 0};
@@ -950,6 +953,48 @@
   return (f.use && g.use && f.g.m == g.g.m) ? f.v_bytes : 0;
 }
 
+struct BnWinoPlan {
+  WinoPlan dg, wg;
+  bool use;
+};
+static BnWinoPlan bn_wino_plan(const pm_tensor* y, int cin, const pm_conv_params* p0) {
+  BnWinoPlan b{};
+  if (!y || !p0 || p0->struct_size != (int32_t)sizeof(pm_conv_params) || !pm_is_f32(y) || cin <= 0) return b;
+  const pm_conv_params tp = tier_params(p0, y, y);
+  if (tp.prec != 0 || tp.stride != 1) return b;
+  pm_tensor x = *y;
+  x.c = cin, x.pitch = cin, x.ptr = nullptr;
+  b.dg = wino_plan(y, cin, &tp);
+  b.wg = wino_plan(&x, y->c, &tp, true);
+  const pm_wino_geom &a = b.dg.g, &c = b.wg.g;
+  b.use = b.dg.use && b.wg.use && a.m == c.m && a.tiles == c.tiles && a.TY == c.TY && a.TX == c.TX && a.d == c.d && b.dg.Kp % 4 == 0;
+  return b;
+}
+extern "C" int pm_bn_bwd_wino_bytes(const pm_tensor* y, int cin, const pm_conv_params* p, int64_t* v_bytes, int64_t* z_bytes) {
+  PM_REQUIRE(v_bytes && z_bytes, PM_EINVAL, "bn_bwd_wino_bytes: null");
+  *v_bytes = *z_bytes = 0;
+  const BnWinoPlan b = bn_wino_plan(y, cin, p);
+  if (!b.use) return PM_EUNSUPPORTED;
+  *v_bytes = (int64_t)b.dg.v_bytes, *z_bytes = (int64_t)b.wg.m_bytes;
+  return PM_OK;
+}
+extern "C" int pm_bn_bwd_wino(const pm_tensor* g, const pm_tensor* y, const float* mean, const float* invstd, const float* gamma, const float* beta, const float* sums,
+                              float count, int cin, const pm_conv_params* p, void* v, int64_t v_bytes, void* z, int64_t z_bytes, void* stream) {
+  PM_REQUIRE(g && y && p, PM_EINVAL, "bn_bwd_wino: null");
+  PM_REQUIRE(p->struct_size == (int32_t)sizeof(pm_conv_params), PM_EINVAL, "bn_wino_bwd: pm_conv_params.struct_size %d != %zu (library ABI %d)", p->struct_size,
+             sizeof(pm_conv_params), PM_ABI_VERSION);
+  PM_REQUIRE(pm_is_f32(g) && pm_is_f32(y) && pm_vec4(g) && pm_vec4(y) && pm_same_shape(g, y), PM_EINVAL,
+             "bn_bwd_wino: g and y fp32 of one shape, 16B aligned, pitch %% 4 == 0 and C %% 4 == 0");
+  PM_REQUIRE(mean && invstd && gamma && beta && sums, PM_EINVAL, "bn_bwd_wino: BatchNorm vectors missing");
+  const BnWinoPlan b = bn_wino_plan(y, cin, p);
+  PM_REQUIRE(b.use, PM_EINVAL, "bn_bwd_wino: both gradients of this convolution must take the Winograd route on one tiling (ask pm_bn_bwd_wino_bytes)");
+  PM_REQUIRE(v && z && pm_aligned16(v) && pm_aligned16(z) && (size_t)v_bytes >= b.dg.v_bytes && (size_t)z_bytes >= b.wg.m_bytes, PM_EINVAL,
+             "bn_bwd_wino: V needs %zu bytes, Z %zu (16B aligned)", b.dg.v_bytes, b.wg.m_bytes);
+  const pm_wino_bn bn = {mean, invstd, gamma, beta};
+  return pm_wino_bn_bwd_xf((const float*)g->ptr, g->pitch, (const float*)y->ptr, y->pitch, y->c, b.dg.Kp, b.dg.g, bn, sums, count, (float*)v, (float*)z,
+                           (hipStream_t)stream);
+}
+
 extern "C" size_t pm_conv_wxf_bytes(const pm_tensor* x, const pm_tensor* y, const pm_conv_params* p0) {
   if (!x || !y || !p0) return 0;
   const pm_conv_params tp = tier_params(p0, x, y);
@@ -1080,16 +1125,20 @@
     PM_REQUIRE(need != 0 && (size_t)ep->bn_partials_bytes >= need, PM_EINVAL, "conv_fwd: this call cannot emit bn_partials (ask pm_conv_bn_partials_bytes): %zu needed", need);
   }
   PM_REQUIRE(w && pm_aligned16(w), PM_EINVAL, "conv_fwd: weight null or unaligned");
+  const bool in_bn = ep && (ep->in_mean || ep->in_invstd || ep->in_gamma || ep->in_beta);
   {
     pm_conv_epilogue e1 = {(int64_t)sizeof(pm_conv_epilogue), nullptr, nullptr, nullptr, nullptr, 0, 0};
     if (ep) e1 = *ep;
     PM_REQUIRE((e1.scale == nullptr) == (e1.shift == nullptr), PM_EINVAL, "conv_fwd: scale and shift go together");
     const WinoPlan wp = wino_plan(x, y->c, p);
+    PM_REQUIRE(!in_bn || (wp.use && pm_is_f32(x) && e1.in_mean && e1.in_invstd && e1.in_gamma && e1.in_beta), PM_EINVAL,
+               "conv_fwd: an input BatchNorm needs all four vectors and a call on the fp32 Winograd route (ask pm_conv_winograd_v_bytes)");
     if (wp.use) {
       PM_REQUIRE(ws && ws_bytes >= wino_ws(wp), PM_EWORKSPACE, "conv_fwd(winograd): workspace %zu < %zu", ws_bytes, wino_ws(wp));
       float* keep = (p->wino_v && (size_t)p->wino_v_bytes >= wp.v_bytes) ? (float*)p->wino_v : nullptr;
       float* uext = (p->wxf && (size_t)p->wxf_bytes >= wp.u_bytes) ? (float*)p->wxf : nullptr;
-      return wino_conv(x, w, y->c, x->c, false, y, wp, e1, ws, (hipStream_t)stream, keep, uext, p->wxf_valid != 0);
+      const pm_wino_bn bn = {e1.in_mean, e1.in_invstd, e1.in_gamma, e1.in_beta};
+      return wino_conv(x, w, y->c, x->c, false, y, wp, e1, ws, (hipStream_t)stream, keep, uext, p->wxf_valid != 0, in_bn ? &bn : nullptr);
     }
   }
   if (p->prec == 2) {
@@ -1143,6 +1192,14 @@
   const long add_pitch = add ? add->pitch : 0;
   PM_REQUIRE(w && pm_aligned16(w), PM_EINVAL, "conv_bwd_data: weight null or unaligned");
   hipStream_t st0 = (hipStream_t)stream;
+  if (p->wino_v_valid) {
+    const WinoPlan wp = (pm_is_f32(dy) && pm_is_f32(dx) && !dgrad_bf16_ok(p)) ? wino_plan(dy, dx->c, p) : WinoPlan{};
+    PM_REQUIRE(wp.use && p->wino_v && (size_t)p->wino_v_bytes >= wp.v_bytes, PM_EINVAL,
+               "conv_bwd_data: wino_v_valid needs the fp32 Winograd route and a transform of %zu bytes", wp.use ? wp.v_bytes : (size_t)0);
+    PM_REQUIRE(ws && ws_bytes >= wino_ws(wp), PM_EWORKSPACE, "conv_bwd_data(winograd): workspace %zu < %zu", ws_bytes, wino_ws(wp));
+    const pm_conv_epilogue e1 = {(int64_t)sizeof(pm_conv_epilogue), nullptr, nullptr, nullptr, addp, add_pitch, 0};
+    return wino_conv(dy, w, dy->c, dx->c, true, dx, wp, e1, ws, st0, (float*)p->wino_v, nullptr, false, nullptr, true);
+  }
   if (p->stride == 2) {
     const size_t need = pm_conv_workspace(dx, dy, p, MODE_DGRAD);
     PM_REQUIRE(ws && ws_bytes >= need, PM_EWORKSPACE, "conv_bwd_data(stride 2): workspace %zu < %zu", ws_bytes, need);
@@ -1265,15 +1322,17 @@
   gemm_dims(MODE_WGRAD, x, dy, p, M, Nn, K);
   Plan pl = make_plan(MODE_WGRAD, M, Nn, K, p->prec != 0);
   const Bf16WgradPlan bw = tier ? Bf16WgradPlan{} : bf16_wgrad_plan(x, dy, p);
+  const WinoPlan wp = wino_plan(x, dy->c, p, true);
+  PM_REQUIRE(!p->wino_z || (wp.use && !bw.use && !tier && !dbias && (size_t)p->wino_z_bytes >= wp.m_bytes), PM_EINVAL,
+             "conv_bwd_weight: wino_z needs the fp32 Winograd route, no bias gradient and %zu bytes", wp.use ? wp.m_bytes : (size_t)0);
   if (bw.use) {
     if (int e = conv_wgrad_bf16(x, dy, dw, p, bw, ws, st)) return e;
     pl.ws_bytes = bf16_wgrad_ws(bw);
   }
-  const WinoPlan wp = wino_plan(x, dy->c, p, true);
   if (wp.use) {
     const WinoWgradPlan q = wino_wgrad_plan(wp, dy->c);
     float* kept = (p->wino_v && (size_t)p->wino_v_bytes >= wp.v_bytes) ? (float*)p->wino_v : nullptr;
-    if (int e = wino_wgrad(x, dy, dw, wp, q, ws, st, kept)) return e;
+    if (int e = wino_wgrad(x, dy, dw, wp, q, ws, st, kept, (float*)p->wino_z)) return e;
     pl.ws_bytes = wino_wgrad_ws(wp, q);
   }
   ConvK k;
diff --git a/pinthememory_amd/csrc/pm_common.h b/pinthememory_amd/csrc/pm_common.h
--- a/pinthememory_amd/csrc/pm_common.h
+++ b/pinthememory_amd/csrc/pm_common.h
@@ -43,7 +43,12 @@
   long tiles;
 };
 pm_wino_geom pm_wino_make_geom(int n, int h, int w, int d, int m);
-int pm_wino_input_xf(const float* x, long pitch, int C, int Kp, const pm_wino_geom& g, float* V, hipStream_t st);
+struct pm_wino_bn {
+  const float *mean, *invstd, *gamma, *beta;
+};
+int pm_wino_input_xf(const float* x, long pitch, int C, int Kp, const pm_wino_geom& g, float* V, hipStream_t st, const pm_wino_bn* bn = nullptr);
+int pm_wino_bn_bwd_xf(const float* gr, long gpitch, const float* y, long ypitch, int C, int Kp, const pm_wino_geom& g, const pm_wino_bn& bn, const float* sums,
+                      float count, float* V, float* Z, hipStream_t st);
 int pm_wino_filter_xf(const float* w, int Cout, int Cin, int Kp, bool dgrad, int m, float* U, hipStream_t st);
 int pm_wino_filter_xf_multi(const float* const* w, float* const* U, const int* cout, const int* cin, const int* kp, const int* m, int n, hipStream_t st);
 int pm_wino_output_xf(const float* M, int Cout, const pm_wino_geom& g, float* y, long ypitch, const float* bias, const float* scale, const float* shift,
diff --git a/pinthememory_amd/csrc/winograd.hip b/pinthememory_amd/csrc/winograd.hip
--- a/pinthememory_amd/csrc/winograd.hip
+++ b/pinthememory_amd/csrc/winograd.hip
@@ -1,4 +1,5 @@
 #include "pm_common.h"
+#include "bn_math.h"
 
 namespace {
 
@@ -108,8 +109,9 @@
   return t;
 }
 
-template <int MT, int W>
-__global__ __launch_bounds__(256) void wino_input_kernel(const float* __restrict__ x, long xp, int C, int Kp, const pm_wino_geom g, float* __restrict__ V) {
+template <int MT, int W, bool BN>
+__global__ __launch_bounds__(256) void wino_input_kernel(const float* __restrict__ x, long xp, int C, int Kp, const pm_wino_geom g, float* __restrict__ V,
+                                                         const pm_wino_bn bn) {
   constexpr int A = MT + 2;
   const unsigned kg = Kp / W;
   const unsigned total = (unsigned)g.tiles * kg;
@@ -119,6 +121,10 @@
     const int c = (int)(i - tile * kg) * W;
     const TileId t = decode_tile(tile, g);
     const bool cok = c < C;
+    Vec<W> mu, is, ga, be;
+    if constexpr (BN) {
+      if (cok) mu = vload<W>(bn.mean + c), is = vload<W>(bn.invstd + c), ga = vload<W>(bn.gamma + c), be = vload<W>(bn.beta + c);
+    }
     Vec<W> tt[A][A];
 #pragma unroll
     for (int b = 0; b < A; ++b) {
@@ -128,7 +134,14 @@
 #pragma unroll
       for (int a = 0; a < A; ++a) {
         const int yy = t.ry + g.d * (MT * t.ty + a - 1);
-        col[a] = (xok && (unsigned)yy < (unsigned)g.H) ? vload<W>(x + ((long)(t.n * g.H + yy) * g.W + xx) * xp + c) : vzero<W>();
+        const bool ok = xok && (unsigned)yy < (unsigned)g.H;
+        col[a] = ok ? vload<W>(x + ((long)(t.n * g.H + yy) * g.W + xx) * xp + c) : vzero<W>();
+        if constexpr (BN) {
+          if (ok) {
+#pragma unroll
+            for (int q = 0; q < W; ++q) col[a].v[q] = fmaxf(bn_affine(col[a].v[q], mu.v[q], is.v[q], ga.v[q], be.v[q]), 0.f);
+          }
+        }
       }
       mat_apply<MT, W_BT>(col, o);
 #pragma unroll
@@ -311,6 +324,78 @@
   }
 }
 
+template <int MT, int W>
+__global__ __launch_bounds__(256) void wino_bn_bwd_kernel(const float* __restrict__ gr, long gp, const float* __restrict__ y, long yp, int C, int Kp,
+                                                          const pm_wino_geom g, const pm_wino_bn bn, const float* __restrict__ sums, float count,
+                                                          float* __restrict__ V, float* __restrict__ Z) {
+  constexpr int A = MT + 2;
+  const unsigned kg = Kp / W;
+  const unsigned total = (unsigned)g.tiles * kg;
+  const long plane = g.tiles * (long)Kp, zplane = g.tiles * (long)C;
+  const float inv_n = count > 0.f ? 1.f / count : 1.f / sums[2 * C];
+  for (unsigned i = blockIdx.x * 256u + threadIdx.x; i < total; i += gridDim.x * 256u) {
+    const unsigned tile = i / kg;
+    const int c = (int)(i - tile * kg) * W;
+    const TileId t = decode_tile(tile, g);
+    const bool cok = c < C;
+    Vec<W> mu, is, ga, be, s1, s2;
+    if (cok) {
+      mu = vload<W>(bn.mean + c), is = vload<W>(bn.invstd + c), ga = vload<W>(bn.gamma + c), be = vload<W>(bn.beta + c);
+      s1 = vload<W>(sums + c), s2 = vload<W>(sums + C + c);
+    }
+    Vec<W> tt[A][A], zin[MT][MT];
+#pragma unroll
+    for (int b = 0; b < A; ++b) {
+      const int xx = t.rx + g.d * (MT * t.tx + b - 1);
+      const bool xok = cok && (unsigned)xx < (unsigned)g.W;
+      Vec<W> col[A], o[A];
+#pragma unroll
+      for (int a = 0; a < A; ++a) {
+        const int yy = t.ry + g.d * (MT * t.ty + a - 1);
+        col[a] = vzero<W>();
+        if (xok && (unsigned)yy < (unsigned)g.H) {
+          const long pix = (long)(t.n * g.H + yy) * g.W + xx;
+          const Vec<W> gv = vload<W>(gr + pix * gp + c), v = vload<W>(y + pix * yp + c);
+#pragma unroll
+          for (int q = 0; q < W; ++q) {
+            const float gm = bn_affine(v.v[q], mu.v[q], is.v[q], ga.v[q], be.v[q]) > 0.f ? gv.v[q] : 0.f;
+            col[a].v[q] = bn_bwd_dx(gm, v.v[q], mu.v[q], is.v[q], ga.v[q], s1.v[q], s2.v[q], inv_n);
+          }
+        }
+        if (a >= 1 && a <= MT && b >= 1 && b <= MT) zin[b - 1][a - 1] = col[a];
+      }
+      mat_apply<MT, W_BT>(col, o);
+#pragma unroll
+      for (int a = 0; a < A; ++a) tt[a][b] = o[a];
+    }
+    float* out = V + (long)tile * Kp + c;
+#pragma unroll
+    for (int a = 0; a < A; ++a) {
+      Vec<W> o[A];
+      mat_apply<MT, W_BT>(tt[a], o);
+#pragma unroll
+      for (int b = 0; b < A; ++b) vstore<W>(out + (a * A + b) * plane, o[b]);
+    }
+    if (!cok) continue;
+    Vec<W> r[A][MT];
+#pragma unroll
+    for (int b = 0; b < MT; ++b) {
+      Vec<W> o[A];
+      mat_apply<MT, W_A>(zin[b], o);
+#pragma unroll
+      for (int a = 0; a < A; ++a) r[a][b] = o[a];
+    }
+    float* zout = Z + (long)tile * C + c;
+#pragma unroll
+    for (int a = 0; a < A; ++a) {
+      Vec<W> o[A];
+      mat_apply<MT, W_A>(r[a], o);
+#pragma unroll
+      for (int b = 0; b < A; ++b) vstore<W>(zout + (a * A + b) * zplane, o[b]);
+    }
+  }
+}
+
 template <int MT>
 __global__ __launch_bounds__(256) void wino_dw_kernel(const float* __restrict__ slab, int ks, int Cout, int Cin, int Kp, float* __restrict__ dw) {
   constexpr int A = MT + 2, P = A * A;
@@ -511,10 +596,25 @@
   return g;
 }
 
-int pm_wino_input_xf(const float* x, long pitch, int C, int Kp, const pm_wino_geom& g, float* V, hipStream_t st) {
-  if (g.m == 4) hipLaunchKernelGGL((wino_input_kernel<4, 2>), dim3(nblocks(g.tiles * (Kp / 2))), dim3(256), 0, st, x, pitch, C, Kp, g, V);
-  else hipLaunchKernelGGL((wino_input_kernel<2, 4>), dim3(nblocks(g.tiles * (Kp / 4))), dim3(256), 0, st, x, pitch, C, Kp, g, V);
+int pm_wino_input_xf(const float* x, long pitch, int C, int Kp, const pm_wino_geom& g, float* V, hipStream_t st, const pm_wino_bn* bn) {
+  const pm_wino_bn b = bn ? *bn : pm_wino_bn{};
+  if (g.m == 4) {
+    if (bn) hipLaunchKernelGGL((wino_input_kernel<4, 2, true>), dim3(nblocks(g.tiles * (Kp / 2))), dim3(256), 0, st, x, pitch, C, Kp, g, V, b);
+    else hipLaunchKernelGGL((wino_input_kernel<4, 2, false>), dim3(nblocks(g.tiles * (Kp / 2))), dim3(256), 0, st, x, pitch, C, Kp, g, V, b);
+  } else {
+    if (bn) hipLaunchKernelGGL((wino_input_kernel<2, 4, true>), dim3(nblocks(g.tiles * (Kp / 4))), dim3(256), 0, st, x, pitch, C, Kp, g, V, b);
+    else hipLaunchKernelGGL((wino_input_kernel<2, 4, false>), dim3(nblocks(g.tiles * (Kp / 4))), dim3(256), 0, st, x, pitch, C, Kp, g, V, b);
+  }
   return pm_check_launch("wino_input");
+}
+
+int pm_wino_bn_bwd_xf(const float* gr, long gpitch, const float* y, long ypitch, int C, int Kp, const pm_wino_geom& g, const pm_wino_bn& bn, const float* sums,
+                      float count, float* V, float* Z, hipStream_t st) {
+  if (g.m == 4)
+    hipLaunchKernelGGL((wino_bn_bwd_kernel<4, 2>), dim3(nblocks(g.tiles * (Kp / 2))), dim3(256), 0, st, gr, gpitch, y, ypitch, C, Kp, g, bn, sums, count, V, Z);
+  else
+    hipLaunchKernelGGL((wino_bn_bwd_kernel<2, 4>), dim3(nblocks(g.tiles * (Kp / 4))), dim3(256), 0, st, gr, gpitch, y, ypitch, C, Kp, g, bn, sums, count, V, Z);
+  return pm_check_launch("wino_bn_bwd");
 }
 
 int pm_wino_filter_xf(const float* w, int Cout, int Cin, int Kp, bool dgrad, int m, float* U, hipStream_t st) {
diff --git a/pinthememory_amd/hip/kernels.py b/pinthememory_amd/hip/kernels.py
--- a/pinthememory_amd/hip/kernels.py
+++ b/pinthememory_amd/hip/kernels.py
@@ -206,7 +206,21 @@
     return _XFORM_COUNT[0]
 
 
-def conv_fwd(x, w_krsc, stride, pad, dil, bias=None, scale=None, shift=None, residual=None, relu=False, out=None, keep_v=None, bn_partials=None, out_dtype=None):
+def winograd_v_bytes(x, w_krsc, stride, pad, dil):
+    if not KEEP_WINOGRAD_V or x.dtype != torch.float32:
+        return 0
+    cout, kh, kw, cin = w_krsc.shape
+
+    def query():
+        n, h, w_, _ = x.shape
+        ho, wo = conv_out_hw(h, w_, kh, stride, pad, dil)
+        yd = L.PmTensor(None, n, ho, wo, cout, cout, L.PM_F32, 0)
+        return _lib().pm_conv_winograd_v_bytes(byref(tdesc(x)), byref(yd), byref(L.conv_params(kh, kw, stride, pad, dil, CONV_PREC)))
+    return _sizes(('v', x.shape, x.stride(), w_krsc.shape, stride, pad, dil, CONV_PREC, _GEN[0]), query)
+
+
+def conv_fwd(x, w_krsc, stride, pad, dil, bias=None, scale=None, shift=None, residual=None, relu=False, out=None, keep_v=None, bn_partials=None, out_dtype=None,
+             in_bn=None):
     cout, kh, kw, cin = w_krsc.shape
     n, h, w_, c = x.shape
     assert c == cin, 'conv: Cin mismatch %d vs %d' % (c, cin)
@@ -239,10 +253,10 @@
         part = torch.empty(npb // 4, dtype=torch.float32, device=x.device) if npb else None
         bn_partials.append(part)
     ep = None
-    if bias is not None or scale is not None or residual is not None or relu or part is not None:
+    if bias is not None or scale is not None or residual is not None or relu or part is not None or in_bn is not None:
         rd = tdesc(residual) if residual is not None else None
         ep = L.conv_epilogue(ptr(bias), ptr(scale), ptr(shift), rd.ptr if rd else None, rd.pitch if rd else 0, 1 if relu else 0, ptr(part),
-                            part.numel() * 4 if part is not None else 0)
+                            part.numel() * 4 if part is not None else 0, *([ptr(t) for t in in_bn] if in_bn is not None else []))
     check(lib.pm_conv_fwd(byref(xd), w_krsc.data_ptr(), byref(yd), byref(p), byref(ep) if ep else None, ptr(ws), nb, stream()), 'pm_conv_fwd')
     if u_ent is not None:
         ent, version = u_ent
@@ -252,11 +266,13 @@
     return y
 
 
-def conv_bwd_data(dy, w_krsc, x_shape, stride, pad, dil, add=None, dtype=None):
+def conv_bwd_data(dy, w_krsc, x_shape, stride, pad, dil, add=None, dtype=None, wino_dv=None):
     cout, kh, kw, cin = w_krsc.shape
     dx = new(x_shape, dy, dtype=dtype)
     dyd, dxd = tdesc(dy), tdesc(dx)
     p = L.conv_params(kh, kw, stride, pad, dil, CONV_PREC)
+    if wino_dv is not None:
+        p.wino_v, p.wino_v_bytes, p.wino_v_valid = wino_dv.data_ptr(), wino_dv.numel() * 4, 1
     lib = _lib()
     nb, nbu = _sizes(('d', dy.shape, dy.stride(), dy.dtype, dyd.flags, w_krsc.shape, dx.shape, dx.stride(), dx.dtype, stride, pad, dil, CONV_PREC, _GEN[0]),
                      lambda: (lib.pm_conv_workspace(byref(dxd), byref(dyd), byref(p), 1), lib.pm_conv_wxf_bytes_dgrad(byref(dyd), byref(dxd), byref(p))))
@@ -272,7 +288,7 @@
     return dx
 
 
-def conv_bwd_weight(x, dy, w_shape_krsc, stride, pad, dil, want_bias=False, wino_v=None, on_stream=None):
+def conv_bwd_weight(x, dy, w_shape_krsc, stride, pad, dil, want_bias=False, wino_v=None, on_stream=None, wino_z=None):
     cout, kh, kw, cin = w_shape_krsc
     dw = torch.empty(w_shape_krsc, dtype=torch.float32, device=x.device)
     db = torch.empty(cout, dtype=torch.float32, device=x.device) if want_bias else None
@@ -280,6 +296,8 @@
     p = L.conv_params(kh, kw, stride, pad, dil, CONV_PREC)
     if wino_v is not None:
         p.wino_v, p.wino_v_bytes = wino_v.data_ptr(), wino_v.numel() * 4
+    if wino_z is not None:
+        p.wino_z, p.wino_z_bytes = wino_z.data_ptr(), wino_z.numel() * 4
     lib = _lib()
     nb = _sizes(('w', x.shape, x.stride(), x.dtype, dy.shape, dy.stride(), dy.dtype, w_shape_krsc, stride, pad, dil, CONV_PREC, wino_v is not None, _GEN[0]),
                 lambda: lib.pm_conv_workspace(byref(xd), byref(dyd), byref(p), 2))
@@ -425,6 +443,24 @@
     check(_lib().pm_bn_bwd_apply(byref(tdesc(dy)), byref(yd) if yd else None, byref(tdesc(x)), mean.data_ptr(), invstd.data_ptr(), gamma.data_ptr(),
                                  ptr(beta), sums.data_ptr(), float(count), relu, byref(tdesc(dx)), byref(dr) if dr else None, stream()), 'pm_bn_bwd_apply')
     return dx, dres
+
+
+def bn_bwd_wino_bytes(y, cin, stride, pad, dil):
+    def query():
+        vb, zb = ctypes.c_int64(0), ctypes.c_int64(0)
+        rc = _lib().pm_bn_bwd_wino_bytes(byref(tdesc(y)), cin, byref(L.conv_params(3, 3, stride, pad, dil, CONV_PREC)), byref(vb), byref(zb))
+        return (vb.value, zb.value) if rc == 0 else None
+    return _sizes(('bw', y.shape, y.stride(), y.dtype, cin, stride, pad, dil, CONV_PREC, _GEN[0]), query)
+
+
+def bn_bwd_wino(dy, y, mean, invstd, gamma, beta, sums, count, cin, stride, pad, dil):
+    vb, zb = bn_bwd_wino_bytes(y, cin, stride, pad, dil)
+    v = torch.empty(vb // 4, dtype=torch.float32, device=y.device)
+    z = torch.empty(zb // 4, dtype=torch.float32, device=y.device)
+    check(_lib().pm_bn_bwd_wino(byref(tdesc(dy)), byref(tdesc(y)), mean.data_ptr(), invstd.data_ptr(), gamma.data_ptr(), beta.data_ptr(), sums.data_ptr(),
+                                float(count), cin, byref(L.conv_params(3, 3, stride, pad, dil, CONV_PREC)), v.data_ptr(), vb, z.data_ptr(), zb, stream()),
+          'pm_bn_bwd_wino')
+    return v, z
 
 
 def relu_bwd(dy, y):
diff --git a/pinthememory_amd/hip/lib.py b/pinthememory_amd/hip/lib.py
--- a/pinthememory_amd/hip/lib.py
+++ b/pinthememory_amd/hip/lib.py
@@ -28,7 +28,7 @@
 class PmConvParams(ctypes.Structure):
     _fields_ = [('struct_size', c_int32), ('kh', c_int32), ('kw', c_int32), ('stride', c_int32), ('pad', c_int32), ('dil', c_int32), ('prec', c_int32),
                 ('wino_v', c_void_p), ('wino_v_bytes', c_int64),
-                ('wxf', c_void_p), ('wxf_bytes', c_int64), ('wxf_valid', c_int32)]
+                ('wxf', c_void_p), ('wxf_bytes', c_int64), ('wxf_valid', c_int32), ('wino_v_valid', c_int32), ('wino_z', c_void_p), ('wino_z_bytes', c_int64)]
 
 
 class PmRouting(ctypes.Structure):
@@ -38,7 +38,8 @@
 
 class PmConvEpilogue(ctypes.Structure):
     _fields_ = [('struct_size', c_int64), ('bias', c_void_p), ('scale', c_void_p), ('shift', c_void_p), ('residual', c_void_p),
-                ('residual_pitch', c_int64), ('relu', c_int32), ('bn_partials', c_void_p), ('bn_partials_bytes', c_int64)]
+                ('residual_pitch', c_int64), ('relu', c_int32), ('bn_partials', c_void_p), ('bn_partials_bytes', c_int64),
+                ('in_mean', c_void_p), ('in_invstd', c_void_p), ('in_gamma', c_void_p), ('in_beta', c_void_p)]
 
 
 def conv_params(kh, kw, stride, pad, dil, prec=0):
@@ -49,7 +50,7 @@
     return PmConvEpilogue(ctypes.sizeof(PmConvEpilogue), *fields)
 
 
-ABI_VERSION = 400
+ABI_VERSION = 401
 
 
 class PinmemError(RuntimeError):
@@ -92,6 +93,8 @@
     'pm_bn_bwd_reduce_mask': (_i, [_T, _vp, _T, _vp, _vp, _T, _vp, _vp, _sz, _vp]),
     'pm_bn_bwd_reduce': (_i, [_T, _T, _T, _vp, _vp, _vp, _vp, _i, _T, _vp, _vp, _sz, _vp]),
     'pm_bn_bwd_apply': (_i, [_T, _T, _T, _vp, _vp, _vp, _vp, _vp, _f, _i, _T, _T, _vp]),
+    'pm_bn_bwd_wino_bytes': (_i, [_T, _i, _P, POINTER(c_int64), POINTER(c_int64)]),
+    'pm_bn_bwd_wino': (_i, [_T, _T, _vp, _vp, _vp, _vp, _vp, _f, _i, _P, _vp, _i64, _vp, _i64, _vp]),
     'pm_relu_bwd': (_i, [_T, _T, _T, _vp]),
     'pm_add': (_i, [_T, _T, _T, _vp]),
     'pm_add_n': (_i, [POINTER(_T), _i, _T, _vp]),
diff --git a/pinthememory_amd/hip/ops.py b/pinthememory_amd/hip/ops.py
--- a/pinthememory_amd/hip/ops.py
+++ b/pinthememory_amd/hip/ops.py
@@ -130,16 +130,18 @@
     return (p, True) if p is not None else (weight, False)
 
 
-def _wgrad(x, dy, wshape, geom, want_bias=False, deferred=False, wino_v=None):
+def _wgrad(x, dy, wshape, geom, want_bias=False, deferred=False, wino_v=None, wino_z=None):
     if not deferred:
-        return K.conv_bwd_weight(x, dy, wshape, *geom, want_bias=want_bias, wino_v=wino_v)
+        return K.conv_bwd_weight(x, dy, wshape, *geom, want_bias=want_bias, wino_v=wino_v, wino_z=wino_z)
     side, main = _side_stream(), L.stream_obj()
     ev = torch.cuda.Event()
     ev.record(main)
     side.wait_event(ev)
-    out = K.conv_bwd_weight(x, dy, wshape, *geom, want_bias=want_bias, wino_v=wino_v, on_stream=side)
+    out = K.conv_bwd_weight(x, dy, wshape, *geom, want_bias=want_bias, wino_v=wino_v, on_stream=side, wino_z=wino_z)
     if wino_v is not None:
         wino_v.record_stream(side)
+    if wino_z is not None:
+        wino_z.record_stream(side)
     x.record_stream(side)
     dy.record_stream(side)
     for t in out:
@@ -185,7 +187,11 @@
             and len({y.shape[3] for y in ys}) == 1)
 
 
-def _bn_train_fwd(y, gamma, beta, bn, residual, relu, out=None, partials=None, want_mask=False):
+FOLD_BN_WINO_FWD = True
+FOLD_BN_WINO_BWD = False
+
+
+def _bn_train_stats(y, bn, partials=None):
     c = y.shape[3]
     pixels = y.shape[0] * y.shape[1] * y.shape[2]
     if bn.group is None and BN_FUSED_FINALIZE:
@@ -202,10 +208,26 @@
         if bn.group is not None:
             mom = D.merge_moments(mom, c, bn.group)
         mean, invstd = K.bn_finalize(mom, c, bn.eps, bn.running_mean, bn.running_var, bn.momentum)
+    return mean, invstd
+
+
+def _bn_train_fwd(y, gamma, beta, bn, residual, relu, out=None, partials=None, want_mask=False):
+    mean, invstd = _bn_train_stats(y, bn, partials)
     if want_mask:
         o, mask = K.bn_apply(y, mean, invstd, gamma, beta, residual=residual, relu=relu, out=out, want_mask=True)
         return o, mean, invstd, mask
     return K.bn_apply(y, mean, invstd, gamma, beta, residual=residual, relu=relu, out=out), mean, invstd
+
+
+def _bn_relu_bwd_sums(dv, y, mean, invstd, gamma, beta, group):
+    local, _ = K.bn_bwd_reduce(dv, None, y, mean, invstd, 2, gamma, beta, want_gmask=False, with_count=group is not None)
+    sums = D.all_reduce_sum_copy(local, group) if group is not None else local
+    count = float(y.shape[0] * y.shape[1] * y.shape[2]) if group is None else -1.0
+    return sums, local, count
+
+
+def _fold_bwd(y, cin, geom):
+    return FOLD_BN_WINO_BWD and y.dtype == torch.float32 and K.bn_bwd_wino_bytes(y, cin, *geom) is not None
 
 
 def _bn_train_bwd(dv, o, y, mean, invstd, gamma, beta, relu, group, want_dres, has_res, mask=None):
@@ -236,9 +258,14 @@
         k1, k2, k3 = K.krsc(w1), K.krsc(w2), K.krsc(w3)
         ps = []
         y1 = K.conv_fwd(xv, k1, *geoms[0], bn_partials=ps)
-        o1, m1, i1 = _bn_train_fwd(y1, g1, b1, bns[0], None, True, partials=ps[0])
         kv = []
-        y2 = K.conv_fwd(o1, k2, *geoms[1], keep_v=kv, bn_partials=ps)
+        if FOLD_BN_WINO_FWD and K.winograd_v_bytes(y1, k2, *geoms[1]):
+            m1, i1 = _bn_train_stats(y1, bns[0], ps[0])
+            o1 = None
+            y2 = K.conv_fwd(y1, k2, *geoms[1], keep_v=kv, bn_partials=ps, in_bn=(m1, i1, g1, b1))
+        else:
+            o1, m1, i1 = _bn_train_fwd(y1, g1, b1, bns[0], None, True, partials=ps[0])
+            y2 = K.conv_fwd(o1, k2, *geoms[1], keep_v=kv, bn_partials=ps)
         o2, m2, i2 = _bn_train_fwd(y2, g2, b2, bns[1], None, True, partials=ps[1])
         y3 = K.conv_fwd(o2, k3, *geoms[2], bn_partials=ps)
         merged = False
@@ -287,9 +314,18 @@
             dy3, dres, dg3, db3 = _bn_train_bwd(dv, out, y3, m3, i3, g3, b3, True, gr[2], True, True, mask=mask3)
         dw3, _ = _wgrad(o2, dy3, tuple(k3.shape), ge[2], deferred=df[2])
         do2 = K.conv_bwd_data(dy3, k3, tuple(o2.shape), *ge[2])
-        dy2, _, dg2, db2 = _bn_train_bwd(do2, o2, y2, m2, i2, g2, b2, True, gr[1], False, False)
-        dw2, _ = _wgrad(o1, dy2, tuple(k2.shape), ge[1], deferred=df[1], wino_v=v2)
-        do1 = K.conv_bwd_data(dy2, k2, tuple(o1.shape), *ge[1])
+        x2 = o1 if o1 is not None else y1
+        if v2 is not None and _fold_bwd(y2, k2.shape[3], ge[1]):
+            s2, l2, n2 = _bn_relu_bwd_sums(do2, y2, m2, i2, g2, b2, gr[1])
+            c2 = y2.shape[3]
+            dg2, db2 = l2[c2:2 * c2], l2[:c2]
+            vd2, z2 = K.bn_bwd_wino(do2, y2, m2, i2, g2, b2, s2, n2, k2.shape[3], *ge[1])
+            dw2, _ = _wgrad(x2, y2, tuple(k2.shape), ge[1], deferred=df[1], wino_v=v2, wino_z=z2)
+            do1 = K.conv_bwd_data(y2, k2, tuple(x2.shape), *ge[1], wino_dv=vd2)
+        else:
+            dy2, _, dg2, db2 = _bn_train_bwd(do2, o2, y2, m2, i2, g2, b2, True, gr[1], False, False)
+            dw2, _ = _wgrad(x2, dy2, tuple(k2.shape), ge[1], deferred=df[1], wino_v=v2)
+            do1 = K.conv_bwd_data(dy2, k2, tuple(x2.shape), *ge[1])
         dy1, _, dg1, db1 = _bn_train_bwd(do1, o1, y1, m1, i1, g1, b1, True, gr[0], False, False)
         dw1, _ = _wgrad(xv, dy1, tuple(k1.shape), ge[0], deferred=df[0])
         dwd = dgd = dbd = None
@@ -392,6 +428,13 @@
         stride, pad, dil = ctx.geom
         dv = _grad_view(dout)
         want_dres = ctx.has_res and ctx.needs_input_grad[5]
+        if ctx.train and ctx.relu and not ctx.has_res and not ctx.has_bias and vk is not None and _fold_bwd(y, wk.shape[3], ctx.geom):
+            sums, local, count = _bn_relu_bwd_sums(dv, y, mean, invstd, gamma, beta, ctx.group)
+            c = y.shape[3]
+            vd, z = K.bn_bwd_wino(dv, y, mean, invstd, gamma, beta, sums, count, wk.shape[3], stride, pad, dil)
+            dx = nchw(K.conv_bwd_data(y, wk, tuple(xv.shape), stride, pad, dil, dtype=xv.dtype, wino_dv=vd)) if ctx.needs_input_grad[0] else None
+            dwk, _ = _wgrad(xv, y, tuple(wk.shape), (stride, pad, dil), deferred=ctx.deferred, wino_v=vk, wino_z=z)
+            return dx, dwk.permute(0, 3, 1, 2), None, local[c:2 * c], local[:c], None, None, None, None, None, None
         if ctx.train:
             dy, dres, dgamma, dbeta = _bn_train_bwd(dv, o, y, mean, invstd, gamma, beta, ctx.relu, ctx.group, want_dres, ctx.has_res)
         else:
```

New measurement: 155.7 (median of 4 runs). No clear change (+0.0%).
